# marbl/Winnowmap

Measured on AMD Instinct MI355X. Metric: mapped Gbp/s, higher is better.
Workload: dtype int8

## Files before the change

__graft_entry__.py:

```python
import os
import sys

ROOT = os.path.dirname(os.path.abspath(__file__))
sys.path.insert(0, ROOT)
sys.path.insert(0, os.path.join(ROOT, "tests"))


def build():
    from winnowmap_amd import build as b
    b.build_gpu(verbose=True)
    b.build_oracle()
    b.build_emu()
    b.build_emu_selfmap()
    b.build_emu_sdust()
    b.build_emu_heapseed()
    b.build_emu_evenk()
    b.build_emu_sketchsteps()
    b.build_emu_extra()
    b.build_emu_fix()
    b.build_emu_eqx()
    b.build_emu_cs()
    b.build_emu_chain()
    b.build_harness()
    import winnowmap_amd
    from winnowmap_amd import gpu
    gpu.lib()


def smoke():
    import numpy as np
    from winnowmap_amd import gpu
    import wmtest as W
    import kswcases
    ctx = gpu.Context(0, 2 << 30)
    cases = kswcases.ont_segments(5, 64)
    sc = gpu.KswScore(2, -4, -1, 4, 2, 24, 1)
    jobs, seqs = gpu.pack_jobs([(c["q"], c["t"], dict(w=c["w"], zdrop=c["zdrop"], end_bonus=c["end_bonus"], flag=c["flag"])) for c in cases])
    res, pool = ctx.ksw_batch(sc, jobs, seqs)
    for i, c in enumerate(cases):
        o = W.o_ksw_extd2(c["q"], c["t"], w=c["w"], zdrop=c["zdrop"], end_bonus=c["end_bonus"], flag=c["flag"])
        assert all(int(res[i][k]) == o[k] for k in W.EZ_FIELDS), (i, res[i], o)
        assert np.array_equal(pool[res[i]["cig_off"]:res[i]["cig_off"] + res[i]["n_cigar"]], o["cigar"]), i
    import ctypes as C
    import tempfile
    from winnowmap_amd import build as b, synth
    tmp = tempfile.mkdtemp()
    ref = synth.make_reference(1, 200000, 5, repeat_frac=0.1)
    fa = os.path.join(tmp, "ref.fa")
    synth.write_fasta(fa, ref)
    km, cnt = synth.repetitive_kmers(ref, 15)
    kf = os.path.join(tmp, "rep.txt")
    synth.write_kmer_list(kf, km, cnt, 15)
    reads, _ = synth.make_reads(ref, 4, 12000, 6, profile="ont", sv_frac=0.25)
    rs = [synth.codes_to_ascii(r) for r in reads]
    idx = gpu.Index(fa, kf, k=15, w=50, n_threads=4)
    idx.upload(ctx)
    m = gpu.Mapper(ctx, idx, "map-ont", gpu.MM_F_CIGAR | gpu.MM_F_OUT_CG)
    text, hits, cigars, first = m.map(["r%d" % i for i in range(len(rs))], rs)
    H = C.CDLL(b.build_harness())
    H.h_index_build.restype = C.c_void_p
    H.h_index_build.argtypes = [C.c_char_p, C.c_char_p, C.c_int, C.c_int, C.c_int]
    H.h_map_many.argtypes = [C.c_void_p, C.c_char_p, C.c_int64, C.c_int, C.POINTER(C.c_char_p), W.i32p, C.c_int, W.i32p, C.c_int, C.POINTER(C.c_int64), W.u32p, C.c_int64, C.POINTER(C.c_int64)]
    hh = H.h_index_build(fa.encode(), kf.encode(), 15, 50, 4)
    n = len(rs)
    ho = np.zeros(16 * 1024, np.int32); co = np.zeros(4000000, np.uint32); hf = (C.c_int64 * (n + 1))(); nc = C.c_int64()
    nh = H.h_map_many(hh, b"map-ont", 0x4 | 0x20, n, (C.c_char_p * n)(*rs), np.array([len(r) for r in rs], np.int32), 2, ho, 1024, hf, co, len(co), C.byref(nc))
    assert nh == len(hits) and nh > 0, (nh, len(hits))
    assert np.array_equal(ho[:16 * nh].reshape(-1, 16), hits) and np.array_equal(co[:nc.value], cigars) and list(hf) == list(first)
    m.close(); idx.close(); ctx.close()
    print("smoke OK: %d ksw alignments and %d end-to-end hits (%d CIGAR ops) bit-exact vs the oracle" % (len(cases), nh, nc.value))


if __name__ == "__main__":
    build()
    if len(sys.argv) > 1 and sys.argv[1] == "smoke":
        smoke()
```

include/wm_gpu.h:

```cpp
#ifndef WM_GPU_H
#define WM_GPU_H
#include <stdint.h>
#include <stddef.h>
#ifdef __cplusplus
extern "C" {
#endif

#define WM_OK        0
#define WM_ENODEV   (-1)
#define WM_EINVAL   (-2)
#define WM_ENOMEM   (-3)
#define WM_EINTERNAL (-4)

typedef struct wm_ctx_s wm_ctx_t;

typedef struct { uint64_t x, y; } wm128_t;

int wm_ctx_create(int device, size_t arena_bytes, wm_ctx_t **out);
void wm_ctx_destroy(wm_ctx_t *ctx);
const char *wm_last_error(void);
const char *wm_build_defines(void);
int wm_device_count(void);
float wm_last_kernel_ms(const wm_ctx_t *ctx);
int wm_ctx_device(const wm_ctx_t *ctx);

typedef struct {
	int8_t match, mismatch, sc_ambi;
	int8_t q, e, q2, e2;
} wm_ksw_score_t;

typedef struct {
	uint32_t q_off, t_off;
	int32_t qlen, tlen;
	int32_t w, zdrop, end_bonus, flag;
} wm_ksw_job_t;

typedef struct {
	int32_t max, zdropped, max_q, max_t, mqe, mqe_t, mte, mte_q, score, reach_end;
	int32_t n_cigar;
	uint32_t cig_off;
} wm_ksw_result_t;

#define WM_KSW_MAX_TLEN (1 << 28)

int wm_ksw_batch(wm_ctx_t *ctx, const wm_ksw_score_t *sc, int n_jobs, const wm_ksw_job_t *jobs,
                 const uint8_t *seqs, size_t seqs_bytes,
                 wm_ksw_result_t *results, uint32_t *cigar_pool, size_t cigar_cap, size_t *cigar_used);

typedef struct {
	int64_t qwin_off;
	int32_t qwin_len, q_pos;
	int32_t rid, t_pos;
	int32_t qlen, tlen;
	int32_t w, zdrop, end_bonus, flag;
	int8_t step, has_n, pad[6];
} wm_ksw_pos_t;
int wm_reads_upload(wm_ctx_t *ctx, const uint8_t *codes, size_t n);
int wm_ksw_batch_pos(wm_ctx_t *ctx, const wm_ksw_score_t *sc, int n_jobs, const wm_ksw_pos_t *jobs,
                     wm_ksw_result_t *results, uint32_t *cigar_pool, size_t cigar_cap, size_t *cigar_used);
#define WM_KSW_F_ZDWALK 0x10000
typedef struct { int32_t max_zdrop, t0, t1, q0, q1; } wm_zd_t;
int wm_ksw_batch_pos_zd(wm_ctx_t *ctx, const wm_ksw_score_t *sc, int n_jobs, const wm_ksw_pos_t *jobs,
                        wm_ksw_result_t *results, uint32_t *cigar_pool, size_t cigar_cap, size_t *cigar_used, wm_zd_t *zd);

#define WM_EXTRA_MAX_ABS (1 << 30)
typedef struct { int32_t match, mismatch, ambi, q, e; } wm_extra_score_t;
typedef struct { uint32_t q_off, t_off; uint32_t cig_off; int32_t n_cigar; } wm_extra_job_t;
typedef struct { int64_t qwin_off; int32_t qwin_len, q_pos, rid, t_pos; uint32_t cig_off; int32_t n_cigar; } wm_extra_pos_t;
typedef struct { int32_t dp_max, mlen, blen, n_ambi, qoff, toff; } wm_extra_res_t;
int wm_extra_batch(wm_ctx_t *ctx, const wm_extra_score_t *score, int n_jobs, const wm_extra_job_t *jobs, const uint8_t *seqs, size_t seqs_bytes,
                   const uint32_t *cigars, size_t n_ops, wm_extra_res_t *out);
int wm_extra_batch_pos(wm_ctx_t *ctx, const wm_extra_score_t *score, int n_jobs, const wm_extra_pos_t *jobs, const uint32_t *cigars, size_t n_ops,
                       wm_extra_res_t *out);
typedef struct { int32_t n_cigar, qshift, tshift, changed; } wm_fix_res_t;
int wm_fix_extra_batch(wm_ctx_t *ctx, const wm_extra_score_t *score, int n_jobs, const wm_extra_job_t *jobs, const uint8_t *seqs, size_t seqs_bytes,
                       const uint32_t *cigars, size_t n_ops, uint32_t *cigars_out, wm_fix_res_t *fix_out, wm_extra_res_t *extra_out);
int wm_fix_extra_batch_pos(wm_ctx_t *ctx, const wm_extra_score_t *score, int n_jobs, const wm_extra_pos_t *jobs, const uint32_t *cigars, size_t n_ops,
                           uint32_t *cigars_out, wm_fix_res_t *fix_out, wm_extra_res_t *extra_out);
void wm_extra_set_routing(int long_min_cols, int tile_cols);
int wm_extra_tile_cols(void);
void wm_set_extra_device(int on);
int wm_extra_device_enabled(void);
void wm_extra_stats(uint64_t *out6, int reset);
void wm_set_fix_device(int on);
int wm_fix_device_enabled(void);
void wm_fix_stats(uint64_t *out7, int reset);
typedef struct { uint64_t off; int32_t n_cigar, in_place; } wm_eqx_res_t;
int wm_eqx_batch(wm_ctx_t *ctx, int n_jobs, const wm_extra_job_t *jobs, const uint8_t *seqs, size_t seqs_bytes, const uint32_t *cigars, size_t n_ops,
                 uint32_t *cigars_out, size_t out_cap, size_t *out_used, wm_eqx_res_t *out);
int wm_eqx_batch_pos(wm_ctx_t *ctx, int n_jobs, const wm_extra_pos_t *jobs, const uint32_t *cigars, size_t n_ops,
                     uint32_t *cigars_out, size_t out_cap, size_t *out_used, wm_eqx_res_t *out);
void wm_set_eqx_device(int on);
int wm_eqx_device_enabled(void);
void wm_eqx_stats(uint64_t *out6, int reset);
#define WM_CS_SHORT 0
#define WM_CS_LONG  1
#define WM_CS_MD    2
typedef struct { uint64_t off; uint32_t len; int32_t pad; } wm_cs_res_t;
int wm_cs_batch(wm_ctx_t *ctx, int mode, int n_jobs, const wm_extra_job_t *jobs, const uint8_t *seqs, size_t seqs_bytes, const uint32_t *cigars, size_t n_ops,
                char *text_out, size_t out_cap, size_t *out_used, wm_cs_res_t *out);
int wm_cs_batch_pos(wm_ctx_t *ctx, int mode, int n_jobs, const wm_extra_pos_t *jobs, const uint32_t *cigars, size_t n_ops,
                    char *text_out, size_t out_cap, size_t *out_used, wm_cs_res_t *out);
void wm_set_cs_device(int on);
int wm_cs_device_enabled(void);
void wm_cs_stats(uint64_t *out6, int reset);

int wm_debug_stripe_timing(uint64_t *out16, int reset);

int wm_ksw_ll_i16(int qlen, const uint8_t *query, int tlen, const uint8_t *target, const int8_t *mat5x5, int gapo, int gape, int *qe, int *te);

int wm_ksw_exts2_batch(wm_ctx_t *ctx, const wm_ksw_score_t *sc, int noncan, int junc_bonus, int n_jobs, const wm_ksw_job_t *jobs,
                       const uint8_t *seqs, size_t seqs_bytes, const uint8_t *junc,
                       wm_ksw_result_t *results, uint32_t *cigar_pool, size_t cigar_cap, size_t *cigar_used);

typedef struct wm_ksw_dev_batch_s wm_ksw_dev_batch_t;
int wm_ksw_dev_prepare(wm_ctx_t *ctx, const wm_ksw_score_t *sc, int n_jobs, const wm_ksw_job_t *jobs,
                       const uint8_t *seqs, size_t seqs_bytes, wm_ksw_dev_batch_t **out);
int wm_ksw_dev_run(wm_ctx_t *ctx, wm_ksw_dev_batch_t *b);
int wm_ksw_dev_fetch(wm_ctx_t *ctx, wm_ksw_dev_batch_t *b, wm_ksw_result_t *results,
                     uint32_t *cigar_pool, size_t cigar_cap, size_t *cigar_used);
int wm_ksw_dev_stats(const wm_ksw_dev_batch_t *b, uint64_t *cells, uint64_t *tb_bytes, float *dp_ms, float *bt_ms);
void wm_ksw_dev_free(wm_ctx_t *ctx, wm_ksw_dev_batch_t *b);

void wm_ksw_set_routing(int on, int rows4, int rows8);
void wm_ksw_set_chain_routing(int mode, int min_rows_exact, int bp);
void wm_ksw_set_dual(int on);
int wm_ksw_dual_enabled(void);

int wm_ksw_extd2(wm_ctx_t *ctx, int qlen, const uint8_t *query, int tlen, const uint8_t *target, int8_t m,
                 const int8_t *mat, int8_t q, int8_t e, int8_t q2, int8_t e2, int w, int zdrop, int end_bonus,
                 int flag, wm_ksw_result_t *ez, uint32_t **cigar_out);

typedef struct wm_index_s wm_index_t;
int wm_index_build(const char *fasta, const char *kmer_file, int k, int w, int n_threads, wm_index_t **out);
int wm_index_build_gpu(wm_ctx_t *ctx, const char *fasta, const char *kmer_file, int k, int w, int n_threads, wm_index_t **out, double *stats);
int wm_index_build_flag(const char *fasta, const char *kmer_file, int k, int w, int idx_flag, int n_threads, wm_index_t **out);
int wm_index_build_gpu_flag(wm_ctx_t *ctx, const char *fasta, const char *kmer_file, int k, int w, int idx_flag, int n_threads, wm_index_t **out, double *stats);
void wm_index_destroy(wm_index_t *idx);
int wm_index_save(const wm_index_t *idx, const char *path);
int wm_index_load(const char *path, const char *kmer_file, wm_index_t **out);
int wm_index_upload(wm_ctx_t *ctx, const wm_index_t *idx);
int wm_index_read_junc_bed(wm_index_t *idx, const char *path);
int wm_index_add_junc(wm_index_t *idx, int ctg, int n, const int32_t *st, const int32_t *en, const int32_t *strand);
int wm_index_n_seq(const wm_index_t *idx);
const char *wm_index_seq_name(const wm_index_t *idx, int rid);
int wm_index_seq_len(const wm_index_t *idx, int rid);
uint64_t wm_index_n_minimizers(const wm_index_t *idx);
const uint64_t *wm_index_get(const wm_index_t *idx, uint64_t minier, int *n);

int wm_write_repetitive_kmers(const char *fasta, int k, double distinct, const char *out_path, uint64_t *n_out);
int wm_write_repetitive_kmers_gpu(wm_ctx_t *ctx, const char *fasta, int k, double distinct, const char *out_path, uint64_t *n_out, double *stats);
int wm_index_export(const wm_index_t *idx, uint64_t *sizes9, uint32_t *S, uint64_t *hkey, uint64_t *hval, uint64_t *P, uint8_t *bloom,
                    uint64_t *seq_meta, char *names);
int wm_index_import(const uint64_t *sizes9, const uint32_t *S, const uint64_t *hkey, const uint64_t *hval, const uint64_t *P, const uint8_t *bloom,
                    const uint64_t *seq_meta, const char *names, wm_index_t **out);

int wm_sketch_batch(wm_ctx_t *ctx, int n, const uint8_t *seqs, size_t seqs_bytes, const uint64_t *seq_off, const int32_t *len,
                    wm128_t *out, size_t out_cap, uint64_t *out_off, int32_t *counts);
int wm_sketch_set_filter(wm_ctx_t *ctx, const uint8_t *bits, size_t n_bytes, uint64_t table_bits, uint32_t salt0, uint32_t salt1, int k, int w);
int wm_seed_batch(wm_ctx_t *ctx, int n, const wm128_t *mini, const uint64_t *mini_off, const int32_t *n_mini, const int32_t *qlen,
                  int max_occ, int64_t flag, wm128_t *out, size_t out_cap, uint64_t *out_off, int32_t *n_anchors, int32_t *rep_len);
typedef struct { uint32_t lo, eq; } wm_qkey_t;
int wm_index_query_key(const wm_index_t *idx, const char *qname, wm_qkey_t *key);
int wm_seed_batch_keyed(wm_ctx_t *ctx, int n, const wm128_t *mini, const uint64_t *mini_off, const int32_t *n_mini, const int32_t *qlen, const wm_qkey_t *keys,
                        int max_occ, int64_t flag, wm128_t *out, size_t out_cap, uint64_t *out_off, int32_t *n_anchors, int32_t *rep_len);
typedef struct { int32_t max_dist_x, min_dist_x, max_dist_y, bw, max_skip, max_iter, min_cnt, min_sc; float gap_scale;
                 int32_t is_cdna;  } wm_chain_par_t;
int wm_chain_batch(wm_ctx_t *ctx, int n, wm128_t *a, const uint64_t *a_off, const int32_t *n_a, const wm_chain_par_t *par,
                   uint64_t *u, uint64_t *u_off, int32_t *n_u, int32_t *n_v);
typedef struct {
	int64_t seq_off;
	uint64_t stage_off, pre_off;
	int32_t len, n_pre;
	wm_chain_par_t par;
} wm_window_job_t;
typedef struct { int32_t n_anchors, rep_len, n_mini, n_u, n_v; uint32_t u_off, a_off; } wm_window_res_t;
int wm_window_batch(wm_ctx_t *ctx, int n, const wm_window_job_t *jobs, const uint8_t *seqs, size_t seqs_bytes, const wm128_t *pre, size_t n_pre_total,
                    int max_occ, int64_t flag, wm_window_res_t *res, uint64_t *u_pool, size_t u_cap, size_t *u_used, wm128_t *a_pool, size_t a_cap, size_t *a_used);
int wm_window_batch_keyed(wm_ctx_t *ctx, int n, const wm_window_job_t *jobs, const wm_qkey_t *keys, const uint8_t *seqs, size_t seqs_bytes, const wm128_t *pre, size_t n_pre_total,
                          int max_occ, int64_t flag, wm_window_res_t *res, uint64_t *u_pool, size_t u_cap, size_t *u_used, wm128_t *a_pool, size_t a_cap, size_t *a_used);
int wm_window_batch_dust(wm_ctx_t *ctx, int n, const wm_window_job_t *jobs, const wm_qkey_t *keys, const uint8_t *seqs, size_t seqs_bytes, const wm128_t *pre, size_t n_pre_total,
                         int max_occ, int64_t flag, int sdust_thres, wm_window_res_t *res, uint64_t *u_pool, size_t u_cap, size_t *u_used, wm128_t *a_pool, size_t a_cap, size_t *a_used);
int wm_sdust_batch(wm_ctx_t *ctx, int n, const uint8_t *seqs, size_t seqs_bytes, const uint64_t *seq_off, const int32_t *len, const uint8_t *resident, int thres,
                   int32_t *iv, size_t iv_cap, uint64_t *iv_off, int32_t *n_iv, int32_t *p_high);
void wm_sdust_stats(double *out5, int reset);
void wm_exts2_stats(uint64_t *out2, int reset);
float wm_last_aux_ms(const wm_ctx_t *ctx);
void wm_sketch_set_step_chunks(int on);
int wm_last_sketch_chunks(const wm_ctx_t *ctx);

typedef struct wm_mapper_s wm_mapper_t;
int wm_mapper_create(wm_ctx_t *ctx, const wm_index_t *idx, const char *preset, int64_t flag, wm_mapper_t **out);
void wm_mapper_destroy(wm_mapper_t *m);
void wm_set_even_k(int on);
int wm_even_k_enabled(void);
int wm_mapper_set_threads(wm_mapper_t *m, int n_threads, size_t arena_bytes_per_group);
int wm_map_reads(wm_mapper_t *m, int n, const char *const *names, const char *const *seqs, const int32_t *lens,
                 const char **text, size_t *text_len, const int32_t **hits, const uint32_t **cigars, const int64_t **hit_first);
#define WM_MAX_SLOTS 4
int wm_map_reads_slot(wm_mapper_t *m, int slot, int n, const char *const *names, const char *const *seqs, const int32_t *lens,
                      const char **text, size_t *text_len, const int32_t **hits, const uint32_t **cigars, const int64_t **hit_first);
int wm_mapper_set_slots(wm_mapper_t *m, int n);
int wm_map_reads_rep_len_defined(const wm_mapper_t *m, int slot, const uint8_t **flags, size_t *n);
int wm_map_file(wm_mapper_t *m, const char *reads_path, const char *out_path, int64_t mini_batch_bases, double *stats);
int wm_index_upload_dev(wm_ctx_t *ctx, const wm_index_t *idx, const void *d_S, const void *d_hkey, const void *d_hval, const void *d_P, const void *d_bloom, int src_device);
int wm_index_upload_peer(wm_ctx_t *dst, const wm_index_t *idx, const wm_ctx_t *src);
int wm_map_file_multi(wm_mapper_t *const *mappers, int n, const char *reads_path, const char *out_path, int64_t mini_batch_bases, double *stats);
int wm_mapper_set_cmdline(wm_mapper_t *m, int argc, const char *const *argv);
int wm_set_cmdline(int argc, const char *const *argv);
typedef struct {
	int64_t flag;
	int32_t seed, sdust_thres, max_qlen;
	int32_t bw, max_gap, max_gap_ref, min_gap_ref, max_frag_len;
	int32_t max_chain_skip, max_chain_iter, min_cnt, min_chain_score;
	float chain_gap_scale;
	int32_t SVaware, SVawareMinReadLength, suffixSampleOffset, min_mapq;
	float min_qcov;
	int32_t minPrefixLength, maxPrefixLength;
	float prefixIncrementFactor;
	int32_t stage2_bw, stage2_zdrop_inv, stage2_max_gap;
	float mask_level;
	int32_t mask_len;
	float pri_ratio;
	int32_t best_n;
	int32_t max_join_long, max_join_short, min_join_flank_sc;
	float min_join_flank_ratio, alt_drop;
	int32_t a, b, q, e, q2, e2, sc_ambi;
	int32_t zdrop, zdrop_inv, end_bonus, min_dp_max, min_ksw_len;
	float max_clip_ratio;
	float mid_occ_frac;
	int32_t min_mid_occ, mid_occ, max_occ;
	int64_t mini_batch_size, max_sw_mat;
	int32_t noncan, junc_bonus;
	int32_t anchor_ext_len, anchor_ext_shift;
} wm_mapopt_t;
int wm_mapopt_preset(const char *preset, wm_mapopt_t *out, int *k, int *w);
int wm_mapper_create_opt(wm_ctx_t *ctx, const wm_index_t *idx, const wm_mapopt_t *opt, wm_mapper_t **out);
int wm_index_build_parts(const char *fasta, const char *kmer_file, int k, int w, int n_threads, uint64_t batch_bases, wm_index_t **out, int cap, int *n_parts);
int wm_map_file_split(wm_ctx_t *ctx, int n_parts, wm_index_t *const *parts, const wm_mapopt_t *opt, int n_threads, const char *reads_path, const char *out_path,
                      int64_t mini_batch_bases, double *stats);
typedef struct wm_split_s wm_split_t;
int wm_split_begin(wm_ctx_t *ctx, const wm_mapopt_t *opt, int k, int w, int n_threads, const char *reads_path, int64_t mini_batch_bases, wm_split_t **out);
int wm_split_add_part(wm_split_t *s, wm_index_t *part);
int wm_split_finish(wm_split_t *s, const char *out_path, double *stats);
void wm_split_abort(wm_split_t *s);
int wm_map_file_split_fasta(wm_ctx_t *ctx, const char *fasta, const char *kmer_file, int k, int w, int build_threads, uint64_t batch_bases, int on_device,
                            const wm_mapopt_t *opt, int n_threads, const char *reads_path, const char *out_path, int64_t mini_batch_bases, double *stats, int *n_parts);

int wm_mapper_set_sam_header(wm_mapper_t *m, int on);
int wm_mapper_stats(const wm_mapper_t *m, uint64_t *out9);
int wm_mapper_kernel_stats(const wm_mapper_t *m, double *out, int cap, int *n_classes);
int wm_ksw_n_classes(void);
int wm_ctx_kernel_stats(const wm_ctx_t *ctx, double *out, int cap, int *n_classes);
int wm_mapper_kernel_union(const wm_mapper_t *m, double since_ms, double *out, int cap, double *now_ms);
int wm_mapper_host_stats(const wm_mapper_t *m, double *out, int cap);
int wm_sam_header(const wm_index_t *idx, int argc, const char *const *argv, const char **text, size_t *text_len);

#ifdef __cplusplus
}
#endif
#endif
```

winnowmap_amd/build.py:

```python
import os
import subprocess
import sys

HERE = os.path.dirname(os.path.abspath(__file__))
ROOT = os.path.dirname(HERE)
CSRC = os.path.join(HERE, "csrc")
LIB = os.path.join(HERE, "libwmgpu.so")
HIPCC = os.environ.get("HIPCC", "/opt/rocm/bin/hipcc")


class _Lock:

    def __init__(self, target):
        self.path = target + ".lock"

    def __enter__(self):
        import fcntl
        self.f = open(self.path, "w")
        fcntl.flock(self.f, fcntl.LOCK_EX)

    def __exit__(self, *a):
        import fcntl
        fcntl.flock(self.f, fcntl.LOCK_UN)
        self.f.close()
# ... 49 lines not shown
        if any(rcs):
            raise subprocess.CalledProcessError(next(r for r in rcs if r), cmds[next(i for i, r in enumerate(rcs) if r)])
        link = lambda out_: [HIPCC, "--offload-arch=gfx950", "-shared", "-fPIC", "-o", out_] + [os.path.join(objdir, u + ".o") for u in UNITS] + ["-lz", "-lpthread"]
        if verbose:
            print(" ".join(link(LIB)), file=sys.stderr)
        _run_to(LIB, link)
        with open(stamp, "w") as f:
            f.write(defines)
    return LIB


def build_oracle():
    with _Lock(os.path.join(ROOT, "oracle", "libwm_oracle.so")):
        subprocess.check_call(["make", "-C", os.path.join(ROOT, "oracle"), "oracle"], stdout=subprocess.DEVNULL)
        if os.path.exists("/root/reference/src/map.c"):
            subprocess.check_call(["make", "-C", os.path.join(ROOT, "oracle"), "ref", "-j8"], stdout=subprocess.DEVNULL)
            if os.path.exists(LIB):
                subprocess.check_call(["make", "-C", os.path.join(ROOT, "oracle"), "wm", "subst", "-j8"], stdout=subprocess.DEVNULL)


def build_emu(defines=()):
    emu = os.path.join(ROOT, "tests", "simt_emu")
    tag = "".join("_" + "".join(ch if ch.isalnum() else "_" for ch in d) for d in defines)
    out = os.path.join(emu, "libwm_emu%s.so" % tag)
    srcs = [os.path.join(emu, f) for f in ("emu_driver.cpp", "simt.h")] + [os.path.join(CSRC, f) for f in os.listdir(CSRC) if f.endswith(".h")]
    with _Lock(out):
        if _newer(out, srcs):
            _run_to(out, lambda o: ["g++", "-O1", "-std=c++17", "-fPIC", "-shared", "-ffp-contract=off", "-Wno-unknown-pragmas"] +
                    ["-D" + d for d in defines] + ["-I" + emu, "-I" + CSRC, "-o", o, os.path.join(emu, "emu_driver.cpp")])
    return out


def build_emu_selfmap():
    emu = os.path.join(ROOT, "tests", "simt_emu")
    out = os.path.join(emu, "libwm_emu_selfmap.so")
    srcs = [os.path.join(emu, f) for f in ("emu_selfmap.cpp", "simt.h")] + \
           [os.path.join(CSRC, f) for f in ("seedchain_kernel.h", "window_kernel.h", "wm_internal.h", os.path.join("host", "wm_names.h"))]
    with _Lock(out):
        if _newer(out, srcs):
            _run_to(out, lambda o: ["g++", "-O1", "-std=c++17", "-fPIC", "-shared", "-ffp-contract=off", "-Wno-unknown-pragmas",
                                    "-I" + emu, "-I" + CSRC, "-o", o, os.path.join(emu, "emu_selfmap.cpp")])
    return out


def build_emu_heapseed():
    emu = os.path.join(ROOT, "tests", "simt_emu")
    out = os.path.join(emu, "libwm_emu_heapseed.so")
    core = os.path.join(CSRC, "host", "wm_core.cpp")
    srcs = [os.path.join(emu, f) for f in ("emu_heapseed.cpp", "simt.h")] + [core] + \
           [os.path.join(CSRC, f) for f in ("seedchain_kernel.h", "window_kernel.h", "wm_internal.h", os.path.join("host", "wm_core.h"))]
    with _Lock(out):
        if _newer(out, srcs):
            _run_to(out, lambda o: ["g++", "-O1", "-std=c++17", "-fPIC", "-shared", "-pthread", "-ffp-contract=off", "-Wno-unknown-pragmas",
                                    "-I" + emu, "-I" + CSRC, "-o", o, os.path.join(emu, "emu_heapseed.cpp"), core])
    return out


def build_emu_sdust(defines=()):
    emu = os.path.join(ROOT, "tests", "simt_emu")
    tag = "".join("_" + "".join(ch if ch.isalnum() else "_" for ch in d) for d in defines)
    out = os.path.join(emu, "libwm_emu_sdust%s.so" % tag)
    srcs = [os.path.join(emu, f) for f in ("emu_sdust.cpp", "simt.h")] + \
           [os.path.join(CSRC, f) for f in ("sdust_kernel.h", "sketch_kernel.h", "reads2bit.h", "wm_internal.h", os.path.join("host", "wm_sdust.h"), os.path.join("host", "wm_core.h"))]
    with _Lock(out):
        if _newer(out, srcs):
            _run_to(out, lambda o: ["g++", "-O3", "-std=c++17", "-fPIC", "-shared", "-ffp-contract=off", "-Wno-unknown-pragmas"] +
                    ["-D" + d for d in defines] + ["-I" + emu, "-I" + CSRC, "-o", o, os.path.join(emu, "emu_sdust.cpp")])
    return out


def build_emu_evenk():
    emu = os.path.join(ROOT, "tests", "simt_emu")
    out = os.path.join(emu, "libwm_emu_evenk.so")
    srcs = [os.path.join(emu, f) for f in ("emu_evenk.cpp", "simt.h")] + [os.path.join(CSRC, f) for f in ("sketch_kernel.h", "reads2bit.h", "wm_internal.h")]
    with _Lock(out):
        if _newer(out, srcs):
            _run_to(out, lambda o: ["g++", "-O3", "-std=c++17", "-fPIC", "-shared", "-ffp-contract=off", "-Wno-unknown-pragmas",
                                    "-I" + emu, "-I" + CSRC, "-o", o, os.path.join(emu, "emu_evenk.cpp")])
    return out


def build_emu_sketchsteps():
    emu = os.path.join(ROOT, "tests", "simt_emu")
    out = os.path.join(emu, "libwm_emu_sketchsteps.so")
    srcs = [os.path.join(emu, f) for f in ("emu_sketchsteps.cpp", "simt.h")] + [os.path.join(CSRC, f) for f in ("sketch_kernel.h", "reads2bit.h", "wm_internal.h")]
    with _Lock(out):
        if _newer(out, srcs):
            _run_to(out, lambda o: ["g++", "-O3", "-std=c++17", "-fPIC", "-shared", "-ffp-contract=off", "-Wno-unknown-pragmas",
                                    "-I" + emu, "-I" + CSRC, "-o", o, os.path.join(emu, "emu_sketchsteps.cpp")])
    return out


def build_emu_extra():
    emu = os.path.join(ROOT, "tests", "simt_emu")
    out = os.path.join(emu, "libwm_emu_extra.so")
    srcs = [os.path.join(emu, f) for f in ("emu_extra.cpp", "simt.h")] + [os.path.join(CSRC, f) for f in ("extra_kernel.h", "reads2bit.h")] + \
           [os.path.join(ROOT, "include", "wm_gpu.h")]
    with _Lock(out):
        if _newer(out, srcs):
            _run_to(out, lambda o: ["g++", "-O2", "-std=c++17", "-fPIC", "-shared", "-ffp-contract=off", "-Wno-unknown-pragmas",
                                    "-I" + emu, "-I" + CSRC, "-o", o, os.path.join(emu, "emu_extra.cpp")])
    return out


def build_emu_fix():
    emu = os.path.join(ROOT, "tests", "simt_emu")
    out = os.path.join(emu, "libwm_emu_fix.so")
    srcs = [os.path.join(emu, f) for f in ("emu_fix.cpp", "simt.h")] + \
           [os.path.join(CSRC, f) for f in ("fix_kernel.h", "cigar_fix.h", "extra_kernel.h", "reads2bit.h")] + [os.path.join(ROOT, "include", "wm_gpu.h")]
    with _Lock(out):
        if _newer(out, srcs):
            _run_to(out, lambda o: ["g++", "-O2", "-std=c++17", "-fPIC", "-shared", "-ffp-contract=off", "-Wno-unknown-pragmas",
                                    "-I" + emu, "-I" + CSRC, "-o", o, os.path.join(emu, "emu_fix.cpp")])
    return out


def build_emu_eqx():
    emu = os.path.join(ROOT, "tests", "simt_emu")
    out = os.path.join(emu, "libwm_emu_eqx.so")
    srcs = [os.path.join(emu, f) for f in ("emu_eqx.cpp", "simt.h")] + \
           [os.path.join(CSRC, f) for f in ("eqx_kernel.h", "cigar_eqx.h", "extra_kernel.h", "reads2bit.h")] + [os.path.join(ROOT, "include", "wm_gpu.h")]
    with _Lock(out):
        if _newer(out, srcs):
            _run_to(out, lambda o: ["g++", "-O2", "-std=c++17", "-fPIC", "-shared", "-ffp-contract=off", "-Wno-unknown-pragmas",
                                    "-I" + emu, "-I" + CSRC, "-o", o, os.path.join(emu, "emu_eqx.cpp")])
    return out


def build_emu_cs():
    emu = os.path.join(ROOT, "tests", "simt_emu")
    out = os.path.join(emu, "libwm_emu_cs.so")
    srcs = [os.path.join(emu, f) for f in ("emu_cs.cpp", "simt.h")] + \
           [os.path.join(CSRC, f) for f in ("cs_kernel.h", "cigar_cs.h", "extra_kernel.h", "reads2bit.h")] + [os.path.join(ROOT, "include", "wm_gpu.h")]
    with _Lock(out):
        if _newer(out, srcs):
            _run_to(out, lambda o: ["g++", "-O2", "-std=c++17", "-fPIC", "-shared", "-ffp-contract=off", "-Wno-unknown-pragmas",
                                    "-I" + emu, "-I" + CSRC, "-o", o, os.path.join(emu, "emu_cs.cpp")])
    return out


def build_emu_fix_main(sanitize=True):
    emu = os.path.join(ROOT, "tests", "simt_emu")
    out = os.path.join(emu, "emu_fix_main_san" if sanitize else "emu_fix_main")
    srcs = [os.path.join(emu, f) for f in ("emu_fix_main.cpp", "emu_fix.cpp", "simt.h")] + \
           [os.path.join(CSRC, f) for f in ("fix_kernel.h", "cigar_fix.h", "extra_kernel.h", "reads2bit.h")] + [os.path.join(ROOT, "include", "wm_gpu.h")]
    with _Lock(out):
        if _newer(out, srcs):
            _run_to(out, lambda o: ["g++", "-O1", "-g", "-std=c++17", "-ffp-contract=off", "-Wno-unknown-pragmas"] +
                                   (["-fsanitize=address,undefined", "-fno-sanitize-recover=undefined", "-fno-omit-frame-pointer"] if sanitize else []) +
                                   ["-I" + emu, "-I" + CSRC, "-o", o, os.path.join(emu, "emu_fix_main.cpp"), os.path.join(emu, "emu_fix.cpp")])
    return out


def build_emu_stripe(defines=()):
    emu = os.path.join(ROOT, "tests", "simt_emu")
    tag = "".join("_" + "".join(ch if ch.isalnum() else "_" for ch in d) for d in defines)
    out = os.path.join(emu, "libwm_emu_stripe%s.so" % tag)
    srcs = [os.path.join(emu, f) for f in ("emu_stripe.cpp", "simt.h")] + \
           [os.path.join(CSRC, f) for f in ("ksw_stripe_kernel.h", "ksw_packed_kernel.h", "ksw_kernel.h", "ksw_plan.h")]
    with _Lock(out):
        if _newer(out, srcs):
            _run_to(out, lambda o: ["g++", "-O1", "-std=c++17", "-fPIC", "-shared", "-pthread", "-ffp-contract=off", "-Wno-unknown-pragmas"] +
                    ["-D" + d for d in defines] + ["-I" + emu, "-I" + CSRC, "-o", o, os.path.join(emu, "emu_stripe.cpp")])
    return out


def build_emu_chain(defines=()):
    emu = os.path.join(ROOT, "tests", "simt_emu")
    tag = "".join("_" + "".join(ch if ch.isalnum() else "_" for ch in d) for d in defines)
    out = os.path.join(emu, "libwm_emu_chain%s.so" % tag)
    srcs = [os.path.join(emu, f) for f in ("emu_chain.cpp", "simt.h")] + \
           [os.path.join(CSRC, f) for f in ("ksw_chain_kernel.h", "ksw_stripe_kernel.h", "ksw_packed_kernel.h", "ksw_kernel.h", "ksw_plan.h")]
    with _Lock(out):
        if _newer(out, srcs):
            _run_to(out, lambda o: ["g++", "-O1", "-std=c++17", "-fPIC", "-shared", "-pthread", "-ffp-contract=off", "-Wno-unknown-pragmas"] +
                    ["-D" + d for d in defines] + ["-I" + emu, "-I" + CSRC, "-o", o, os.path.join(emu, "emu_chain.cpp")])
    return out


def build_harness():
    hd = os.path.join(ROOT, "tests", "host_harness")
    out = os.path.join(hd, "libwm_harness.so")
    srcs = [os.path.join(hd, "harness.cpp"), os.path.join(ROOT, "oracle", "wm_oracle.c")] + \
           [os.path.join(CSRC, "host", f) for f in os.listdir(os.path.join(CSRC, "host"))]
    with _Lock(out):
        if _newer(out, srcs):
            _run_to(out, lambda o: ["g++", "-std=c++17", "-O2", "-g", "-ffp-contract=off", "-fPIC", "-shared", "-o", o,
                                    os.path.join(hd, "harness.cpp"), os.path.join(ROOT, "oracle", "wm_oracle.c"), "-lz", "-pthread"])
    return out


if __name__ == "__main__":
    build_gpu(force="--force" in sys.argv, verbose=True)
    build_oracle()
    build_emu()
    build_emu_selfmap()
    build_emu_heapseed()
    build_emu_sdust()
    build_emu_evenk()
    build_emu_sketchsteps()
    build_emu_extra()
    build_emu_fix()
    build_emu_eqx()
    build_emu_cs()
    build_emu_stripe()
    build_emu_chain()
    build_harness()
```

winnowmap_amd/csrc/wm_ksw.hip:

```cpp
#include "wm_rt.h"
#include "simt.h"
#include "ksw_kernel.h"
#include "ksw_packed_kernel.h"
#include "ksw_packed_multi_kernel.h"
#include "ksw_dual_kernel.h"
#include "ksw_stripe_kernel.h"
#include "ksw_chain_kernel.h"
#include "ksw_exts2_kernel.h"
#include "cigar_walk.h"
#include "reads2bit.h"

#ifndef WM_OCC_HINT
#define WM_OCC_HINT 1
#endif
template <int BP, bool CLIP, bool HASN, bool EXACT>
__global__ __launch_bounds__(64, (WM_OCC_HINT && BP == 8 && CLIP && EXACT) ? 4 : 1) void ksw_dpp_kernel(wm_ksw_score_t sc, const wm_ksw_djob_t *__restrict__ jobs,
                                                      const int *__restrict__ order, const uint8_t *__restrict__ seqs,
                                                      uint8_t *__restrict__ tb, wm_ksw_dres_t *__restrict__ res)
{
	if constexpr (EXACT || CLIP || BP >= 16) WM_SETPRIO(2);
	const int j = order[blockIdx.x];
	wmk::ksw_dp_packed<BP, CLIP, HASN, EXACT>(sc, jobs[j], seqs, tb, res + j);
}

// ... 433 lines not shown
			for (int kk = 129; kk >= 0; --kk) { pos_[kk] = acc; acc += cnt[kk]; }
			tmp.resize(o.size());
			for (int j : o) tmp[pos_[size_key(j)]++] = j;
			o.swap(tmp);
		}
	}
	size_t chain_mw = 0;
	bool chain_any = false;
	for (int kc = 0; kc < WM_KSW_NCLASS - WM_KSW_CHAIN; ++kc) {
		const int sw = 128 * wm_ksw_chain_bp[kc >> 2];
		const std::vector<int> &o = b->order[WM_KSW_CHAIN + kc];
		b->d_cmap[kc][0] = b->d_cmap[kc][1] = 0;
		for (size_t jo = 0; jo < o.size(); ++jo) {
			const wm_ksw_djob_t &d = b->jobs[o[jo]];
			const int nwv = wm_chain_nwv(d.n_col, d.tlen, sw);
			std::vector<uint4> &cm = b->cmap[kc][(d.flag & KSW_F_APPROX_MAX) ? 0 : 1];
			for (int wv = 0; wv < nwv; ++wv) cm.push_back(make_uint4((unsigned)jo, (unsigned)wv, (unsigned)(chain_mw / 16), (unsigned)nwv));
			chain_mw += ((size_t)wm_chain_box::words(nwv) + 15) & ~(size_t)15;
			chain_any = true;
		}
	}
	const size_t nj = n_jobs > 0 ? n_jobs : 1;
	auto al256 = [](size_t x) { return (x + 255) & ~(size_t)255; };
	const size_t o_ord = al256(nj * sizeof(wm_ksw_djob_t)), o_src = o_ord + al256(nj * sizeof(int));
	size_t o_cm[WM_KSW_NCLASS - WM_KSW_CHAIN][2], tab_bytes = o_src + (pos ? al256(nj * sizeof(wm_ksw_dsrc_t)) : 0);
	for (int kc = 0; kc < WM_KSW_NCLASS - WM_KSW_CHAIN; ++kc)
		for (int e = 0; e < 2; ++e) { o_cm[kc][e] = tab_bytes; tab_bytes += al256(b->cmap[kc][e].size() * sizeof(uint4)); }
	uint8_t *d_tab = (uint8_t*)arena_take(c, tab_bytes);
	b->d_jobs = (wm_ksw_djob_t*)d_tab;
	b->d_order = d_tab ? (int*)(d_tab + o_ord) : 0;
	for (int kc = 0; kc < WM_KSW_NCLASS - WM_KSW_CHAIN && d_tab; ++kc)
		for (int e = 0; e < 2; ++e) if (!b->cmap[kc][e].empty()) b->d_cmap[kc][e] = (uint4*)(d_tab + o_cm[kc][e]);
	b->d_res = (wm_ksw_dres_t*)arena_take(c, al256(nj * sizeof(wm_ksw_dres_t)) + nj * 4 + 64);
	b->d_off = b->d_res ? (uint32_t*)((uint8_t*)b->d_res + al256(nj * sizeof(wm_ksw_dres_t))) : 0;
	b->d_err = (int*)arena_take(c, 64);
	b->d_total = b->d_err ? (uint32_t*)(b->d_err + 1) : 0;
	bool any_zd = false;
	for (int i = 0; i < n_jobs && !any_zd; ++i) any_zd = (b->jobs[i].flag & WM_KSW_F_ZDWALK) != 0;
	b->d_zd = any_zd ? (wm_zd_t*)arena_take(c, nj * sizeof(wm_zd_t)) : 0;
	b->d_seqs = (uint8_t*)arena_take(c, slab_bytes + 64);
	b->slab_bytes = slab_bytes;
	wm_ksw_dsrc_t *d_src = pos && d_tab ? (wm_ksw_dsrc_t*)(d_tab + o_src) : 0;
	b->d_cig = (uint32_t*)arena_take(c, (cig_off + 16) * 4);
	b->pool_cap = cig_off + 16;
	b->d_pool = (uint32_t*)arena_take(c, b->pool_cap * 4);
	b->d_tb = (uint8_t*)arena_take(c, tb_off + 64);
	{
		uint64_t go = 0;
		for (int j : b->order[WM_KSW_GENERIC]) { const uint64_t T = ((uint64_t)b->jobs[j].tlen + 15) / 16 * 16; b->goff.push_back(go); go += 12 * T + 256; }
		b->d_gscratch = (uint8_t*)arena_take(c, go + 256);
		b->d_goff = (uint64_t*)arena_take(c, b->goff.size() * 8 + 64);
		if (!b->d_gscratch || !b->d_goff) b->d_tb = 0;
		uint64_t so = 0;
		for (int j : b->order[WM_KSW_BLOCK3]) { b->b3off.push_back(so); so += 3 * wm_ksw_blk3_wn(b->jobs[j].tlen); }
		b->d_b3state = (uint8_t*)arena_take(c, so * 4 + 256);
		b->d_b3off = (uint64_t*)arena_take(c, b->b3off.size() * 8 + 64);
		if (!b->d_b3state || !b->d_b3off) b->d_tb = 0;
	}
	if (chain_any) {
		b->mail_words = chain_mw;
		b->d_mail = (wm_mbox_t*)arena_take(c, chain_mw * 8 + 256);
		b->d_tickets = (int*)arena_take(c, 64 * sizeof(int));
		if (!b->d_mail || !b->d_tickets) b->d_tb = 0;
	}
	if (!b->d_jobs || !b->d_order || !b->d_res || !b->d_off || !b->d_total || !b->d_err || !b->d_seqs || (any_zd && !b->d_zd) || (pos && !d_src) || !b->d_cig || !b->d_pool || !b->d_tb) {
		c->arena_used = b->arena_mark;
		delete b;
		return set_err(WM_ENOMEM, "batch needs %.1f MB of traceback + buffers; arena is %.1f MB", (tb_off + cig_off * 8 + slab_bytes) / 1048576.0, c->arena_bytes / 1048576.0);
	}
	b->ord.clear();
	b->ord.reserve(nj);
	for (int k = 0; k < WM_KSW_NCLASS; ++k) b->ord.insert(b->ord.end(), b->order[k].begin(), b->order[k].end());
	UBuf<uint8_t> ptab(tab_bytes, c);
	if (n_jobs) memcpy(ptab.data(), b->jobs.data(), (size_t)n_jobs * sizeof(wm_ksw_djob_t));
	if (!b->ord.empty()) memcpy(ptab.data() + o_ord, b->ord.data(), b->ord.size() * sizeof(int));
	if (pos && n_jobs > 0) memcpy(ptab.data() + o_src, dsrc.data(), (size_t)n_jobs * sizeof(wm_ksw_dsrc_t));
	for (int kc = 0; kc < WM_KSW_NCLASS - WM_KSW_CHAIN; ++kc)
		for (int e = 0; e < 2; ++e)
			if (!b->cmap[kc][e].empty()) memcpy(ptab.data() + o_cm[kc][e], b->cmap[kc][e].data(), b->cmap[kc][e].size() * sizeof(uint4));
	HIPCHK(hipMemcpyAsync(d_tab, ptab.data(), tab_bytes, hipMemcpyHostToDevice, c->stream));
	if (pos) {
		if (n_jobs > 0) hipLaunchKernelGGL(ksw_expand_kernel, dim3(n_jobs), dim3(64), 0, c->stream, b->d_jobs, d_src, c->d_reads, c->d_reads_nm, c->d_S, b->d_seqs);
	} else if (slab_bytes) HIPCHK(hipMemcpyAsync(b->d_seqs, seqs + slab_lo, slab_bytes, hipMemcpyHostToDevice, c->stream));
	if (!b->goff.empty()) HIPCHK(hipMemcpyAsync(b->d_goff, b->goff.data(), b->goff.size() * 8, hipMemcpyHostToDevice, c->stream));
	if (!b->b3off.empty()) HIPCHK(hipMemcpyAsync(b->d_b3off, b->b3off.data(), b->b3off.size() * 8, hipMemcpyHostToDevice, c->stream));
	HIPCHK(ctx_sync(c));
	*out = b;
	return WM_OK;
}

extern "C" int wm_ksw_dev_prepare(wm_ctx_t *c, const wm_ksw_score_t *sc_in, int n_jobs, const wm_ksw_job_t *jobs,
                                  const uint8_t *seqs, size_t seqs_bytes, wm_ksw_dev_batch_t **out)
{
	return ksw_prepare_impl(c, sc_in, n_jobs, jobs, seqs, seqs_bytes, 0, out);
}

int reads_alloc(wm_ctx_t *c, size_t cap)
{
	const size_t pkw = cap / 32 + 2, nmw = cap / 64 + 2;
	c->d_reads = 0; c->d_reads_nm = 0; c->reads_cap = 0;
	if (hipMalloc((void**)&c->d_reads, (pkw + nmw) * 8) != hipSuccess) { (void)hipGetLastError(); c->d_reads = 0; return set_err(WM_ENOMEM, "cannot allocate %zu bytes for the resident reads", (pkw + nmw) * 8); }
	c->d_reads_nm = c->d_reads + pkw;
	c->reads_cap = cap;
	return WM_OK;
}
extern "C" int wm_reads_upload(wm_ctx_t *c, const uint8_t *codes, size_t n)
{
	if (!c || (n && !codes)) return set_err(WM_EINVAL, "null argument");
	HIPCHK(hipSetDevice(c->device));
	if (!c->owns_reads) { c->d_reads = 0; c->d_reads_nm = 0; c->reads_cap = 0; }
	if (n + 256 > c->reads_cap) {
		if (c->d_reads) HIPCHK(hipFree(c->d_reads));
		c->d_reads = 0; c->d_reads_nm = 0; c->reads_cap = 0;
		const size_t cap = (n + n / 8 + (1 << 20) + 255) & ~(size_t)255;
		const int rc = reads_alloc(c, cap);
		if (rc) return rc;
	}
	c->owns_reads = true;
	std::vector<uint64_t> pk(wm_pk_words(n)), nm(wm_nm_words(n));
	wm_pack_codes(codes, n, pk.data(), nm.data());
	HIPCHK(hipMemcpy(c->d_reads, pk.data(), pk.size() * 8, hipMemcpyHostToDevice));
	HIPCHK(hipMemcpy(c->d_reads_nm, nm.data(), nm.size() * 8, hipMemcpyHostToDevice));
	c->reads_bytes = n;
	return WM_OK;
}

static bool pmulti_lean() { static const bool v = !(getenv("WM_KSW_PMULTI_LEAN") && atoi(getenv("WM_KSW_PMULTI_LEAN")) == 0); return v; }
static int ksw_pmulti_level() { const char *e = getenv("WM_KSW_PMULTI"); return e ? atoi(e) : 2; }

extern "C" int wm_ksw_dev_run(wm_ctx_t *c, wm_ksw_dev_batch_t *b)
{
	HIPCHK(hipSetDevice(c->device));
	const int n = b->n_jobs;
	if (n == 0) return WM_OK;
	HIPCHK(hipMemsetAsync(b->d_err, 0, 4, c->stream));
	if (b->d_mail) {
		HIPCHK(hipMemsetAsync(b->d_mail, 0xff, b->mail_words * 8, c->stream));
		HIPCHK(hipMemsetAsync(b->d_tickets, 0, 64 * sizeof(int), c->stream));
	}
	if (!b->degenerate.empty()) hipLaunchKernelGGL(ksw_reset_kernel, dim3((n + 255) / 256), dim3(256), 0, c->stream, n, b->d_jobs, b->d_res);
	HIPCHK(hipEventRecord(c->ev[0], c->stream));
	int off = 0;
	static const bool trace_k = getenv("WM_TRACE_KSW") != 0;
	auto class_done = [&](int k, double t0) {
		if (!trace_k) return;
		hipStreamSynchronize(c->stream);
		const std::vector<int> &o = b->order[k];
		const wm_ksw_djob_t &big = b->jobs[o[0]];
		fprintf(stderr, "[ksw class %2d] jobs %zu  %.2f ms  largest q=%d t=%d w=%d flag=0x%x n_col=%d\n", k, o.size(), now_ms() - t0, big.qlen, big.tlen, big.w, big.flag, big.n_col);
	};
	int n_nonempty = 0, used_mask = 0, rr = 0;
	for (int k = 0; k < WM_KSW_NCLASS; ++k) n_nonempty += !b->order[k].empty();
	static const int n_side = std::max(0, std::min(4, getenv("WM_SIDE_STREAMS") ? atoi(getenv("WM_SIDE_STREAMS")) : 3));
	const bool fan = n_nonempty > 1 && !trace_k && n_side > 0;
	if (fan) HIPCHK(hipEventRecord(c->kev[4], c->stream));
	hipStream_t ks = c->stream;
	hipStream_t side[4] = {0, 0, 0, 0};
	int pool_lo = 0, pool_n = c->n_side_pool, wclass = 0;
	if (c->side_pool && c->n_side_pool >= 6) {
		static const long heavy_units = getenv("WM_KSW_HEAVY_UNITS") ? atol(getenv("WM_KSW_HEAVY_UNITS")) : 8192, huge_units = getenv("WM_KSW_HUGE_UNITS") ? atol(getenv("WM_KSW_HUGE_UNITS")) : 131072;
		static int split_l = -1, split_h = -1;
		if (split_l < 0) { int a, h; side_split(c->n_side_pool, &a, &h); split_h = h; split_l = a; }
		if (split_l > 0 && split_h > 0 && split_l + split_h < c->n_side_pool) {
			long mx = 0;
			for (const wm_ksw_djob_t &d : b->jobs) {
				if (d.klass < 0) continue;
				long w_ = d.w < 0 ? std::max(d.qlen, d.tlen) : d.w, nn = std::min(d.qlen, d.tlen);
				if (nn > w_ + 1) nn = w_ + 1;
				mx = std::max(mx, ((long)d.qlen + d.tlen) * ((nn + 127) / 128 + 1));
			}
			wclass = huge_units > 0 && mx > huge_units ? 2 : heavy_units > 0 && mx > heavy_units ? 1 : 0;
			pool_lo = wclass == 0 ? 0 : wclass == 1 ? split_l : split_l + split_h;
			pool_n = wclass == 0 ? split_l : wclass == 1 ? split_h : c->n_side_pool - split_l - split_h;
		}
	}
	const int n_use = c->side_pool ? std::min(n_side, pool_n) : n_side;
	if (fan && n_use > 0) {
		if (c->side_pool) { const unsigned b0 = c->side_next[wclass].fetch_add((unsigned)n_use); for (int i = 0; i < n_use; ++i) side[i] = c->side_pool[pool_lo + (int)((b0 + (unsigned)i) % (unsigned)pool_n)]; }
		else for (int i = 0; i < n_use; ++i) { if (!c->kstream[i]) HIPCHK(hipStreamCreateWithFlags(&c->kstream[i], hipStreamNonBlocking)); side[i] = c->kstream[i]; }
	}
	auto next_stream = [&]() {
		if (!fan || n_use <= 0) return;
		const int si = rr++ % n_use;
		ks = side[si];
		if (!(used_mask >> si & 1)) { hipStreamWaitEvent(ks, c->kev[4], 0); used_mask |= 1 << si; }
	};
	static const bool class_events = !(getenv("WM_KSW_CLASS_EVENTS") && atoi(getenv("WM_KSW_CLASS_EVENTS")) == 0);
	int offs[WM_KSW_NCLASS + 1];
	offs[0] = 0;
	for (int k = 0; k < WM_KSW_NCLASS; ++k) offs[k + 1] = offs[k] + (int)b->order[k].size();
	int lorder[WM_KSW_NCLASS], nl = 0;
	lorder[nl++] = WM_KSW_GENERIC; lorder[nl++] = WM_KSW_BLOCK3; lorder[nl++] = WM_KSW_BLOCK2; lorder[nl++] = WM_KSW_BLOCK;
	for (int k = WM_KSW_NCLASS - 1; k >= WM_KSW_STRIPE; --k) lorder[nl++] = k;
	for (int k = WM_KSW_BLOCK - 1; k >= 0; --k) lorder[nl++] = k;
	for (int li = 0; li < nl; ++li) {
		const int k = lorder[li];
		const int nk = (int)b->order[k].size();
		if (nk == 0) continue;
		off = offs[k];
		next_stream();
		const double tk0 = trace_k ? now_ms() : 0;
		if (class_events) hipEventRecord(c->cev[k][0], ks);
		struct Done { decltype(class_done) &f; int k; double t; hipEvent_t e; hipStream_t s; bool on; ~Done() { if (on) hipEventRecord(e, s); f(k, t); } } done_guard{ class_done, k, tk0, c->cev[k][1], ks, class_events };
		if (k == WM_KSW_BLOCK || k == WM_KSW_BLOCK2 || k == WM_KSW_BLOCK3) {
			const size_t fixed = (size_t)WM_KSW_BLK_PUB * 4;
			if (k == WM_KSW_BLOCK || k == WM_KSW_BLOCK2) {
				const int seq_cap = 64 * 1024;
				if (k == WM_KSW_BLOCK) {
					const size_t lds = (size_t)wmk::ksw_pmulti_lds<4, 8>::INTS * 4 + seq_cap;
					HIPCHK(hipFuncSetAttribute((const void*)ksw_pmulti_kernel<4, 8>, hipFuncAttributeMaxDynamicSharedMemorySize, (int)lds));
					hipLaunchKernelGGL((ksw_pmulti_kernel<4, 8>), dim3(nk), dim3(64 * 8), lds, ks, b->sc, b->d_jobs, b->d_order + off, b->d_seqs, b->d_tb, b->d_res, seq_cap);
				} else {
					const size_t lds = (size_t)wmk::ksw_pmulti_lds<8, 8>::INTS * 4 + seq_cap;
					HIPCHK(hipFuncSetAttribute((const void*)ksw_pmulti_kernel<8, 8>, hipFuncAttributeMaxDynamicSharedMemorySize, (int)lds));
					hipLaunchKernelGGL((ksw_pmulti_kernel<8, 8>), dim3(nk), dim3(64 * 8), lds, ks, b->sc, b->d_jobs, b->d_order + off, b->d_seqs, b->d_tb, b->d_res, seq_cap);
				}
			} else {
				const size_t lds = fixed + WM_KSW_BLK3_SEQ_LDS;
				HIPCHK(hipFuncSetAttribute((const void*)ksw_block_kernel<WM_KSW_BLK2_K, 0>, hipFuncAttributeMaxDynamicSharedMemorySize, (int)lds));
				hipLaunchKernelGGL((ksw_block_kernel<WM_KSW_BLK2_K, 0>), dim3(nk), dim3(64 * WM_KSW_BLK_NWV), lds, ks, b->sc, b->d_jobs, b->d_order + off, b->d_seqs, b->d_tb, b->d_res, (int)WM_KSW_BLK3_SEQ_LDS, (int*)b->d_b3state, b->d_b3off);
			}
			continue;
		}
		if (k >= WM_KSW_CHAIN) {
			const int kc = k - WM_KSW_CHAIN, var = kc & 3;
			for (int e = 1; e >= 0; --e) {
				const int nw = (int)b->cmap[kc][e].size();
				if (!nw) continue;
				if (wm_ksw_chain_bp[kc >> 2] == 2) {
					if (e) launch_chain<2, true>(var, nw, ks, b->sc, b->d_jobs, b->d_order + off, b->d_seqs, b->d_tb, b->d_res, b->d_cmap[kc][e], b->d_tickets + 2 * kc + e, b->d_mail);
					else launch_chain<2, false>(var, nw, ks, b->sc, b->d_jobs, b->d_order + off, b->d_seqs, b->d_tb, b->d_res, b->d_cmap[kc][e], b->d_tickets + 2 * kc + e, b->d_mail);
				} else {
					if (e) launch_chain<4, true>(var, nw, ks, b->sc, b->d_jobs, b->d_order + off, b->d_seqs, b->d_tb, b->d_res, b->d_cmap[kc][e], b->d_tickets + 2 * kc + e, b->d_mail);
					else launch_chain<4, false>(var, nw, ks, b->sc, b->d_jobs, b->d_order + off, b->d_seqs, b->d_tb, b->d_res, b->d_cmap[kc][e], b->d_tickets + 2 * kc + e, b->d_mail);
				}
			}
			continue;
		}
		if (k >= WM_KSW_STRIPE) {
			const int var = (k - WM_KSW_STRIPE) & 3;
			static const char *dump_dir = getenv("WM_KSW_DUMP");
			if (dump_dir) {
				static std::atomic<int> seq(0);
				std::vector<uint8_t> hs(b->slab_bytes + 64);
				hipStreamSynchronize(c->stream);
				hipMemcpy(hs.data(), b->d_seqs, b->slab_bytes, hipMemcpyDeviceToHost);
				char path[512];
				snprintf(path, sizeof(path), "%s/stripe_%d_%d.bin", dump_dir, (int)getpid(), seq++);
				if (FILE *fp = fopen(path, "wb")) {
					const int32_t hdr[4] = { k, nk, (int32_t)sizeof(wm_ksw_djob_t), (int32_t)sizeof(wm_ksw_score_t) };
					fwrite(hdr, 4, 4, fp); fwrite(&b->sc, sizeof(b->sc), 1, fp);
					for (int j : b->order[k]) {
						const wm_ksw_djob_t &d = b->jobs[j];
						fwrite(&d, sizeof(d), 1, fp); fwrite(hs.data() + d.q_off, 1, d.qlen, fp); fwrite(hs.data() + d.t_off, 1, d.tlen, fp);
					}
					fclose(fp);
					b->dumped.push_back(path);
				}
			}
			switch ((k - WM_KSW_STRIPE) >> 2) {
			case 0: launch_stripe<2, 4>(var, nk, ks, b->sc, b->d_jobs, b->d_order + off, b->d_seqs, b->d_tb, b->d_res); break;
			case 1: launch_stripe<2, 8>(var, nk, ks, b->sc, b->d_jobs, b->d_order + off, b->d_seqs, b->d_tb, b->d_res); break;
			case 2: launch_stripe<4, 8>(var, nk, ks, b->sc, b->d_jobs, b->d_order + off, b->d_seqs, b->d_tb, b->d_res); break;
			case 4: launch_stripe<1, 16>(var, nk, ks, b->sc, b->d_jobs, b->d_order + off, b->d_seqs, b->d_tb, b->d_res); break;
			case 5: launch_stripe<2, 16>(var, nk, ks, b->sc, b->d_jobs, b->d_order + off, b->d_seqs, b->d_tb, b->d_res); break;
			default: launch_stripe<8, 8>(var, nk, ks, b->sc, b->d_jobs, b->d_order + off, b->d_seqs, b->d_tb, b->d_res); break;
			}
			continue;
		}
		if (k == WM_KSW_GENERIC) {
			hipLaunchKernelGGL(ksw_generic_kernel, dim3(nk), dim3(64), 0, ks, b->sc, b->d_jobs, b->d_order + off, b->d_seqs, b->d_tb, b->d_gscratch, b->d_goff, b->d_res);
			continue;
		}
		switch (k & ~7) {
		case WM_KSW_P4: launch_dpp<4>(k & 7, nk, ks, b->sc, b->d_jobs, b->d_order + off, b->d_seqs, b->d_tb, b->d_res); break;
		case WM_KSW_P8: launch_dpp<8>(k & 7, nk, ks, b->sc, b->d_jobs, b->d_order + off, b->d_seqs, b->d_tb, b->d_res); break;
		default:
			if (ksw_pmulti_level() >= 2) {
				const int seq_cap = 32 * 1024;
				const size_t lds = (size_t)wmk::ksw_pmulti_lds<4, 4>::INTS * 4 + seq_cap;
				auto go = [&](auto kern) -> int {
					HIPCHK(hipFuncSetAttribute((const void*)kern, hipFuncAttributeMaxDynamicSharedMemorySize, (int)lds));
					hipLaunchKernelGGL(kern, dim3(nk), dim3(64 * 4), lds, ks, b->sc, b->d_jobs, b->d_order + off, b->d_seqs, b->d_tb, b->d_res, seq_cap);
					return WM_OK;
				};
				int rc_;
				if (!pmulti_lean()) rc_ = go(ksw_pmulti_kernel<4, 4, true, true>);
				else if ((k & 2) && (k & 1)) rc_ = go(ksw_pmulti_kernel<4, 4, true, true>);
				else if (k & 2) rc_ = go(ksw_pmulti_kernel<4, 4, true, false>);
				else if (k & 1) rc_ = go(ksw_pmulti_kernel<4, 4, false, true>);
				else rc_ = go(ksw_pmulti_kernel<4, 4, false, false>);
				if (rc_) return rc_;
			} else
				launch_dpp<16>(k & 7, nk, ks, b->sc, b->d_jobs, b->d_order + off, b->d_seqs, b->d_tb, b->d_res);
			break;
		}
	}
	for (int si = 0; si < 4; ++si)
		if (used_mask >> si & 1) { HIPCHK(hipEventRecord(c->kev[si], side[si])); HIPCHK(hipStreamWaitEvent(c->stream, c->kev[si], 0)); }
	HIPCHK(hipEventRecord(c->ev[1], c->stream));
	if (getenv("WM_KSW_COOP_BT") && atoi(getenv("WM_KSW_COOP_BT")) > 0)
		hipLaunchKernelGGL(ksw_backtrack_coop_kernel, dim3(n), dim3(64), 0, c->stream, n, b->d_jobs, b->d_tb, b->d_res, b->d_cig, b->d_err);
	else
		hipLaunchKernelGGL(ksw_backtrack_kernel, dim3((n + 63) / 64), dim3(64), 0, c->stream, n, b->d_jobs, b->d_tb, b->d_res, b->d_cig, b->d_err);
	hipLaunchKernelGGL(ksw_scan_kernel, dim3(1), dim3(1024), 0, c->stream, n, b->d_res, b->d_off, b->d_total);
	hipLaunchKernelGGL(ksw_gather_kernel, dim3(n), dim3(64), 0, c->stream, b->d_jobs, b->d_res, b->d_off, b->d_cig, b->d_pool, (uint32_t)b->pool_cap);
	if (b->d_zd) hipLaunchKernelGGL(ksw_zdwalk_kernel, dim3((n + 63) / 64), dim3(64), 0, c->stream, n, b->sc_in, b->d_jobs, b->d_res, b->d_off, b->d_pool, b->d_seqs, b->d_zd);
	HIPCHK(hipEventRecord(c->ev[2], c->stream));
	HIPCHK(hipGetLastError());
	int *h_small = c->pin_small ? c->pin_small : &b->h_err;
	uint32_t *h_total = c->pin_small ? (uint32_t*)(c->pin_small + 1) : &b->total_ops;
	if (c->pin_small) HIPCHK(hipMemcpyAsync(h_small, b->d_err, 8, hipMemcpyDeviceToHost, c->stream));
	else { HIPCHK(hipMemcpyAsync(h_small, b->d_err, 4, hipMemcpyDeviceToHost, c->stream)); HIPCHK(hipMemcpyAsync(h_total, b->d_total, 4, hipMemcpyDeviceToHost, c->stream)); }
	HIPCHK(ctx_sync(c));
	b->h_err = *h_small; b->total_ops = *h_total;
	for (const std::string &f : b->dumped) unlink(f.c_str());
	b->dumped.clear();
	HIPCHK(hipEventElapsedTime(&b->dp_ms, c->ev[0], c->ev[1]));
	HIPCHK(hipEventElapsedTime(&b->bt_ms, c->ev[1], c->ev[2]));
	c->last_ms = b->dp_ms + b->bt_ms;
	for (int k = 0; k < WM_KSW_NCLASS && class_events; ++k)
		if (!b->order[k].empty()) {
			float ms = 0;
			if (hipEventElapsedTime(&ms, c->cev[k][0], c->cev[k][1]) == hipSuccess) {
				c->k_ms[k] += ms; c->k_cells[k] += b->class_cells[k]; c->k_launches[k] += 1;
				float t0 = 0;
				if (hipEvent_t base = device_base_event(c->device)) if (hipEventElapsedTime(&t0, base, c->cev[k][0]) == hipSuccess) {
					std::lock_guard<std::mutex> lk(c->iv_mu);
					if (c->k_iv[k].size() > 100000) c->k_iv[k].erase(c->k_iv[k].begin(), c->k_iv[k].begin() + 50000);
					c->k_iv[k].push_back(std::make_pair(t0, t0 + ms));
				}
			}
		}
	if (b->h_err == 2) return set_err(WM_EINTERNAL, "a stripe-pipelined / chained-workgroup alignment kernel gave up waiting for a neighbouring wavefront (watchdog, ksw_stripe_kernel.h, ksw_chain_kernel.h); WM_KSW_CHAIN=0 / WM_KSW_STRIPE=0 route around them");
	if (b->h_err) return set_err(WM_EINTERNAL, "cigar slot overflow in backtrack");
	return WM_OK;
}

extern "C" int wm_ksw_dev_fetch(wm_ctx_t *c, wm_ksw_dev_batch_t *b, wm_ksw_result_t *results, uint32_t *cigar_pool, size_t cigar_cap, size_t *cigar_used)
try {
	HIPCHK(hipSetDevice(c->device));
	const int n = b->n_jobs;
	if (cigar_used) *cigar_used = b->total_ops;
	if (n == 0) return WM_OK;
	const size_t off_at = (size_t)((uint8_t*)b->d_off - (uint8_t*)b->d_res);
	UBuf<uint8_t> ro(off_at + (size_t)n * 4, c);
	const wm_ksw_dres_t *res = (const wm_ksw_dres_t*)ro.data();
	const uint32_t *off = (const uint32_t*)(ro.data() + off_at);
	if (b->total_ops > cigar_cap) return set_err(WM_ENOMEM, "cigar_pool too small: need %u ops", b->total_ops);
	HIPCHK(hipMemcpyAsync(ro.data(), b->d_res, off_at + (size_t)n * 4, hipMemcpyDeviceToHost, c->stream));
	if (b->total_ops) HIPCHK(hipMemcpyAsync(cigar_pool, b->d_pool, (size_t)b->total_ops * 4, hipMemcpyDeviceToHost, c->stream));
	HIPCHK(ctx_sync(c));
	WM_SITE("ksw.results");
	wm::parallel_for(c->host_threads, (size_t)n, [&](size_t i) {
		wm_ksw_result_t &o = results[i];
		const wm_ksw_dres_t &r = res[i];
		o.max = r.max; o.zdropped = r.zdropped; o.max_q = r.max_q; o.max_t = r.max_t; o.mqe = r.mqe; o.mqe_t = r.mqe_t;
		o.mte = r.mte; o.mte_q = r.mte_q; o.score = r.score; o.reach_end = r.reach_end; o.n_cigar = r.n_cigar; o.cig_off = off[i];
	});
	return WM_OK;
}
catch (const std::bad_alloc &) { return set_err(WM_ENOMEM, "out of host memory"); }

extern "C" int wm_ksw_dev_stats(const wm_ksw_dev_batch_t *b, uint64_t *cells, uint64_t *tb_bytes, float *dp_ms, float *bt_ms)
{
	if (cells) *cells = b->cells;
	if (tb_bytes) *tb_bytes = b->tb_bytes;
	if (dp_ms) *dp_ms = b->dp_ms;
	if (bt_ms) *bt_ms = b->bt_ms;
	return WM_OK;
}

extern "C" void wm_ksw_dev_free(wm_ctx_t *c, wm_ksw_dev_batch_t *b)
{
	if (!b) return;
	if (c && c->arena_used >= b->arena_mark) c->arena_used = b->arena_mark;
	delete b;
}

static int ksw_fetch_zd(wm_ctx_t *c, wm_ksw_dev_batch_t *b, wm_zd_t *out)
{
	const int n = b->n_jobs;
	if (!b->d_zd) { for (int i = 0; i < n; ++i) out[i] = wm_zd_t{ 0, -1, -1, -1, -1 }; return WM_OK; }
	if (n == 0) return WM_OK;
	HIPCHK(hipSetDevice(c->device));
	UBuf<wm_zd_t> z(n, c);
	HIPCHK(hipMemcpyAsync(z.data(), b->d_zd, (size_t)n * sizeof(wm_zd_t), hipMemcpyDeviceToHost, c->stream));
	HIPCHK(ctx_sync(c));
	memcpy(out, z.data(), (size_t)n * sizeof(wm_zd_t));
	return WM_OK;
}

static int ksw_batch_impl(wm_ctx_t *c, const wm_ksw_score_t *sc, int n_jobs, const wm_ksw_job_t *jobs, const uint8_t *seqs, size_t seqs_bytes, const wm_ksw_pos_t *pos,
                          wm_ksw_result_t *results, uint32_t *cigar_pool, size_t cigar_cap, size_t *cigar_used, wm_zd_t *zd = 0)
{
	if (!c) return set_err(WM_EINVAL, "null context");
	size_t used = 0;
	int i0 = 0;
	float kms = 0;
	const size_t budget = (size_t)(c->arena_bytes * 0.8);
	while (i0 < n_jobs || (n_jobs == 0 && i0 == 0)) {
		int i1 = i0;
		size_t need = 0;
		while (i1 < n_jobs) {
			const int ql = pos ? pos[i1].qlen : jobs[i1].qlen, tl = pos ? pos[i1].tlen : jobs[i1].tlen, w = pos ? pos[i1].w : jobs[i1].w;
			size_t t = 128;
			if (ql > 0 && tl > 0) t = ((size_t)ql + tl) * ((size_t)wm_ksw_ncol(ql, tl, w) + 10) + 512;
			if (i1 > i0 && need + t > budget) break;
			need += t; ++i1;
		}
		wm_ksw_dev_batch_t *b = 0;
		const double ta = now_ms();
		int rc = ksw_prepare_impl(c, sc, i1 - i0, pos ? 0 : jobs + i0, seqs, seqs_bytes, pos ? pos + i0 : 0, &b);
		if (rc) return rc;
		const double tb_ = now_ms();
		rc = wm_ksw_dev_run(c, b);
		const double tc = now_ms();
		size_t u = 0;
		if (!rc) rc = wm_ksw_dev_fetch(c, b, results + i0, cigar_pool + used, cigar_cap - used, &u);
		if (!rc && zd) rc = ksw_fetch_zd(c, b, zd + i0);
		c->acc_cells += b->cells; c->t_prep += tb_ - ta; c->t_run += tc - tb_; c->t_fetch += now_ms() - tc; kms += b->dp_ms + b->bt_ms;
		wm_ksw_dev_free(c, b);
		if (rc) { if (cigar_used) *cigar_used = used + u; return rc; }
		for (int i = i0; i < i1; ++i) results[i].cig_off += (uint32_t)used;
		used += u;
		i0 = i1;
		if (n_jobs == 0) break;
	}
	if (cigar_used) *cigar_used = used;
	c->last_ms = kms;
	return WM_OK;
}

extern "C" int wm_ksw_batch(wm_ctx_t *c, const wm_ksw_score_t *sc, int n_jobs, const wm_ksw_job_t *jobs, const uint8_t *seqs, size_t seqs_bytes,
                            wm_ksw_result_t *results, uint32_t *cigar_pool, size_t cigar_cap, size_t *cigar_used)
{
	return ksw_batch_impl(c, sc, n_jobs, jobs, seqs, seqs_bytes, 0, results, cigar_pool, cigar_cap, cigar_used);
}

extern "C" int wm_ksw_batch_pos(wm_ctx_t *c, const wm_ksw_score_t *sc, int n_jobs, const wm_ksw_pos_t *jobs,
                                wm_ksw_result_t *results, uint32_t *cigar_pool, size_t cigar_cap, size_t *cigar_used)
{
	if (n_jobs > 0 && !jobs) return set_err(WM_EINVAL, "null jobs");
	return ksw_batch_impl(c, sc, n_jobs, 0, 0, 0, jobs, results, cigar_pool, cigar_cap, cigar_used);
}

extern "C" int wm_ksw_batch_pos_zd(wm_ctx_t *c, const wm_ksw_score_t *sc, int n_jobs, const wm_ksw_pos_t *jobs,
                                   wm_ksw_result_t *results, uint32_t *cigar_pool, size_t cigar_cap, size_t *cigar_used, wm_zd_t *zd)
{
	if (n_jobs > 0 && (!jobs || !zd)) return set_err(WM_EINVAL, "null jobs / zd");
	return ksw_batch_impl(c, sc, n_jobs, 0, 0, 0, jobs, results, cigar_pool, cigar_cap, cigar_used, zd);
}

extern "C" int wm_debug_stripe_timing(uint64_t *out16, int reset)
{
#ifdef WM_STRIPE_TIMING
	unsigned long long h[16];
	if (hipMemcpyFromSymbol(h, HIP_SYMBOL(g_wm_stripe_timing), sizeof(h)) != hipSuccess) return set_err(WM_EINTERNAL, "hipMemcpyFromSymbol: %s", hipGetErrorString(hipGetLastError()));
	for (int i = 0; i < 16; ++i) out16[i] = h[i];
	if (reset) { memset(h, 0, sizeof(h)); if (hipMemcpyToSymbol(HIP_SYMBOL(g_wm_stripe_timing), h, sizeof(h)) != hipSuccess) return set_err(WM_EINTERNAL, "hipMemcpyToSymbol failed"); }
	return WM_OK;
#else
	(void)out16; (void)reset;
	return set_err(WM_EINVAL, "this library was not built with WM_STRIPE_TIMING");
#endif
}

extern "C" int wm_ksw_extd2(wm_ctx_t *c, int qlen, const uint8_t *query, int tlen, const uint8_t *target, int8_t m, const int8_t *mat,
                            int8_t q, int8_t e, int8_t q2, int8_t e2, int w, int zdrop, int end_bonus, int flag, wm_ksw_result_t *ez, uint32_t **cigar_out)
{
	if (m != 5) return set_err(WM_EINVAL, "only the 5-letter alphabet of src/align.c:9 is supported");
	wm_ksw_score_t sc = { mat[0], mat[1], mat[24], q, e, q2, e2 };
	wm_ksw_job_t jb = { 0, (uint32_t)(qlen > 0 ? qlen : 0), qlen, tlen, w, zdrop, end_bonus, flag };
	std::vector<uint8_t> seqs((qlen > 0 ? qlen : 0) + (tlen > 0 ? tlen : 0) + 1);
	if (qlen > 0) memcpy(seqs.data(), query, qlen);
	if (tlen > 0) memcpy(seqs.data() + (qlen > 0 ? qlen : 0), target, tlen);
	const size_t cap = (size_t)(qlen > 0 ? qlen : 0) + (tlen > 0 ? tlen : 0) + 4;
	uint32_t *cig = (uint32_t*)malloc(cap * 4);
	size_t used = 0;
	int rc = wm_ksw_batch(c, &sc, 1, &jb, seqs.data(), seqs.size(), ez, cig, cap, &used);
	if (rc) { free(cig); *cigar_out = 0; return rc; }
	*cigar_out = cig;
	return WM_OK;
}

__global__ __launch_bounds__(64) void ksw_exts2_kernel(wm_ksw_score_t sc, int noncan, int junc_bonus, const wm_ksw_djob_t *__restrict__ jobs,
                                                        const uint8_t *__restrict__ seqs, const uint8_t *__restrict__ junc, uint8_t *__restrict__ tb,
                                                        uint8_t *scratch, const uint64_t *__restrict__ scratch_off, wm_ksw_dres_t *__restrict__ res)
{
	const int j = blockIdx.x;
	const wm_ksw_djob_t jb = jobs[j];
	const uint64_t T = ((uint64_t)jb.tlen + 15) / 16 * 16;
	signed char *mem = (signed char*)(scratch + scratch_off[j]);
	wmk::ksw_dp_exts2<true>(sc, noncan, junc_bonus, jb, seqs, junc, tb, mem, (int*)(mem + 8 * T), res + j);
}
__global__ __launch_bounds__(64) void ksw_exts2_backtrack_kernel(wm_ksw_score_t sc, int n, const wm_ksw_djob_t *__restrict__ jobs, const uint8_t *__restrict__ tb,
                                                                  wm_ksw_dres_t *__restrict__ res, uint32_t *__restrict__ cig_scratch, int *__restrict__ err)
{
	const int j = blockIdx.x * 64 + threadIdx.x;
	if (j >= n) return;
	wm_ksw_dres_t r = res[j];
	int nc = 0;
	if (r.bt_i == KSW_BT_WATCHDOG) atomicMax(err, 2);
	if (r.bt_i >= 0) {
		nc = wmk::ksw_exts2_backtrack_thread(sc, jobs[j], tb, r.bt_i, r.bt_j, cig_scratch + jobs[j].cig_off, jobs[j].cig_cap);
		if (nc < 0) { atomicMax(err, 1); nc = 0; }
	}
	res[j].n_cigar = nc;
}

extern "C" int wm_ksw_exts2_batch(wm_ctx_t *c, const wm_ksw_score_t *sc_in, int noncan, int junc_bonus, int n_jobs, const wm_ksw_job_t *jobs,
                                  const uint8_t *seqs, size_t seqs_bytes, const uint8_t *junc,
                                  wm_ksw_result_t *results, uint32_t *cigar_pool, size_t cigar_cap, size_t *cigar_used)
try {
	if (!c) return set_err(WM_EINVAL, "null context");
	if (cigar_used) *cigar_used = 0;
	if (n_jobs < 0) return set_err(WM_EINVAL, "n_jobs < 0");
	if (n_jobs == 0) return WM_OK;
	if (!sc_in || !jobs || !seqs || !results) return set_err(WM_EINVAL, "null argument");
	const wm_ksw_score_t sc = *sc_in;
	const int sc_bad = wm_ksw_exts2_score_check(&sc);
	if (sc_bad == 1) return set_err(WM_EINVAL, "ksw_exts2 needs e > 0 and q2 > q + e (src/ksw2_exts2_sse.c:66)");
	if (sc_bad == 2) return set_err(WM_EINVAL, "mismatch penalty above 2 (q + e): the reference returns without aligning (src/ksw2_exts2_sse.c:84)");
	if (sc_bad == 3) return set_err(WM_EINVAL, "N score below -2 (q + e): the reference returns without aligning (src/ksw2_exts2_sse.c:84)");
	if (noncan < -127 || noncan > 127 || junc_bonus < -127 || junc_bonus > 127) return set_err(WM_EINVAL, "noncan / junc_bonus are int8 in the reference");
	HIPCHK(hipSetDevice(c->device));
	ArenaMark mark(c);
	std::vector<wm_ksw_djob_t> dj(n_jobs);
	std::vector<uint64_t> soff(n_jobs);
	uint64_t tb_off = 0, cig_off = 0, sc_off = 0;
	for (int i = 0; i < n_jobs; ++i) {
		const wm_ksw_job_t &jb = jobs[i];
		if (jb.qlen <= 0 || jb.tlen <= 0) return set_err(WM_EINVAL, "job %d: empty operand", i);
		if (jb.tlen > WM_KSW_MAX_TLEN) return set_err(WM_EINVAL, "job %d: target longer than WM_KSW_MAX_TLEN = %d bases (the exact-maximum reduction carries the target lane in 28 bits)", i, WM_KSW_MAX_TLEN);
		if ((uint64_t)jb.q_off + jb.qlen > seqs_bytes || (uint64_t)jb.t_off + jb.tlen > seqs_bytes) return set_err(WM_EINVAL, "job %d: operands outside seqs", i);
		if (jb.flag & (0x01 | 0x04 | 0x10)) return set_err(WM_EINVAL, "job %d: KSW_EZ_SCORE_ONLY / GENERIC_SC / APPROX_DROP are not supported", i);
		wm_ksw_djob_t &d = dj[i];
		memset(&d, 0, sizeof(d));
		d.q_off = jb.q_off; d.t_off = jb.t_off; d.qlen = jb.qlen; d.tlen = jb.tlen; d.w = -1; d.zdrop = jb.zdrop; d.end_bonus = 0; d.flag = jb.flag;
		d.n_col = (((jb.qlen < jb.tlen ? jb.qlen : jb.tlen) + 15) / 16 + 1) * 16;
		d.tb_off = tb_off;
		tb_off += ((uint64_t)(jb.qlen + jb.tlen - 1) * d.n_col + 15) & ~(uint64_t)15;
		d.cig_off = (uint32_t)cig_off; d.cig_cap = jb.qlen + jb.tlen + 2;
		cig_off += d.cig_cap;
		soff[i] = sc_off;
		sc_off += (12 * (((uint64_t)jb.tlen + 15) / 16 * 16) + 256 + 255) & ~(uint64_t)255;
	}
	if (cig_off >= ((uint64_t)1 << 32)) return set_err(WM_ENOMEM, "ksw_exts2: batch too large (split it)");
	const size_t nj = (size_t)n_jobs;
	wm_ksw_djob_t *d_jobs = (wm_ksw_djob_t*)arena_take(c, nj * sizeof(wm_ksw_djob_t));
	uint64_t *d_soff = (uint64_t*)arena_take(c, nj * 8);
	wm_ksw_dres_t *d_res = (wm_ksw_dres_t*)arena_take(c, nj * sizeof(wm_ksw_dres_t));
	uint32_t *d_off = (uint32_t*)arena_take(c, nj * 4 + 64);
	uint32_t *d_total = (uint32_t*)arena_take(c, 64);
	int *d_err = (int*)arena_take(c, 64);
	uint8_t *d_seqs = (uint8_t*)arena_take(c, seqs_bytes + 64);
	uint8_t *d_junc = junc ? (uint8_t*)arena_take(c, seqs_bytes + 64) : 0;
	uint32_t *d_cig = (uint32_t*)arena_take(c, (cig_off + 16) * 4);
	uint32_t *d_pool = (uint32_t*)arena_take(c, (cig_off + 16) * 4);
	uint8_t *d_scratch = (uint8_t*)arena_take(c, sc_off + 256);
	uint8_t *d_tb = (uint8_t*)arena_take(c, tb_off + 64);
	if (!d_jobs || !d_soff || !d_res || !d_off || !d_total || !d_err || !d_seqs || (junc && !d_junc) || !d_cig || !d_pool || !d_scratch || !d_tb)
		return set_err(WM_ENOMEM, "ksw_exts2: batch does not fit the arena (%llu traceback bytes); split it", (unsigned long long)tb_off);
	HIPCHK(hipMemcpyAsync(d_jobs, dj.data(), nj * sizeof(wm_ksw_djob_t), hipMemcpyHostToDevice, c->stream));
	HIPCHK(hipMemcpyAsync(d_soff, soff.data(), nj * 8, hipMemcpyHostToDevice, c->stream));
	HIPCHK(hipMemcpyAsync(d_seqs, seqs, seqs_bytes, hipMemcpyHostToDevice, c->stream));
	if (junc) HIPCHK(hipMemcpyAsync(d_junc, junc, seqs_bytes, hipMemcpyHostToDevice, c->stream));
	HIPCHK(hipMemsetAsync(d_err, 0, 4, c->stream));
	hipLaunchKernelGGL(ksw_exts2_kernel, dim3(n_jobs), dim3(64), 0, c->stream, sc, noncan, junc_bonus, d_jobs, d_seqs, d_junc, d_tb, d_scratch, d_soff, d_res);
	hipLaunchKernelGGL(ksw_exts2_backtrack_kernel, dim3((n_jobs + 63) / 64), dim3(64), 0, c->stream, sc, n_jobs, d_jobs, d_tb, d_res, d_cig, d_err);
	hipLaunchKernelGGL(ksw_scan_kernel, dim3(1), dim3(1024), 0, c->stream, n_jobs, d_res, d_off, d_total);
	hipLaunchKernelGGL(ksw_gather_kernel, dim3(n_jobs), dim3(64), 0, c->stream, d_jobs, d_res, d_off, d_cig, d_pool, (uint32_t)(cig_off + 16));
	HIPCHK(hipGetLastError());
	UBuf<wm_ksw_dres_t> res(nj, c);
	UBuf<uint32_t> off(nj, c);
	UBuf<uint32_t> small(4, c);
// ... 25 lines not shown
```

winnowmap_amd/csrc/wm_mapper.hip:

```cpp
#include "wm_rt.h"
#include "reads2bit.h"
#include "host/wm_core.cpp"
#include "host/wm_index.cpp"
#include "host/wm_seqio.cpp"
#include "host/wm_hit.cpp"
#include "host/wm_chain.cpp"
#include "host/wm_ops.cpp"
#include "host/wm_align.cpp"
#include "host/wm_mapper.cpp"
#include "host/wm_format.cpp"
#include "host/wm_kmers.cpp"
#include "host/wm_pipeline.cpp"

static std::atomic<uint64_t> g_exts2_calls{0}, g_exts2_groups{0};
extern "C" void wm_exts2_stats(uint64_t *out2, int reset)
{
	if (out2) { out2[0] = g_exts2_calls.load(); out2[1] = g_exts2_groups.load(); }
	if (reset) { g_exts2_calls = 0; g_exts2_groups = 0; }
}

struct GpuOpsCtx {
	wm_ctx_t *c;
	uint64_t cells = 0;
	double ksw_us = 0, aux_us = 0;
// ... 323 lines not shown
	}
	bool cs_batch(std::vector<wm::CsReq*> &reqs)
	{
		const int n = (int)reqs.size();
		if (!resident || n == 0) return false;
		const int mode = reqs[0]->mode;
		uint64_t bound = 0;
		for (int i = 0; i < n; ++i) {
			const wm::CsReq &r = *reqs[i];
			if (!r.resident() || r.mode != mode || wm_cigar_cs_check(mode, r.cigar->data(), (int)r.cigar->size()) != -1) return false;
			const int64_t b = wm_cigar_cs_bound(r.cigar->data(), (int)r.cigar->size());
			if (b >= ((int64_t)1 << 31)) return false;
			bound += (uint64_t)b;
		}
		const double t0 = now_ms();
		std::vector<wm_extra_pos_t> jobs(n);
		size_t tot = 0;
		for (int i = 0; i < n; ++i) {
			const wm::CsReq &r = *reqs[i];
			wm_extra_pos_t &j = jobs[i];
			j.qwin_off = r.qwin_off; j.qwin_len = r.qwin_len; j.q_pos = r.q_pos; j.rid = r.rid; j.t_pos = r.rs; j.cig_off = (uint32_t)tot; j.n_cigar = (int32_t)r.cigar->size();
			tot += r.cigar->size();
		}
		if (tot >= ((size_t)1 << 31)) { error = "cs batch exceeds 2^31 CIGAR ops"; return true; }
		UBuf<uint32_t> cig(tot + 1, c);
		WM_SITE("cs.cigars");
		wm::parallel_for(c->host_threads, (size_t)n, [&](size_t i) { if (!reqs[i]->cigar->empty()) memcpy(cig.data() + jobs[i].cig_off, reqs[i]->cigar->data(), reqs[i]->cigar->size() * 4); });
		std::vector<wm_cs_res_t> res(n);
		size_t cap = (size_t)(bound / 8) + 64, used = 0;
		std::vector<char> pool(cap);
		int rc = wm_cs_batch_pos(c, mode, n, jobs.data(), cig.data(), tot, pool.data(), cap, &used, res.data());
		if (rc == WM_ENOMEM && used > cap) { cap = used; pool.resize(cap); rc = wm_cs_batch_pos(c, mode, n, jobs.data(), cig.data(), tot, pool.data(), cap, &used, res.data()); }
		if (rc) { fail("cs"); return true; }
		WM_SITE("cs.unpack");
		wm::parallel_for(c->host_threads, (size_t)n, [&](size_t i) { reqs[i]->body->assign(pool.data() + res[i].off, (size_t)res[i].len); });
		wm::CsStats &st = wm::cs_stats();
		st.on_device += (uint64_t)n; ++st.calls; st.bytes += (uint64_t)used; st.us += (uint64_t)((now_ms() - t0) * 1e3);
		return true;
	}
	void exts2_batch(const wm_ksw_score_t &sc, int noncan, int junc_bonus, std::vector<wm::KswReq*> &reqs)
	{
		const size_t budget = (size_t)(c->arena_bytes * 0.6);
		const int n = (int)reqs.size();
		if (n > 0) ++g_exts2_calls;
		for (int i0 = 0; i0 < n;) {
			size_t need = 0, tot = 0, cap = 16;
			int i1 = i0;
			for (; i1 < n; ++i1) {
				const wm::KswReq &r = *reqs[i1];
				const size_t n_col = (size_t)((((r.ql < r.tl ? r.ql : r.tl) + 15) / 16 + 1) * 16);
				const size_t b = ((size_t)r.ql + r.tl) * (n_col + 10) + 16 * (size_t)r.tl + 1024;
				if (i1 > i0 && (need + b > budget || tot + r.ql + r.tl >= ((size_t)1 << 31))) break;
				need += b; tot += (size_t)r.ql + r.tl; cap += (size_t)r.ql + r.tl + 2;
			}
			const int m = i1 - i0;
			++g_exts2_groups;
			std::vector<wm_ksw_job_t> jobs(m);
			std::vector<wm_ksw_result_t> res(m);
			std::vector<uint8_t> seqs(tot + 1), junc;
			std::vector<uint32_t> pool(cap);
			size_t off = 0, used = 0;
			bool any_junc = false;
			for (int i = 0; i < m; ++i) any_junc |= !reqs[i0 + i]->junc.empty();
			if (any_junc) junc.assign(tot + 1, 0);
			for (int i = 0; i < m; ++i) {
				wm::KswReq &r = *reqs[i0 + i];
				jobs[i].q_off = (uint32_t)off; off += (size_t)r.ql;
				jobs[i].t_off = (uint32_t)off; off += (size_t)r.tl;
				jobs[i].qlen = r.ql; jobs[i].tlen = r.tl; jobs[i].w = -1; jobs[i].zdrop = r.zdrop; jobs[i].end_bonus = 0; jobs[i].flag = r.flag;
			}
			wm::parallel_for(c->host_threads, (size_t)m, [&](size_t i) {
				const wm::KswReq &r = *reqs[i0 + i];
				r.copy_query(seqs.data() + jobs[i].q_off); r.copy_target(seqs.data() + jobs[i].t_off);
				if (!r.junc.empty()) memcpy(junc.data() + jobs[i].t_off, r.junc.data(), r.junc.size());
			});
			if (wm_ksw_exts2_batch(c, &sc, noncan, junc_bonus, m, jobs.data(), seqs.data(), tot, any_junc ? junc.data() : 0, res.data(), pool.data(), cap, &used)) { fail("ksw_exts2"); return; }
			for (int i = 0; i < m; ++i) {
				reqs[i0 + i]->ez = res[i];
				reqs[i0 + i]->cigar.assign(pool.begin() + res[i].cig_off, pool.begin() + res[i].cig_off + res[i].n_cigar);
			}
			i0 = i1;
		}
	}
};

struct GpuOps {
	std::vector<GpuOpsCtx> ctxs;
	std::vector<int> free_;
	std::mutex mu;
	std::condition_variable cv;
	void init(const std::vector<wm_ctx_t*> &cs) { ctxs.resize(cs.size()); for (size_t i = 0; i < cs.size(); ++i) { ctxs[i].c = cs[i]; free_.push_back((int)i); } }
	int max_inflight() const { return (int)ctxs.size(); }
	bool waits_asleep() const { return getenv("WM_SPIN_SYNC") == 0; }
	std::mutex reads_mu;
	hipStream_t up_stream = 0;
	uint64_t *stage[WM_MAX_SLOTS] = { 0 }; size_t stage_words[WM_MAX_SLOTS] = { 0 }; bool stage_pinned[WM_MAX_SLOTS] = { false };
	~GpuOps()
	{
		if (up_stream) hipStreamDestroy(up_stream);
		for (int i = 0; i < WM_MAX_SLOTS; ++i) if (stage[i]) { if (stage_pinned[i]) hipHostFree(stage[i]); else free(stage[i]); }
	}
	size_t slab = 0;
	int n_slabs = 0;
	std::atomic<int> slots_hint{0};
	bool slot_busy[WM_MAX_SLOTS] = { false };
	bool load_reads(const uint8_t *codes, size_t n, int slot, int64_t *base, std::string &err)
	{
		*base = 0;
		const bool off = getenv("WM_NO_RESIDENT") != 0;
		if (off || ctxs.empty() || slot < 0 || slot >= WM_MAX_SLOTS) return false;
		wm_ctx_t *c0 = ctxs[0].c;
		std::lock_guard<std::mutex> lk(reads_mu);
		if (hipSetDevice(c0->device) != hipSuccess) return false;
		if (slot + 1 > slots_hint.load()) slots_hint = slot + 1;
		if (n + 256 > slab || slot >= n_slabs || !c0->d_reads || !c0->owns_reads) {
			for (int o = 0; o < WM_MAX_SLOTS; ++o) if (o != slot && slot_busy[o]) {
				static std::atomic<bool> told(false);
				if (!told.exchange(true)) fprintf(stderr, "[wmgpu] mini-batch on slot %d is served from host views (no resident slab: %d slab(s) of %zu bases, another slot busy); "
				                                  "tell the mapper how many mini-batches are in flight (wm_mapper_set_slots / WM_READ_SLABS)\n", slot, n_slabs, slab);
				return false;
			}
			if (c0->d_reads && c0->owns_reads) hipFree(c0->d_reads);
			c0->d_reads = 0; c0->owns_reads = false; slab = 0;
			const size_t want = (n + n / 8 + (1 << 20) + 255) & ~(size_t)255;
			n_slabs = std::max(2, std::min((int)WM_MAX_SLOTS, getenv("WM_READ_SLABS") ? atoi(getenv("WM_READ_SLABS")) : std::max(slots_hint.load(), getenv("WM_MAP_LANES") ? atoi(getenv("WM_MAP_LANES")) : 2)));
			if (slot >= n_slabs) n_slabs = slot + 1;
			if (reads_alloc(c0, (size_t)n_slabs * want) != WM_OK) return false;
			c0->owns_reads = true; c0->reads_bytes = (size_t)n_slabs * want; slab = want;
			for (size_t i = 1; i < ctxs.size(); ++i) {
				wm_ctx_t *c = ctxs[i].c;
				if (c->owns_reads && c->d_reads) hipFree(c->d_reads);
				c->d_reads = c0->d_reads; c->d_reads_nm = c0->d_reads_nm; c->reads_bytes = c0->reads_bytes; c->reads_cap = 0; c->owns_reads = false;
			}
		}
		const size_t pkw = wm_pk_words(n), nmw = wm_nm_words(n);
		if (stage_words[slot] < pkw + nmw) {
			if (stage[slot]) { if (stage_pinned[slot]) hipHostFree(stage[slot]); else free(stage[slot]); }
			stage[slot] = 0; stage_words[slot] = 0;
			const size_t want_w = pkw + nmw + (pkw + nmw) / 8 + 1024;
			stage_pinned[slot] = hipHostMalloc((void**)&stage[slot], want_w * 8, hipHostMallocDefault) == hipSuccess;
			if (!stage_pinned[slot]) { (void)hipGetLastError(); stage[slot] = (uint64_t*)malloc(want_w * 8); }
			if (!stage[slot]) { err = "no host memory for the packed reads"; return false; }
			stage_words[slot] = want_w;
		}
		uint64_t *h_pk = stage[slot], *h_nm = stage[slot] + pkw;
		{
			const size_t CH = (size_t)1 << 22;
			const size_t n_ch = (n + CH - 1) / CH;
			const int nt = (int)std::max<size_t>(1, std::min<size_t>(std::min<size_t>(8, (size_t)wm::usable_cores()), n_ch));
			wm::parallel_for(nt, n_ch, [&](size_t ci) { const size_t at = ci * CH, len = std::min(CH, n - at); wm_pack_blocks(codes + at, len, h_pk + at / 32, h_nm + at / 64); });
			for (size_t i = 2 * ((n + 63) / 64); i < pkw; ++i) h_pk[i] = 0;
			for (size_t i = (n + 63) / 64; i < nmw; ++i) h_nm[i] = 0;
		}
		if (!up_stream && hipStreamCreateWithFlags(&up_stream, hipStreamNonBlocking) != hipSuccess) { up_stream = 0; (void)hipGetLastError(); }
		uint64_t *d_pk = c0->d_reads + (size_t)slot * slab / 32, *d_nm = c0->d_reads_nm + (size_t)slot * slab / 64;
		if (n && (up_stream ? (hipMemcpyAsync(d_pk, h_pk, pkw * 8, hipMemcpyHostToDevice, up_stream) != hipSuccess || hipMemcpyAsync(d_nm, h_nm, nmw * 8, hipMemcpyHostToDevice, up_stream) != hipSuccess ||
		                       hipStreamSynchronize(up_stream) != hipSuccess)
		                    : (hipMemcpy(d_pk, h_pk, pkw * 8, hipMemcpyHostToDevice) != hipSuccess || hipMemcpy(d_nm, h_nm, nmw * 8, hipMemcpyHostToDevice) != hipSuccess))) {
			err = std::string("reads upload: ") + hipGetErrorString(hipGetLastError()); return false;
		}
		for (GpuOpsCtx &x : ctxs) x.resident = true;
		slot_busy[slot] = true;
		*base = (int64_t)((size_t)slot * slab);
		return true;
	}
	void release_reads(int slot) { std::lock_guard<std::mutex> lk(reads_mu); if (slot >= 0 && slot < WM_MAX_SLOTS) slot_busy[slot] = false; }
	template <class F> void with(wm::ErrorSink &sink, F f)
	{
		{ std::lock_guard<std::mutex> lk(sink.mu); if (!sink.msg.empty()) return; }
		int i;
		{ std::unique_lock<std::mutex> lk(mu); cv.wait(lk, [&] { return !free_.empty(); }); i = free_.back(); free_.pop_back(); }
		ctxs[i].error.clear();
		try { f(ctxs[i]); }
		catch (const std::exception &e) { if (ctxs[i].error.empty()) ctxs[i].error = std::string("batched device call: ") + e.what(); }
		if (!ctxs[i].error.empty()) { sink.put(ctxs[i].error); ctxs[i].error.clear(); }
		{ std::lock_guard<std::mutex> lk(mu); free_.push_back(i); }
		cv.notify_one();
	}
	template <class R, class F> static void run_split(GpuOpsCtx &x, std::vector<R*> &reqs, F f)
	{
		if (!x.error.empty()) return;
		f(reqs);
		if (x.error.empty() || reqs.size() < 2 || x.error.find("does not fit the arena") == std::string::npos) return;
		x.error.clear();
		std::vector<R*> a(reqs.begin(), reqs.begin() + reqs.size() / 2), b(reqs.begin() + reqs.size() / 2, reqs.end());
		run_split(x, a, f);
		if (x.error.empty()) run_split(x, b, f);
	}
	void sketch_batch(wm::ErrorSink &e, int w, int k, std::vector<wm::SketchReq*> &reqs) { with(e, [&](GpuOpsCtx &x) { run_split(x, reqs, [&](std::vector<wm::SketchReq*> &part) { x.sketch_batch(w, k, part); }); }); }
	void seed_batch(wm::ErrorSink &e, std::vector<wm::SeedReq*> &reqs) { with(e, [&](GpuOpsCtx &x) { run_split(x, reqs, [&](std::vector<wm::SeedReq*> &part) { x.seed_batch(part); }); }); }
	void chain_batch(wm::ErrorSink &e, std::vector<wm::ChainReq*> &reqs) { with(e, [&](GpuOpsCtx &x) { run_split(x, reqs, [&](std::vector<wm::ChainReq*> &part) { x.chain_batch(part); }); }); }
	void ksw_batch(wm::ErrorSink &e, const wm_ksw_score_t &sc, std::vector<wm::KswReq*> &reqs) { with(e, [&](GpuOpsCtx &x) { x.ksw_batch(sc, reqs); }); }
	void exts2_batch(wm::ErrorSink &e, const wm_ksw_score_t &sc, int noncan, int junc_bonus, std::vector<wm::KswReq*> &reqs) { with(e, [&](GpuOpsCtx &x) { x.exts2_batch(sc, noncan, junc_bonus, reqs); }); }
	void extra_batch(wm::ErrorSink &e, const wm_extra_score_t &sc, std::vector<wm::ExtraReq*> &reqs, bool *served)
	{
		*served = false;
		with(e, [&](GpuOpsCtx &x) { bool all = true; run_split(x, reqs, [&](std::vector<wm::ExtraReq*> &part) { all = x.extra_batch(sc, part) && all; }); *served = all; });
	}
	template <class R, class F> void batch_or_rest(wm::ErrorSink &e, std::vector<R*> &reqs, std::vector<R*> &rest, F call)
	{
		bool ran = false;
		with(e, [&](GpuOpsCtx &x) { ran = true; run_split(x, reqs, [&](std::vector<R*> &part) { if (!call(x, part)) rest.insert(rest.end(), part.begin(), part.end()); }); });
		if (!ran) rest = reqs;
	}
	void window_batch(wm::ErrorSink &e, std::vector<wm::WindowReq*> &reqs) { with(e, [&](GpuOpsCtx &x) { run_split(x, reqs, [&](std::vector<wm::WindowReq*> &part) { x.window_batch(part); }); }); }
};

struct CallOps : wm::DeviceOps {
	GpuOps &g;
	wm::ErrorSink err;
	explicit CallOps(GpuOps &g_) : g(g_) {}
	int max_inflight() const override { return g.max_inflight(); }
	bool waits_asleep() const override { return g.waits_asleep(); }
	bool load_reads(const uint8_t *codes, size_t n, int slot, int64_t *base) override
	{
		std::string e;
		const bool ok = g.load_reads(codes, n, slot, base, e);
		if (!e.empty()) err.put(e);
		return ok;
	}
	void release_reads(int slot) override { g.release_reads(slot); }
	void sketch_batch(int w, int k, std::vector<wm::SketchReq*> &reqs) override { g.sketch_batch(err, w, k, reqs); }
	void seed_batch(std::vector<wm::SeedReq*> &reqs) override { g.seed_batch(err, reqs); }
	void chain_batch(std::vector<wm::ChainReq*> &reqs) override { g.chain_batch(err, reqs); }
	void ksw_batch(const wm_ksw_score_t &sc, std::vector<wm::KswReq*> &reqs) override { g.ksw_batch(err, sc, reqs); }
	void exts2_batch(const wm_ksw_score_t &sc, int noncan, int junc_bonus, std::vector<wm::KswReq*> &reqs) override { g.exts2_batch(err, sc, noncan, junc_bonus, reqs); }
	void window_batch(int, int, std::vector<wm::WindowReq*> &reqs) override { g.window_batch(err, reqs); }
	void extra_batch(const wm_extra_score_t &sc, std::vector<wm::ExtraReq*> &reqs) override
	{
		bool served = false;
		g.extra_batch(err, sc, reqs, &served);
		if (!served) wm::DeviceOps::extra_batch(sc, reqs);
	}
	void fix_extra_batch(const wm_extra_score_t &sc, std::vector<wm::FixReq*> &reqs) override
	{
		std::vector<wm::FixReq*> rest;
		g.batch_or_rest(err, reqs, rest, [&](GpuOpsCtx &x, std::vector<wm::FixReq*> &part) { return x.fix_extra_batch(sc, part); });
		if (!rest.empty()) wm::DeviceOps::fix_extra_batch(sc, rest);
	}
	void cs_batch(std::vector<wm::CsReq*> &reqs) override
	{
		std::vector<wm::CsReq*> rest;
		g.batch_or_rest(err, reqs, rest, [](GpuOpsCtx &x, std::vector<wm::CsReq*> &part) { return x.cs_batch(part); });
		if (!rest.empty()) wm::DeviceOps::cs_batch(rest);
	}
	void eqx_batch(std::vector<wm::EqxReq*> &reqs) override
	{
		std::vector<wm::EqxReq*> rest;
		g.batch_or_rest(err, reqs, rest, [](GpuOpsCtx &x, std::vector<wm::EqxReq*> &part) { return x.eqx_batch(part); });
		if (!rest.empty()) wm::DeviceOps::eqx_batch(rest);
	}
};

struct wm_mapper_s {
	wm_ctx_t *c; const wm_index_t *idx;
	std::vector<wm_ctx_t*> workers;
	int n_threads = 1;
	int n_threads_cap = 0;
	int call_threads() const { return n_threads_cap > 0 && n_threads_cap < n_threads ? n_threads_cap : n_threads; }
	wm::IdxOpt io; wm::MapOpt mo;
	struct Result { std::string text; std::vector<int32_t> hits; std::vector<uint32_t> cigars; std::vector<int64_t> first; std::vector<uint8_t> rl_defined; } res[WM_MAX_SLOTS];
	uint64_t stats[9];
	double host_stats[24] = {0};
	std::mutex stats_mu;
	std::unique_ptr<GpuOps> ops;
	int slots_hint = 0;
	bool sam_header = true;
	std::vector<std::string> cmdline;
};

static std::atomic<int> g_even_k(-1);
static bool even_k_on()
{
	const int v = g_even_k.load(std::memory_order_relaxed);
	if (v >= 0) return v != 0;
	const char *e = getenv("WM_EVEN_K");
	return e && atoi(e) != 0;
}
extern "C" void wm_set_even_k(int on) { g_even_k = on < 0 ? -1 : on ? 1 : 0; }
extern "C" int wm_even_k_enabled(void) { return even_k_on(); }
static int mapper_index_ok(const wm_index_t *idx)
{
	if (!(idx->ix.k & 1) && !even_k_on())
		return set_err(WM_EINVAL, "k = %d: the mapper's device path needs an odd k (every preset of the reference has one) unless even k is switched on: wm_set_even_k(1) or WM_EVEN_K=1", idx->ix.k);
	return WM_OK;
}
extern "C" int wm_mapper_create(wm_ctx_t *c, const wm_index_t *idx, const char *preset, int64_t flag, wm_mapper_t **out)
{
	*out = 0;
	if (!c || !idx) return set_err(WM_EINVAL, "null argument");
	if (!c->have_index) return set_err(WM_EINVAL, "wm_index_upload has not been called on this context");
	if (mapper_index_ok(idx)) return WM_EINVAL;
	wm_default_malloc();
	wm_mapper_t *m = new wm_mapper_t();
	m->c = c; m->idx = idx;
	wm::set_preset(0, m->io, m->mo);
	if (preset && preset[0] && wm::set_preset(preset, m->io, m->mo) < 0) { delete m; return set_err(WM_EINVAL, "unknown preset '%s'", preset); }
	m->mo.flag |= flag;
	m->io.k = idx->ix.k; m->io.w = idx->ix.w;
	wm::mapopt_update(m->mo, idx->ix);
	std::string err;
	if (wm::check_opt(m->io, m->mo, err) < 0) { delete m; return set_err(WM_EINVAL, "%s", err.c_str()); }
	memset(m->stats, 0, sizeof(m->stats));
	*out = m;
	return WM_OK;
}
#define WM_MAPOPT_FIELDS(X) X(flag) X(seed) X(sdust_thres) X(max_qlen) X(bw) X(max_gap) X(max_gap_ref) X(min_gap_ref) X(max_frag_len) \
	X(max_chain_skip) X(max_chain_iter) X(min_cnt) X(min_chain_score) X(chain_gap_scale) X(SVawareMinReadLength) X(suffixSampleOffset) X(min_mapq) \
	X(min_qcov) X(minPrefixLength) X(maxPrefixLength) X(prefixIncrementFactor) X(stage2_bw) X(stage2_zdrop_inv) X(stage2_max_gap) X(mask_level) \
	X(mask_len) X(pri_ratio) X(best_n) X(max_join_long) X(max_join_short) X(min_join_flank_sc) X(min_join_flank_ratio) X(alt_drop) X(a) X(b) X(q) X(e) \
	X(q2) X(e2) X(sc_ambi) X(zdrop) X(zdrop_inv) X(end_bonus) X(min_dp_max) X(min_ksw_len) X(max_clip_ratio) X(mid_occ_frac) X(min_mid_occ) X(mid_occ) \
	X(max_occ) X(mini_batch_size) X(max_sw_mat) X(noncan) X(junc_bonus) X(anchor_ext_len) X(anchor_ext_shift)
static void mapopt_to_c(const wm::MapOpt &o, wm_mapopt_t *c)
{
	memset(c, 0, sizeof(*c));
#define X(f) c->f = (decltype(c->f))o.f;
	WM_MAPOPT_FIELDS(X)
#undef X
	c->SVaware = o.SVaware ? 1 : 0;
}
static void mapopt_from_c(const wm_mapopt_t *c, wm::MapOpt &o)
{
#define X(f) o.f = (decltype(o.f))c->f;
	WM_MAPOPT_FIELDS(X)
#undef X
	o.SVaware = c->SVaware != 0;
}
extern "C" int wm_mapopt_preset(const char *preset, wm_mapopt_t *out, int *k, int *w)
{
	wm::IdxOpt io; wm::MapOpt mo;
	wm::set_preset(0, io, mo);
	if (preset && preset[0] && wm::set_preset(preset, io, mo) < 0) return set_err(WM_EINVAL, "unknown preset '%s'", preset);
	mapopt_to_c(mo, out);
	if (k) *k = io.k;
	if (w) *w = io.w;
	return WM_OK;
}
extern "C" int wm_mapper_create_opt(wm_ctx_t *c, const wm_index_t *idx, const wm_mapopt_t *opt, wm_mapper_t **out)
{
	*out = 0;
	if (!c || !idx || !opt) return set_err(WM_EINVAL, "null argument");
	if (!c->have_index) return set_err(WM_EINVAL, "wm_index_upload has not been called on this context");
	if (mapper_index_ok(idx)) return WM_EINVAL;
	wm_default_malloc();
	wm_mapper_t *m = new wm_mapper_t();
	m->c = c; m->idx = idx;
	wm::set_preset(0, m->io, m->mo);
	mapopt_from_c(opt, m->mo);
	m->io.k = idx->ix.k; m->io.w = idx->ix.w;
	wm::mapopt_update(m->mo, idx->ix);
	std::string err;
	if (wm::check_opt(m->io, m->mo, err) < 0) { delete m; return set_err(WM_EINVAL, "%s", err.c_str()); }
	memset(m->stats, 0, sizeof(m->stats));
	*out = m;
	return WM_OK;
}
extern "C" int wm_mapper_set_sam_header(wm_mapper_t *m, int on) { if (!m) return set_err(WM_EINVAL, "null mapper"); m->sam_header = on != 0; return WM_OK; }

extern "C" void wm_mapper_destroy(wm_mapper_t *m)
{
	if (!m) return;
	if (wm::prof_on()) wm::prof_report(stderr);
	for (wm_ctx_t *w : m->workers) wm_ctx_destroy(w);
	delete m;
}

extern "C" int wm_mapper_set_threads(wm_mapper_t *m, int n_threads, size_t arena_bytes_per_context)
{
	if (n_threads < 1) return set_err(WM_EINVAL, "n_threads < 1");
	for (wm_ctx_t *w : m->workers) wm_ctx_destroy(w);
	m->workers.clear();
	m->ops.reset();
	int C = getenv("WM_CONTEXTS") ? atoi(getenv("WM_CONTEXTS")) : (getenv("WM_GROUPS") ? atoi(getenv("WM_GROUPS")) : (n_threads >= 8 ? 6 : n_threads >= 2 ? 2 : 1));
	if (C < 1) C = 1;
	m->n_threads = n_threads;
	const int bt = getenv("WM_BATCH_THREADS") ? atoi(getenv("WM_BATCH_THREADS")) : 1;
	m->c->host_threads = std::max(1, bt);
	for (int g = 1; g < C; ++g) {
		wm_ctx_t *w = 0;
		const int rc = wm_ctx_create(m->c->device, arena_bytes_per_context ? arena_bytes_per_context : m->c->arena_bytes, &w);
		if (rc) return rc;
		w->d_hkey = m->c->d_hkey; w->d_hval = m->c->d_hval; w->d_P = m->c->d_P; w->d_bloom = m->c->d_bloom; w->hbits = m->c->hbits; w->skp = m->c->skp;
		w->d_S = m->c->d_S; w->d_name_rank = m->c->d_name_rank; w->d_seq_len = m->c->d_seq_len; w->seq_off = m->c->seq_off; w->seq_len = m->c->seq_len;
		w->have_index = true; w->owns_index = false;
		w->host_threads = m->c->host_threads;
		m->workers.push_back(w);
	}
	{
		const int hwq = getenv("GPU_MAX_HW_QUEUES") ? atoi(getenv("GPU_MAX_HW_QUEUES")) : 4;
		int P = getenv("WM_SIDE_POOL") ? atoi(getenv("WM_SIDE_POOL")) : std::max(0, hwq - C);
		if (C == 1) P = 0;
		wm_ctx_t *c0 = m->c;
		HIPCHK(hipStreamSynchronize(c0->stream));
		while ((int)c0->owned_pool.size() > P) { hipStreamDestroy(c0->owned_pool.back()); c0->owned_pool.pop_back(); }
		while ((int)c0->owned_pool.size() < P) { hipStream_t st; HIPCHK(hipStreamCreateWithFlags(&st, hipStreamNonBlocking)); c0->owned_pool.push_back(st); }
		c0->side_pool = P > 0 ? c0->owned_pool.data() : 0; c0->n_side_pool = P; c0->side_next = c0->owned_next;
		for (wm_ctx_t *w : m->workers) { w->side_pool = c0->side_pool; w->n_side_pool = P; w->side_next = c0->owned_next; }
	}
	{ size_t mark = 0; if (pin_take(m->c, 1, &mark)) pin_release(m->c, mark); }
	for (wm_ctx_t *w : m->workers) { size_t mark = 0; if (pin_take(w, 1, &mark)) pin_release(w, mark); }
	return WM_OK;
}

static int map_reads_impl(wm_mapper_t *m, std::vector<wm::ReadIn> &reads, double tm0, int slot = 0);

extern "C" int wm_map_reads(wm_mapper_t *m, int n, const char *const *names, const char *const *seqs, const int32_t *lens,
                            const char **text, size_t *text_len, const int32_t **hits, const uint32_t **cigars, const int64_t **hit_first)
{
	const double tm0 = now_ms();
	std::vector<wm::ReadIn> reads(n);
	wm::parallel_for(m->n_threads, (size_t)n, [&](size_t i) { reads[i].name = names[i]; reads[i].seq.assign(seqs[i], lens[i]); });
	const int rc = map_reads_impl(m, reads, tm0, 0);
	if (rc) return rc;
	if (text) *text = m->res[0].text.data();
	if (text_len) *text_len = m->res[0].text.size();
	if (hits) *hits = m->res[0].hits.data();
	if (cigars) *cigars = m->res[0].cigars.data();
	if (hit_first) *hit_first = m->res[0].first.data();
	return WM_OK;
}

extern "C" int wm_map_reads_slot(wm_mapper_t *m, int slot, int n, const char *const *names, const char *const *seqs, const int32_t *lens,
                                 const char **text, size_t *text_len, const int32_t **hits, const uint32_t **cigars, const int64_t **hit_first)
{
	if (!m || slot < 0 || slot >= WM_MAX_SLOTS) return set_err(WM_EINVAL, "slot must be 0 .. WM_MAX_SLOTS - 1");
	const double tm0 = now_ms();
	std::vector<wm::ReadIn> reads(n);
	wm::parallel_for(m->n_threads, (size_t)n, [&](size_t i) { reads[i].name = names[i]; reads[i].seq.assign(seqs[i], lens[i]); });
	const int rc = map_reads_impl(m, reads, tm0, slot);
	if (rc) return rc;
	wm_mapper_t::Result &R = m->res[slot];
	if (text) *text = R.text.data();
	if (text_len) *text_len = R.text.size();
	if (hits) *hits = R.hits.data();
	if (cigars) *cigars = R.cigars.data();
	if (hit_first) *hit_first = R.first.data();
	return WM_OK;
}

static void ensure_ops(wm_mapper_t *m)
{
	if (m->ops) return;
	m->ops.reset(new GpuOps());
	std::vector<wm_ctx_t*> cs; cs.push_back(m->c); cs.insert(cs.end(), m->workers.begin(), m->workers.end());
	m->ops->init(cs);
	m->ops->slots_hint = m->slots_hint;
}

extern "C" int wm_mapper_set_slots(wm_mapper_t *m, int n)
{
	if (!m || n < 1 || n > WM_MAX_SLOTS) return set_err(WM_EINVAL, "slots must be 1 .. WM_MAX_SLOTS");
	std::lock_guard<std::mutex> lk(m->stats_mu);
	if (n > m->slots_hint) m->slots_hint = n;
	ensure_ops(m);
	if (n > m->ops->slots_hint.load()) m->ops->slots_hint = n;
	return WM_OK;
}

extern "C" int wm_map_reads_rep_len_defined(const wm_mapper_t *m, int slot, const uint8_t **flags, size_t *n)
{
	if (!m || slot < 0 || slot >= WM_MAX_SLOTS || !flags) return set_err(WM_EINVAL, "bad argument");
	*flags = m->res[slot].rl_defined.data();
	if (n) *n = m->res[slot].rl_defined.size();
	return WM_OK;
}

static int map_reads_impl(wm_mapper_t *m, std::vector<wm::ReadIn> &reads, double tm0, int slot)
{
	wm_mapper_t::Result &R = m->res[slot];
	static const bool trace_m = getenv("WM_TRACE") != 0;
	const int n = (int)reads.size();
	uint64_t bases = 0;
	for (int i = 0; i < n; ++i) bases += reads[i].seq.size();
	std::vector<wm::ReadOut> out(n);
	const double tm1 = now_ms();
	{
		std::lock_guard<std::mutex> lk(m->stats_mu);
		ensure_ops(m);
	}
	GpuOps &ops = *m->ops;
	uint64_t cells0 = 0; double ksw_us0 = 0, aux_us0 = 0;
	for (GpuOpsCtx &x : ops.ctxs) { cells0 += x.cells; ksw_us0 += x.ksw_us; aux_us0 += x.aux_us; }
	wm::MapStats st;
	hipSetDevice(m->c->device);
	std::vector<std::string> texts(n);
	const std::function<void(size_t)> fmt = [&](size_t i) { wm::write_read(texts[i], m->idx->ix, reads[i], out[i], m->mo.flag); };
	CallOps call(ops);
	wm::map_batch(m->idx->ix, m->mo, &call, reads, out, &st, m->call_threads(), &fmt, slot);
	if (!call.err.msg.empty()) return set_err(WM_ENODEV, "%s", call.err.msg.c_str());
	if (!st.internal_error.empty()) return set_err(WM_EINTERNAL, "%s", st.internal_error.c_str());
	{ std::string ie; if (wm::take_internal_error(ie)) return set_err(WM_EINTERNAL, "%s", ie.c_str()); }
	GpuOpsCtx tot; tot.c = m->c;
	for (GpuOpsCtx &x : ops.ctxs) { tot.cells += x.cells; tot.ksw_us += x.ksw_us; tot.aux_us += x.aux_us; }
	tot.cells -= cells0; tot.ksw_us -= ksw_us0; tot.aux_us -= aux_us0;
	GpuOpsCtx &opsr = tot;
	if (getenv("WM_TRACE")) {
		double a[8] = {0};
		for (GpuOpsCtx &x : ops.ctxs) { a[0] += x.t_pack; a[1] += x.t_prep; a[2] += x.t_run; a[3] += x.t_fetch; a[4] += x.t_unpack; a[5] += x.t_sketch; a[6] += x.t_seed; a[7] += x.t_chain; }
		fprintf(stderr, "[ops, sum over %zu contexts, ms] ksw: pack %.0f prepare %.0f run %.0f fetch %.0f unpack %.0f | sketch %.0f seed %.0f chain %.0f | batches %llu\n", ops.ctxs.size(), a[0], a[1], a[2], a[3], a[4], a[5], a[6], a[7], (unsigned long long)st.n_flush);
	}
	const double tm2 = now_ms();
	std::vector<size_t> toff(n + 1, 0), coff(n + 1, 0);
	R.first.assign(n + 1, 0);
	R.rl_defined.resize(n);
	for (int i = 0; i < n; ++i) {
		R.rl_defined[i] = out[i].rep_len_defined ? 1 : 0;
		toff[i + 1] = toff[i] + texts[i].size();
		R.first[i + 1] = R.first[i] + (int64_t)out[i].regs.size();
		size_t nc = 0;
		for (const wm::Reg &r : out[i].regs) nc += r.cigar.size();
		coff[i + 1] = coff[i] + nc;
	}
	R.text.resize(toff[n]); R.hits.resize((size_t)R.first[n] * 16); R.cigars.resize(coff[n]);
	wm::parallel_for(m->n_threads, (size_t)n, [&](size_t i) {
		if (!texts[i].empty()) memcpy(&R.text[toff[i]], texts[i].data(), texts[i].size());
		int32_t *ho = R.hits.data() + (size_t)R.first[i] * 16;
		uint32_t *co = R.cigars.data() + coff[i];
		for (const wm::Reg &r : out[i].regs) {
			const int32_t o[16] = { r.rid, r.rs, r.re, r.qs, r.qe, (int32_t)r.rev, (int32_t)r.mapq, r.has_p ? (int32_t)r.cigar.size() : 0, r.score, r.cnt, r.mlen, r.blen,
			                        r.dp_score, r.dp_max, r.dp_max2, (int32_t)((r.parent == r.id) | r.inv << 1 | r.sam_pri << 2 | r.split << 3 | (r.has_p ? r.trans_strand << 5 : 0)) };
			memcpy(ho, o, sizeof(o)); ho += 16;
			if (!r.cigar.empty()) { memcpy(co, r.cigar.data(), r.cigar.size() * 4); co += r.cigar.size(); }
		}
	});
	if (trace_m) fprintf(stderr, "[map_reads] n=%d ingest %.1f ms, map %.1f ms, format %.1f ms\n", n, tm1 - tm0, tm2 - tm1, now_ms() - tm2);
	std::lock_guard<std::mutex> stats_lk(m->stats_mu);
	m->stats[0] = st.n_flush; m->stats[1] = st.n_ksw; m->stats[2] = st.n_chain; m->stats[3] = st.n_seed; m->stats[4] = st.n_sketch;
	m->host_stats[0] += st.cpu_fiber; m->host_stats[1] += st.wall_idle;
	for (int op = 0; op < 4; ++op) { m->host_stats[2 + op] += st.cpu_op[op]; m->host_stats[6 + op] += st.wall_op[op]; m->host_stats[10 + op] += (double)st.n_batches[op]; }
	m->host_stats[14] += (tm2 - tm1) * 1e-3; m->host_stats[15] += (now_ms() - tm2) * 1e-3; m->host_stats[16] = m->call_threads(); m->host_stats[17] += st.cpu_help;
	m->host_stats[18] += st.wall_fiber; m->host_stats[19] += st.wall_lock; m->host_stats[20] += st.wall_total;
	if (trace_m) fprintf(stderr, "[host] fibers cpu %.2f s | idle wall %.2f s | batched calls cpu/wall/n: sketch %.2f/%.2f/%llu seed %.2f/%.2f/%llu chain %.2f/%.2f/%llu ksw %.2f/%.2f/%llu\n", st.cpu_fiber, st.wall_idle,
	                     st.cpu_op[0], st.wall_op[0], (unsigned long long)st.n_batches[0], st.cpu_op[1], st.wall_op[1], (unsigned long long)st.n_batches[1],
	                     st.cpu_op[2], st.wall_op[2], (unsigned long long)st.n_batches[2], st.cpu_op[3], st.wall_op[3], (unsigned long long)st.n_batches[3]);
	m->stats[5] = opsr.cells; m->stats[6] = (uint64_t)opsr.ksw_us; m->stats[7] = (uint64_t)opsr.aux_us; m->stats[8] = bases;
	return WM_OK;
}

static std::mutex g_cmdline_mu;
static std::vector<std::string> g_cmdline;
static bool g_split_pg = true;
extern "C" int wm_set_cmdline(int argc, const char *const *argv)
{
	if (argc > 0 && !argv) return set_err(WM_EINVAL, "bad argument");
	std::lock_guard<std::mutex> lk(g_cmdline_mu);
	g_split_pg = argc >= 0;
	g_cmdline.clear();
	if (argc > 0) g_cmdline.assign(argv, argv + argc);
	return WM_OK;
}
extern "C" int wm_mapper_set_cmdline(wm_mapper_t *m, int argc, const char *const *argv)
{
	if (!m || argc < 0 || (argc > 0 && !argv)) return set_err(WM_EINVAL, "bad argument");
	m->cmdline.assign(argv, argv + argc);
	return WM_OK;
}

struct LaneError {
	std::mutex mu; int code = 0; std::string msg;
	void keep(int rc) { std::lock_guard<std::mutex> lk(mu); if (!code) { code = rc; msg = wm_err_text(); } }
};

extern "C" int wm_map_file(wm_mapper_t *m, const char *reads_path, const char *out_path, int64_t mini_batch_bases, double *stats)
{
	wm_err_clear();
	FILE *out = strcmp(out_path, "-") == 0 ? stdout : fopen(out_path, "wb");
	if (!out) return set_err(WM_EINVAL, "cannot open '%s' for writing", out_path);
	std::string err;
	if ((m->mo.flag & 0x8) && m->sam_header) {
		std::string hdr;
		std::vector<const char*> av;
		for (const std::string &a : m->cmdline) av.push_back(a.c_str());
		wm::write_sam_header(hdr, m->idx->ix, (int)av.size(), av.data());
		if (fwrite(hdr.data(), 1, hdr.size(), out) != hdr.size()) { if (out != stdout) fclose(out); return set_err(WM_EINVAL, "write error on '%s'", out_path); }
	}
	wm::FileStats fs;
	const bool with_qual = (m->mo.flag & 0x8) != 0;
	LaneError le;
	const int rc = wm::map_file(reads_path, mini_batch_bases, with_qual, [&](std::vector<wm::ReadIn> &batch, std::string &text, int lane) {
		const int r = map_reads_impl(m, batch, now_ms(), lane);
		if (r == 0) text.swap(m->res[lane].text);
		else le.keep(r);
		return r;
	}, out, &fs, err);
	if (out != stdout) fclose(out);
	if (stats) { stats[0] = (double)fs.n_reads; stats[1] = (double)fs.n_bases; stats[2] = (double)fs.n_batches; stats[3] = fs.t_read; stats[4] = fs.t_map; stats[5] = fs.t_write; }
	if (rc) return le.code ? set_err(le.code, "%s", le.msg.c_str()) : set_err(WM_EINVAL, "%s", err.c_str());
	return WM_OK;
}

extern "C" int wm_map_file_multi(wm_mapper_t *const *ms, int n, const char *reads_path, const char *out_path, int64_t mini_batch_bases, double *stats)
{
	wm_err_clear();
	if (!ms || n < 1 || !reads_path || !out_path) return set_err(WM_EINVAL, "bad argument");
// ... 274 lines not shown
```

winnowmap_amd/csrc/wm_rt.h:

```cpp
#pragma once
#include <hip/hip_runtime.h>
#include <malloc.h>
#include <string.h>
#include <cstring>
#include <stdio.h>
#include <stdlib.h>
#include <string.h>
#include <stdarg.h>
#include <vector>
#include <new>
#include <algorithm>
#include <numeric>
#include <thread>
#include <chrono>
#include <atomic>
#include <mutex>
#include <unistd.h>
#include "host/wm_core.h"
#include "host/wm_index.h"
#include "wm_internal.h"
#include "ksw_plan.h"
struct wm_ctx_s;
void *pin_take(wm_ctx_s *c, size_t bytes, size_t *mark);
void pin_release(wm_ctx_s *c, size_t mark);
template <class T> struct UBuf {
	T *p; size_t n; wm_ctx_s *c; size_t mark; bool pinned;
	explicit UBuf(size_t n_, wm_ctx_s *c_ = 0) : p(0), n(n_), c(c_), mark(0), pinned(false)
	{
		const size_t bytes = (n_ ? n_ : 1) * sizeof(T);
		if (c) { p = (T*)pin_take(c, bytes, &mark); pinned = p != 0; }
		if (!p) p = (T*)malloc(bytes);
		if (!p) throw std::bad_alloc();
	}
	~UBuf() { if (pinned) pin_release(c, mark); else free(p); }
	UBuf(const UBuf&) = delete; UBuf &operator=(const UBuf&) = delete;
	T *data() { return p; } const T *data() const { return p; }
	size_t size() const { return n; }
	T &operator[](size_t i) { return p[i]; } const T &operator[](size_t i) const { return p[i]; }
	T *begin() { return p; } T *end() { return p + n; }
};
inline double now_ms() { return std::chrono::duration<double, std::milli>(std::chrono::steady_clock::now().time_since_epoch()).count(); }

namespace wm { int read_fastx(const std::string &fn, std::vector<std::string> &names, std::vector<std::string> &seqs, std::vector<std::string> *quals, std::vector<std::string> *comments, std::string &err); }

#ifndef WM_PRIO
#define WM_PRIO 1
#endif
#ifndef WM_STRIPE_PRIO
#define WM_STRIPE_PRIO 2
#endif
#if WM_PRIO
#define WM_SETPRIO(n) __builtin_amdgcn_s_setprio(n)
#else
#define WM_SETPRIO(n) ((void)0)
#endif

int set_err(int code, const char *fmt, ...);
void wm_err_clear();
const char *wm_err_text();
#define HIPCHK(x) do { hipError_t e_ = (x); if (e_ != hipSuccess) return set_err(WM_ENODEV, "%s failed: %s (%s:%d)", #x, hipGetErrorString(e_), __FILE__, __LINE__); } while (0)

struct wm_ctx_s {
	int device;
	hipStream_t stream;
	hipStream_t kstream[4];
	hipStream_t *side_pool; int n_side_pool; std::atomic<unsigned> *side_next;
	std::vector<hipStream_t> owned_pool; std::atomic<unsigned> owned_next[3];
	hipEvent_t kev[5];
	hipEvent_t cev[WM_KSW_NCLASS][2];
	double k_ms[WM_KSW_NCLASS]; uint64_t k_cells[WM_KSW_NCLASS], k_launches[WM_KSW_NCLASS];
	std::vector<std::pair<float, float>> k_iv[WM_KSW_NCLASS];
	std::mutex iv_mu;
	uint8_t *arena;
	size_t arena_bytes, arena_used;
	hipEvent_t ev[4];
	hipEvent_t sync_ev;
	float last_ms, aux_ms;
	int sketch_chunks;
	uint64_t acc_cells; double t_prep, t_run, t_fetch;
	uint64_t *d_hkey, *d_hval, *d_P;
	uint8_t *d_bloom;
	uint32_t *d_S;
	std::vector<uint64_t> seq_off; std::vector<uint32_t> seq_len;
	uint32_t *d_name_rank, *d_seq_len;
	uint64_t *d_reads, *d_reads_nm; size_t reads_bytes, reads_cap; bool owns_reads;
	int hbits;
	wm_sketch_params_t skp;
	bool have_index, owns_index;
	bool owns_filter;
	int host_threads;
	uint8_t *pin; size_t pin_bytes, pin_used;
	int *pin_small;
};

hipError_t ctx_sync(wm_ctx_s *c);
void wm_default_malloc();
hipEvent_t device_base_event(int device);
void side_split(int P, int *light, int *heavy);
void *arena_take(wm_ctx_t *c, size_t bytes);
struct ArenaMark { wm_ctx_t *c; size_t m; ArenaMark(wm_ctx_t *c_) : c(c_), m(c_->arena_used) {} ~ArenaMark() { c->arena_used = m; } };
int reads_alloc(wm_ctx_t *c, size_t cap);

struct wm_index_s { wm::Index ix; };

int sketch_batch_impl(wm_ctx_t *c, int n, const uint8_t *seqs, size_t seqs_bytes, const uint64_t *seq_off, const int32_t *len, const uint8_t *resident,
                      wm128_t *out, size_t out_cap, uint64_t *out_off, int32_t *counts);
int wm_index_build_seqs_dev(wm_ctx_t *c, const wm::IdxOpt &io, std::vector<std::string> &names, std::vector<std::string> &seqs, const std::string &kmer_file, int n_threads,
                            wm_index_t **out, double *stats = 0, bool replace_ok = true, double t0 = -1);
size_t sketch_long_bytes(int n, const wm_sketch_job_t *h_jobs, bool allow_long, bool hpc = false, bool even = false);
int sketch_launch(wm_ctx_t *c, int n, const wm_sketch_job_t *h_jobs, const wm_sketch_job_t *d_jobs, const int *d_ord, const uint8_t *d_seqs,
                  double *d_so, uint64_t *d_sx, uint32_t *d_sy, uint32_t *d_sl, wm128_t *d_out, int *d_cnt, bool allow_long, uint8_t *mem = 0, size_t mem_bytes = 0);

struct WinDev { wm_win_res_t *d_res; uint64_t *d_upool; wm128_t *d_vpool; uint64_t *d_ctr; uint64_t ctr[4]; uint32_t tot[3]; };
int window_launch(wm_ctx_t *c, int n, const wm_window_job_t *jobs, const uint8_t *seqs, size_t seqs_bytes, const wm128_t *pre, size_t n_pre_total,
                  int max_occ, int64_t flag, bool slot_full, WinDev &D, const wm_qkey_t *keys = 0, int sdust_thres = 0);
int window_fetch(wm_ctx_t *c, const WinDev &D, int n, wm_window_res_t *res, uint64_t *u_pool, wm128_t *a_pool);
int window_verdict(const WinDev &D, int round);
```

winnowmap_amd/csrc/wm_rt.hip:

```cpp
#include "wm_rt.h"

static thread_local char g_err[512] = "";
const char *wm_err_text() { return g_err; }
void wm_err_clear() { g_err[0] = 0; }
int set_err(int code, const char *fmt, ...)
{
	va_list ap;
	va_start(ap, fmt);
	vsnprintf(g_err, sizeof(g_err), fmt, ap);
	va_end(ap);
	return code;
}


void *pin_take(wm_ctx_s *c, size_t bytes, size_t *mark)
{
	if (!c->pin) {
		if (c->pin_bytes == (size_t)-1) return 0;
		const size_t want = (size_t)(getenv("WM_PINNED_MB") ? atoll(getenv("WM_PINNED_MB")) : 3072) << 20;
		if (want == 0 || hipHostMalloc((void**)&c->pin, want, hipHostMallocDefault) != hipSuccess) { c->pin = 0; c->pin_bytes = (size_t)-1; (void)hipGetLastError(); return 0; }
		c->pin_bytes = want; c->pin_used = 0;
	}
	const size_t off = (c->pin_used + 255) & ~(size_t)255;
	if (off + bytes > c->pin_bytes) return 0;
	*mark = c->pin_used;
	c->pin_used = off + bytes;
	return c->pin + off;
}
void pin_release(wm_ctx_s *c, size_t mark) { c->pin_used = mark; }


extern "C" const char *wm_last_error(void) { return g_err; }
#ifndef WM_BUILD_DEFINES
#define WM_BUILD_DEFINES ""
#endif
extern "C" const char *wm_build_defines(void) { return WM_BUILD_DEFINES; }

hipError_t ctx_sync(wm_ctx_s *c)
{
	static const bool spin = getenv("WM_SPIN_SYNC") != 0;
	if (spin) return hipStreamSynchronize(c->stream);
	hipError_t e = hipEventRecord(c->sync_ev, c->stream);
	if (e != hipSuccess) return e;
	int us = 50;
	for (;;) {
		e = hipEventQuery(c->sync_ev);
		if (e != hipErrorNotReady) return e;
		std::this_thread::sleep_for(std::chrono::microseconds(us));
		if (us < 1000) us *= 2;
	}
}

static void wm_default_hw_queues()
{
	static std::once_flag once;
	std::call_once(once, [] { if (!getenv("WM_NO_PROCESS_DEFAULTS")) setenv("GPU_MAX_HW_QUEUES", "20", 0); });
}

void wm_default_malloc()
{
	static std::once_flag once;
	std::call_once(once, [] {
		const char *off = getenv("WM_MALLOPT");
		if ((off && atoi(off) == 0) || getenv("WM_NO_PROCESS_DEFAULTS")) return;
		if (!getenv("MALLOC_TOP_PAD_")) mallopt(M_TOP_PAD, 64 << 20);
		if (!getenv("MALLOC_TRIM_THRESHOLD_")) mallopt(M_TRIM_THRESHOLD, 0x7fffffff);
		if (!getenv("MALLOC_MMAP_THRESHOLD_")) mallopt(M_MMAP_THRESHOLD, 32 << 20);
	});
}

hipEvent_t device_base_event(int device)
{
	static std::mutex mu;
	static std::vector<hipEvent_t> ev;
	std::lock_guard<std::mutex> lk(mu);
	if ((int)ev.size() <= device) ev.resize(device + 1, (hipEvent_t)0);
	if (!ev[device]) {
		hipEvent_t e;
		if (hipSetDevice(device) != hipSuccess || hipEventCreate(&e) != hipSuccess) return 0;
		if (hipEventRecord(e, 0) != hipSuccess || hipEventSynchronize(e) != hipSuccess) { hipEventDestroy(e); return 0; }
		ev[device] = e;
	}
	return ev[device];
}

void side_split(int P, int *light, int *heavy)
{
	int a = (P * 3 + 3) / 7, h = (P * 2 + 3) / 7;
	if (const char *e = getenv("WM_SIDE_SPLIT")) sscanf(e, "%d,%d", &a, &h);
	*light = std::max(0, a); *heavy = std::max(0, h);
}

extern "C" int wm_device_count(void)
{
	wm_default_hw_queues();
	int n = 0;
	if (hipGetDeviceCount(&n) != hipSuccess) return 0;
	return n;
}

extern "C" int wm_ctx_create(int device, size_t arena_bytes, wm_ctx_t **out)
{
	int n = 0;
	*out = 0;
	wm_default_hw_queues();
	if (hipGetDeviceCount(&n) != hipSuccess || n <= 0) return set_err(WM_ENODEV, "no HIP device visible (libwmgpu has no CPU fallback)");
	if (device < 0 || device >= n) return set_err(WM_EINVAL, "device %d out of range (%d visible)", device, n);
	HIPCHK(hipSetDevice(device));
	wm_ctx_t *c = new wm_ctx_t();
	c->device = device;
	if (arena_bytes == 0) {
		size_t fr = 0, tot = 0;
		HIPCHK(hipMemGetInfo(&fr, &tot));
		arena_bytes = fr / 4 < ((size_t)24 << 30) ? fr / 4 : ((size_t)24 << 30);
	}
	c->arena_bytes = arena_bytes;
	HIPCHK(hipMalloc((void**)&c->arena, arena_bytes));
	HIPCHK(hipStreamCreateWithFlags(&c->stream, hipStreamNonBlocking));
	for (int i = 0; i < 4; ++i) c->kstream[i] = 0;
	c->side_pool = 0; c->n_side_pool = 0; c->side_next = 0;
	for (int i = 0; i < 3; ++i) c->owned_next[i] = 0;
	for (int i = 0; i < 5; ++i) HIPCHK(hipEventCreateWithFlags(&c->kev[i], hipEventDisableTiming));
	for (int k = 0; k < WM_KSW_NCLASS; ++k) { HIPCHK(hipEventCreate(&c->cev[k][0])); HIPCHK(hipEventCreate(&c->cev[k][1])); c->k_ms[k] = 0; c->k_cells[k] = c->k_launches[k] = 0; }
	for (int i = 0; i < 4; ++i) HIPCHK(hipEventCreate(&c->ev[i]));
	HIPCHK(hipEventCreateWithFlags(&c->sync_ev, hipEventBlockingSync | hipEventDisableTiming));
	c->arena_used = 0; c->last_ms = 0; c->aux_ms = 0; c->sketch_chunks = 0; c->host_threads = 1; c->pin = 0; c->pin_bytes = c->pin_used = 0; c->have_index = false; c->owns_index = false; c->d_hkey = c->d_hval = c->d_P = 0; c->d_bloom = 0;
	c->owns_filter = false;
	c->pin_small = 0;
	if (hipHostMalloc((void**)&c->pin_small, 256, hipHostMallocDefault) != hipSuccess) { c->pin_small = 0; (void)hipGetLastError(); }
	c->d_S = 0; c->d_name_rank = c->d_seq_len = 0; c->d_reads = 0; c->d_reads_nm = 0; c->reads_bytes = c->reads_cap = 0; c->owns_reads = false;
	*out = c;
	return WM_OK;
}

extern "C" void wm_ctx_destroy(wm_ctx_t *c)
{
	if (!c) return;
	hipSetDevice(c->device);
	hipStreamSynchronize(c->stream);
	for (int i = 0; i < 4; ++i) hipEventDestroy(c->ev[i]);
	hipEventDestroy(c->sync_ev);
	hipStreamDestroy(c->stream);
	if (c->pin) hipHostFree(c->pin);
	if (c->pin_small) hipHostFree(c->pin_small);
	for (int i = 0; i < 4; ++i) if (c->kstream[i]) hipStreamDestroy(c->kstream[i]);
	for (hipStream_t st : c->owned_pool) hipStreamDestroy(st);
	for (int i = 0; i < 5; ++i) hipEventDestroy(c->kev[i]);
	for (int k = 0; k < WM_KSW_NCLASS; ++k) { hipEventDestroy(c->cev[k][0]); hipEventDestroy(c->cev[k][1]); }
	hipFree(c->arena);
	if (c->have_index && c->owns_index) { hipFree(c->d_hkey); hipFree(c->d_hval); hipFree(c->d_P); hipFree(c->d_bloom); hipFree(c->d_S); hipFree(c->d_name_rank); }
	if (c->d_reads && c->owns_reads) hipFree(c->d_reads);
	if (!c->have_index && c->owns_filter && c->d_bloom) hipFree(c->d_bloom);
	delete c;
}

extern "C" float wm_last_kernel_ms(const wm_ctx_t *c) { return c ? c->last_ms : 0.f; }
extern "C" int wm_ctx_device(const wm_ctx_t *c) { return c ? c->device : -1; }
extern "C" int wm_ctx_kernel_stats(const wm_ctx_t *c, double *out, int cap, int *n_classes)
{
	if (n_classes) *n_classes = WM_KSW_NCLASS;
	if (!c || !out) return set_err(WM_EINVAL, "null context or output");
	if (cap < 3 * WM_KSW_NCLASS) return set_err(WM_EINVAL, "need room for %d doubles", 3 * WM_KSW_NCLASS);
	for (int k = 0; k < WM_KSW_NCLASS; ++k) { out[3 * k] = c->k_ms[k]; out[3 * k + 1] = (double)c->k_cells[k]; out[3 * k + 2] = (double)c->k_launches[k]; }
	return WM_OK;
}

void *arena_take(wm_ctx_t *c, size_t bytes)
{
	size_t a = (c->arena_used + 255) & ~(size_t)255;
	if (a + bytes > c->arena_bytes) return 0;
	c->arena_used = a + bytes;
	return c->arena + a;
}
```

winnowmap_amd/gpu.py:

```python
import ctypes as C
import os
import numpy as np

HERE = os.path.dirname(os.path.abspath(__file__))
LIB_PATH = os.environ.get("WM_LIBWMGPU") or os.path.join(HERE, "libwmgpu.so")


class WmError(RuntimeError):
    pass


class KswScore(C.Structure):
    _fields_ = [("match", C.c_int8), ("mismatch", C.c_int8), ("sc_ambi", C.c_int8),
                ("q", C.c_int8), ("e", C.c_int8), ("q2", C.c_int8), ("e2", C.c_int8)]


KSW_JOB_DTYPE = np.dtype([("q_off", np.uint32), ("t_off", np.uint32), ("qlen", np.int32), ("tlen", np.int32),
                          ("w", np.int32), ("zdrop", np.int32), ("end_bonus", np.int32), ("flag", np.int32)])
KSW_RES_DTYPE = np.dtype([("max", np.int32), ("zdropped", np.int32), ("max_q", np.int32), ("max_t", np.int32),
                          ("mqe", np.int32), ("mqe_t", np.int32), ("mte", np.int32), ("mte_q", np.int32),
                          ("score", np.int32), ("reach_end", np.int32), ("n_cigar", np.int32), ("cig_off", np.uint32)])

KSW_F_ZDWALK = 0x10000
KSW_POS_DTYPE = np.dtype([("qwin_off", np.int64), ("qwin_len", np.int32), ("q_pos", np.int32), ("rid", np.int32), ("t_pos", np.int32),
                          ("qlen", np.int32), ("tlen", np.int32), ("w", np.int32), ("zdrop", np.int32), ("end_bonus", np.int32), ("flag", np.int32),
                          ("step", np.int8), ("has_n", np.int8), ("pad", np.int8, (6,))])

_lib = None


def lib():
    global _lib
    if _lib is None:
        if not os.path.exists(LIB_PATH):
            raise WmError("libwmgpu.so is not built (run `python -m winnowmap_amd.build`); there is no CPU fallback")
        L = C.CDLL(LIB_PATH)
        L.wm_last_error.restype = C.c_char_p
        L.wm_ctx_create.argtypes = [C.c_int, C.c_size_t, C.POINTER(C.c_void_p)]
        L.wm_ctx_destroy.argtypes = [C.c_void_p]
        L.wm_last_kernel_ms.restype = C.c_float
        L.wm_last_kernel_ms.argtypes = [C.c_void_p]
        L.wm_ksw_batch.argtypes = [C.c_void_p, C.POINTER(KswScore), C.c_int, C.c_void_p, C.c_void_p, C.c_size_t,
                                   C.c_void_p, C.c_void_p, C.c_size_t, C.POINTER(C.c_size_t)]
        L.wm_ksw_dev_prepare.argtypes = [C.c_void_p, C.POINTER(KswScore), C.c_int, C.c_void_p, C.c_void_p, C.c_size_t, C.POINTER(C.c_void_p)]
        L.wm_ksw_dev_run.argtypes = [C.c_void_p, C.c_void_p]
        L.wm_ksw_dev_fetch.argtypes = [C.c_void_p, C.c_void_p, C.c_void_p, C.c_void_p, C.c_size_t, C.POINTER(C.c_size_t)]
        L.wm_ksw_dev_stats.argtypes = [C.c_void_p, C.POINTER(C.c_uint64), C.POINTER(C.c_uint64), C.POINTER(C.c_float), C.POINTER(C.c_float)]
        L.wm_ksw_dev_free.argtypes = [C.c_void_p, C.c_void_p]
        _lib = L
    return _lib


def _chk(rc):
    if rc != 0:
        raise WmError("libwmgpu error %d: %s" % (rc, lib().wm_last_error().decode()))


class Context:

    def __init__(self, device=0, arena_bytes=0):
        self._h = C.c_void_p()
        _chk(lib().wm_ctx_create(device, arena_bytes, C.byref(self._h)))

    def close(self):
        if self._h:
            lib().wm_ctx_destroy(self._h)
            self._h = C.c_void_p()

    def __del__(self):
        try:
            self.close()
        except Exception:
            pass

    def last_sketch_chunks(self):
        lib().wm_last_sketch_chunks.argtypes = [C.c_void_p]
        lib().wm_last_sketch_chunks.restype = C.c_int
        return int(lib().wm_last_sketch_chunks(self._h))

    def ksw_batch(self, score, jobs, seqs):
        jobs = np.ascontiguousarray(jobs, KSW_JOB_DTYPE)
        seqs = np.ascontiguousarray(seqs, np.uint8)
        res = np.zeros(len(jobs), KSW_RES_DTYPE)
        cap = int((jobs["qlen"].astype(np.int64) + jobs["tlen"] + 2).sum()) + 16
        pool = np.zeros(cap, np.uint32)
        used = C.c_size_t(0)
        _chk(lib().wm_ksw_batch(self._h, C.byref(score), len(jobs), jobs.ctypes.data, seqs.ctypes.data, seqs.nbytes,
                                res.ctypes.data, pool.ctypes.data, cap, C.byref(used)))
        return res, pool[:used.value]

    def ksw_exts2_batch(self, score, noncan, junc_bonus, jobs, seqs, junc=None):
        jobs = np.ascontiguousarray(jobs, KSW_JOB_DTYPE)
        seqs = np.ascontiguousarray(seqs, np.uint8)
        jn = None if junc is None else np.ascontiguousarray(junc, np.uint8)
        assert jn is None or jn.nbytes == seqs.nbytes
        res = np.zeros(len(jobs), KSW_RES_DTYPE)
        cap = int((jobs["qlen"].astype(np.int64) + jobs["tlen"] + 2).sum()) + 16
        pool = np.zeros(cap, np.uint32)
        used = C.c_size_t(0)
        lib().wm_ksw_exts2_batch.argtypes = [C.c_void_p, C.POINTER(KswScore), C.c_int, C.c_int, C.c_int, C.c_void_p, C.c_void_p, C.c_size_t, C.c_void_p,
                                             C.c_void_p, C.c_void_p, C.c_size_t, C.POINTER(C.c_size_t)]
        _chk(lib().wm_ksw_exts2_batch(self._h, C.byref(score), noncan, junc_bonus, len(jobs), jobs.ctypes.data, seqs.ctypes.data, seqs.nbytes,
                                      None if jn is None else jn.ctypes.data, res.ctypes.data, pool.ctypes.data, cap, C.byref(used)))
        return res, pool[:used.value]

    def reads_upload(self, codes):
        codes = np.ascontiguousarray(codes, np.uint8)
        lib().wm_reads_upload.argtypes = [C.c_void_p, C.c_void_p, C.c_size_t]
        _chk(lib().wm_reads_upload(self._h, codes.ctypes.data, codes.nbytes))

    def ksw_batch_pos(self, score, jobs):
        jobs = np.ascontiguousarray(jobs, KSW_POS_DTYPE)
        assert KSW_POS_DTYPE.itemsize == 56
        res = np.zeros(len(jobs), KSW_RES_DTYPE)
        cap = int((np.maximum(jobs["qlen"], 0).astype(np.int64) + np.maximum(jobs["tlen"], 0) + 2).sum()) + 16
        pool = np.zeros(cap, np.uint32)
        used = C.c_size_t(0)
        lib().wm_ksw_batch_pos.argtypes = [C.c_void_p, C.POINTER(KswScore), C.c_int, C.c_void_p, C.c_void_p, C.c_void_p, C.c_size_t, C.POINTER(C.c_size_t)]
        _chk(lib().wm_ksw_batch_pos(self._h, C.byref(score), len(jobs), jobs.ctypes.data, res.ctypes.data, pool.ctypes.data, cap, C.byref(used)))
        return res, pool[:used.value]

    def ksw_batch_pos_zd(self, score, jobs):
        jobs = np.ascontiguousarray(jobs, KSW_POS_DTYPE)
        res = np.zeros(len(jobs), KSW_RES_DTYPE)
        cap = int((np.maximum(jobs["qlen"], 0).astype(np.int64) + np.maximum(jobs["tlen"], 0) + 2).sum()) + 16
        pool = np.zeros(cap, np.uint32)
        zd = np.zeros((len(jobs), 5), np.int32)
        used = C.c_size_t(0)
        lib().wm_ksw_batch_pos_zd.argtypes = [C.c_void_p, C.POINTER(KswScore), C.c_int, C.c_void_p, C.c_void_p, C.c_void_p, C.c_size_t, C.POINTER(C.c_size_t), C.c_void_p]
        _chk(lib().wm_ksw_batch_pos_zd(self._h, C.byref(score), len(jobs), jobs.ctypes.data, res.ctypes.data, pool.ctypes.data, cap, C.byref(used), zd.ctypes.data))
        return res, pool[:used.value], zd

    def extra_batch(self, score, jobs, seqs, cigars):
        jobs = np.ascontiguousarray(jobs, EXTRA_JOB_DTYPE)
        seqs = np.ascontiguousarray(seqs, np.uint8)
        cigars = np.ascontiguousarray(cigars, np.uint32)
        sc = np.array(score, np.int32)
        assert EXTRA_JOB_DTYPE.itemsize == 16 and sc.shape == (5,)
        out = np.zeros((len(jobs), 6), np.int32)
        lib().wm_extra_batch.argtypes = [C.c_void_p, C.c_void_p, C.c_int, C.c_void_p, C.c_void_p, C.c_size_t, C.c_void_p, C.c_size_t, C.c_void_p]
        _chk(lib().wm_extra_batch(self._h, sc.ctypes.data, len(jobs), jobs.ctypes.data, seqs.ctypes.data, seqs.nbytes, cigars.ctypes.data, len(cigars), out.ctypes.data))
        return out

    def extra_batch_pos(self, score, jobs, cigars):
        jobs = np.ascontiguousarray(jobs, EXTRA_POS_DTYPE)
        cigars = np.ascontiguousarray(cigars, np.uint32)
        sc = np.array(score, np.int32)
        assert EXTRA_POS_DTYPE.itemsize == 32 and sc.shape == (5,)
        out = np.zeros((len(jobs), 6), np.int32)
        lib().wm_extra_batch_pos.argtypes = [C.c_void_p, C.c_void_p, C.c_int, C.c_void_p, C.c_void_p, C.c_size_t, C.c_void_p]
        _chk(lib().wm_extra_batch_pos(self._h, sc.ctypes.data, len(jobs), jobs.ctypes.data, cigars.ctypes.data, len(cigars), out.ctypes.data))
        return out

    def fix_extra_batch(self, score, jobs, seqs, cigars):
        jobs = np.ascontiguousarray(jobs, EXTRA_JOB_DTYPE)
        seqs = np.ascontiguousarray(seqs, np.uint8)
        cigars = np.ascontiguousarray(cigars, np.uint32)
        sc = None if score is None else np.array(score, np.int32)
        assert sc is None or sc.shape == (5,)
        out = np.zeros(len(cigars), np.uint32); fix = np.zeros((len(jobs), 4), np.int32)
        extra = None if sc is None else np.zeros((len(jobs), 6), np.int32)
        lib().wm_fix_extra_batch.argtypes = [C.c_void_p, C.c_void_p, C.c_int, C.c_void_p, C.c_void_p, C.c_size_t, C.c_void_p, C.c_size_t, C.c_void_p, C.c_void_p, C.c_void_p]
        _chk(lib().wm_fix_extra_batch(self._h, None if sc is None else sc.ctypes.data, len(jobs), jobs.ctypes.data, seqs.ctypes.data, seqs.nbytes, cigars.ctypes.data,
                                      len(cigars), out.ctypes.data, fix.ctypes.data, None if extra is None else extra.ctypes.data))
        return out, fix, extra

    def fix_extra_batch_pos(self, score, jobs, cigars):
        jobs = np.ascontiguousarray(jobs, EXTRA_POS_DTYPE)
        cigars = np.ascontiguousarray(cigars, np.uint32)
        sc = None if score is None else np.array(score, np.int32)
        assert sc is None or sc.shape == (5,)
        out = np.zeros(len(cigars), np.uint32); fix = np.zeros((len(jobs), 4), np.int32)
        extra = None if sc is None else np.zeros((len(jobs), 6), np.int32)
        lib().wm_fix_extra_batch_pos.argtypes = [C.c_void_p, C.c_void_p, C.c_int, C.c_void_p, C.c_void_p, C.c_size_t, C.c_void_p, C.c_void_p, C.c_void_p]
        _chk(lib().wm_fix_extra_batch_pos(self._h, None if sc is None else sc.ctypes.data, len(jobs), jobs.ctypes.data, cigars.ctypes.data, len(cigars), out.ctypes.data,
                                          fix.ctypes.data, None if extra is None else extra.ctypes.data))
        return out, fix, extra

    def _eqx(self, fn, head, cigars, n_jobs, out_cap):
        cigars = np.ascontiguousarray(cigars, np.uint32)
        assert EQX_RES_DTYPE.itemsize == 16
        if out_cap is None:
            out_cap = len(cigars) + int((cigars[(cigars & 0xf) == 0] >> 4).astype(np.int64).sum())
        pool = np.zeros(max(int(out_cap), 1), np.uint32)
        res = np.zeros(n_jobs, EQX_RES_DTYPE)
        used = C.c_size_t(0)
        rc = fn(*head, cigars.ctypes.data, len(cigars), pool.ctypes.data, int(out_cap), C.byref(used), res.ctypes.data)
        if rc != 0:
            e = WmError("libwmgpu error %d: %s" % (rc, lib().wm_last_error().decode()))
            e.rc, e.needed, e.res = rc, used.value, res
            raise e
        return pool[:used.value], res

    def eqx_batch(self, jobs, seqs, cigars, out_cap=None):
        jobs = np.ascontiguousarray(jobs, EXTRA_JOB_DTYPE)
        seqs = np.ascontiguousarray(seqs, np.uint8)
        lib().wm_eqx_batch.argtypes = [C.c_void_p, C.c_int, C.c_void_p, C.c_void_p, C.c_size_t, C.c_void_p, C.c_size_t, C.c_void_p, C.c_size_t, C.POINTER(C.c_size_t), C.c_void_p]
        return self._eqx(lib().wm_eqx_batch, (self._h, len(jobs), jobs.ctypes.data, seqs.ctypes.data, seqs.nbytes), cigars, len(jobs), out_cap)

    def eqx_batch_pos(self, jobs, cigars, out_cap=None):
        jobs = np.ascontiguousarray(jobs, EXTRA_POS_DTYPE)
        lib().wm_eqx_batch_pos.argtypes = [C.c_void_p, C.c_int, C.c_void_p, C.c_void_p, C.c_size_t, C.c_void_p, C.c_size_t, C.POINTER(C.c_size_t), C.c_void_p]
        return self._eqx(lib().wm_eqx_batch_pos, (self._h, len(jobs), jobs.ctypes.data), cigars, len(jobs), out_cap)

    def _cs(self, fn, head, cigars, n_jobs, out_cap):
        cigars = np.ascontiguousarray(cigars, np.uint32)
        assert CS_RES_DTYPE.itemsize == 16
        if out_cap is None:
            op, ln = cigars & 0xf, (cigars >> 4).astype(np.int64)
            out_cap = int(np.where((op == 1) | (op == 2), ln + 12, np.where(op == 3, 16, 3 * ln + 12)).sum()) + 11 * n_jobs
        pool = np.zeros(max(int(out_cap), 1), np.uint8)
        res = np.zeros(n_jobs, CS_RES_DTYPE)
        used = C.c_size_t(0)
        rc = fn(*head, cigars.ctypes.data, len(cigars), pool.ctypes.data, int(out_cap), C.byref(used), res.ctypes.data)
        if rc != 0:
            e = WmError("libwmgpu error %d: %s" % (rc, lib().wm_last_error().decode()))
            e.rc, e.needed, e.res = rc, used.value, res
            raise e
        return pool[:used.value], res

    def cs_batch(self, mode, jobs, seqs, cigars, out_cap=None):
        jobs = np.ascontiguousarray(jobs, EXTRA_JOB_DTYPE)
        seqs = np.ascontiguousarray(seqs, np.uint8)
        lib().wm_cs_batch.argtypes = [C.c_void_p, C.c_int, C.c_int, C.c_void_p, C.c_void_p, C.c_size_t, C.c_void_p, C.c_size_t, C.c_void_p, C.c_size_t, C.POINTER(C.c_size_t), C.c_void_p]
        return self._cs(lib().wm_cs_batch, (self._h, int(mode), len(jobs), jobs.ctypes.data, seqs.ctypes.data, seqs.nbytes), cigars, len(jobs), out_cap)

    def cs_batch_pos(self, mode, jobs, cigars, out_cap=None):
        jobs = np.ascontiguousarray(jobs, EXTRA_POS_DTYPE)
        lib().wm_cs_batch_pos.argtypes = [C.c_void_p, C.c_int, C.c_int, C.c_void_p, C.c_void_p, C.c_size_t, C.c_void_p, C.c_size_t, C.POINTER(C.c_size_t), C.c_void_p]
        return self._cs(lib().wm_cs_batch_pos, (self._h, int(mode), len(jobs), jobs.ctypes.data), cigars, len(jobs), out_cap)

# ... 384 lines not shown
class SplitRun:

    def __init__(self, ctx, opt, k, w, n_threads, reads_path, mini_batch_bases=0):
        L = lib()
        L.wm_split_begin.argtypes = [C.c_void_p, C.POINTER(MapOpt), C.c_int, C.c_int, C.c_int, C.c_char_p, C.c_int64, C.POINTER(C.c_void_p)]
        L.wm_split_add_part.argtypes = [C.c_void_p, C.c_void_p]
        L.wm_split_finish.argtypes = [C.c_void_p, C.c_char_p, C.c_void_p]
        L.wm_split_abort.argtypes = [C.c_void_p]
        L.wm_split_abort.restype = None
        self._h = C.c_void_p()
        _chk(L.wm_split_begin(ctx._h, C.byref(opt), k, w, n_threads, os.fsencode(reads_path), mini_batch_bases, C.byref(self._h)))

    def add_part(self, idx):
        _chk(lib().wm_split_add_part(self._h, idx._h))

    def finish(self, out_path):
        st = np.zeros(6, np.float64)
        h, self._h = self._h, None
        _chk(lib().wm_split_finish(h, os.fsencode(out_path), st.ctypes.data))
        return dict(zip(("reads", "bases", "batches", "t_read", "t_map", "t_write"), (float(x) for x in st)))

    def abort(self):
        if self._h:
            lib().wm_split_abort(self._h)
            self._h = None


class Index:

    def __init__(self, fasta=None, kmer_file=None, k=15, w=50, n_threads=8, _handle=None, hpc=False):
        L = lib()
        _bind_map(L)
        self._h = C.c_void_p()
        if _handle is not None:
            self._h = _handle
            return
        L.wm_index_build_flag.argtypes = [C.c_char_p, C.c_char_p, C.c_int, C.c_int, C.c_int, C.c_int, C.POINTER(C.c_void_p)]
        _chk(L.wm_index_build_flag(os.fsencode(fasta), os.fsencode(kmer_file) if kmer_file else None, k, w, 1 if hpc else 0, n_threads, C.byref(self._h)))

    @staticmethod
    def build_on_device(ctx, fasta, kmer_file=None, k=15, w=50, n_threads=8, hpc=False):
        L = lib()
        _bind_map(L)
        L.wm_index_build_gpu_flag.argtypes = [C.c_void_p, C.c_char_p, C.c_char_p, C.c_int, C.c_int, C.c_int, C.c_int, C.POINTER(C.c_void_p), C.c_void_p]
        h = C.c_void_p()
        st = np.zeros(4, np.float64)
        _chk(L.wm_index_build_gpu_flag(ctx._h, os.fsencode(fasta), os.fsencode(kmer_file) if kmer_file else None, k, w, 1 if hpc else 0, n_threads, C.byref(h), st.ctypes.data))
        L.wm_last_aux_ms.restype = C.c_float
        L.wm_last_aux_ms.argtypes = [C.c_void_p]
        return Index(_handle=h), {"read_pack_s": float(st[0]), "device_sketch_s": float(st[1]), "table_s": float(st[2]), "minimizers": int(st[3]),
                                  "table_on_device_s": float(L.wm_last_aux_ms(ctx._h)) * 1e-3}

    def read_junc_bed(self, path):
        L = lib()
        L.wm_index_read_junc_bed.argtypes = [C.c_void_p, C.c_char_p]
        _chk(L.wm_index_read_junc_bed(self._h, os.fsencode(path)))

    def export_arrays(self):
        L = lib()
        sizes = np.zeros(9, np.uint64)
        _chk(L.wm_index_export(self._h, sizes.ctypes.data, None, None, None, None, None, None, None))
        n = [int(sizes[0]), int(sizes[1]), int(sizes[1]), int(sizes[2]), int(sizes[3]), 2 * int(sizes[4]), int(sizes[5])]
        arrs = [np.zeros(max(m, 1), dt) for m, dt in zip(n, _EXPORT_DTYPES)]
        _chk(L.wm_index_export(self._h, sizes.ctypes.data, *[a.ctypes.data for a in arrs]))
        return sizes, arrs

    @staticmethod
    def from_arrays(sizes, arrs):
        L = lib()
        _bind_map(L)
        h = C.c_void_p()
        arrs = [np.ascontiguousarray(a, dt) for a, dt in zip(arrs, _EXPORT_DTYPES)]
        sizes = np.ascontiguousarray(sizes, np.uint64)
        _chk(L.wm_index_import(sizes.ctypes.data, *[a.ctypes.data for a in arrs], C.byref(h)))
        return Index(_handle=h)

    def save(self, path):
        L = lib()
        L.wm_index_save.argtypes = [C.c_void_p, C.c_char_p]
        _chk(L.wm_index_save(self._h, path.encode()))

    @staticmethod
    def load(path, kmer_file=None):
        L = lib()
        _bind_map(L)
        L.wm_index_load.argtypes = [C.c_char_p, C.c_char_p, C.POINTER(C.c_void_p)]
        h = C.c_void_p()
        _chk(L.wm_index_load(path.encode(), kmer_file.encode() if kmer_file else None, C.byref(h)))
        return Index(_handle=h)

    def upload(self, ctx):
        _chk(lib().wm_index_upload(ctx._h, self._h))

    def upload_dev(self, ctx, d_ptrs, src_device):
        L = lib()
        L.wm_index_upload_dev.argtypes = [C.c_void_p, C.c_void_p] + [C.c_void_p] * 5 + [C.c_int]
        _chk(L.wm_index_upload_dev(ctx._h, self._h, *[C.c_void_p(int(p)) for p in d_ptrs], int(src_device)))

    def upload_peer(self, dst_ctx, src_ctx):
        L = lib()
        L.wm_index_upload_peer.argtypes = [C.c_void_p, C.c_void_p, C.c_void_p]
        _chk(L.wm_index_upload_peer(dst_ctx._h, self._h, src_ctx._h))

    @property
    def n_minimizers(self):
        if not self._h:
            raise RuntimeError("the index has been closed")
        return int(lib().wm_index_n_minimizers(self._h))

    def names(self):
        L = lib()
        return [L.wm_index_seq_name(self._h, i).decode() for i in range(L.wm_index_n_seq(self._h))]

    def query_key(self, name):
        return tuple(int(x) for x in self.query_keys([name])[0])

    def query_keys(self, names):
        L = lib()
        L.wm_index_query_key.argtypes = [C.c_void_p, C.c_char_p, C.c_void_p]
        out = np.zeros((len(names), 2), np.uint32)
        for i, nm in enumerate(names):
            _chk(L.wm_index_query_key(self._h, nm if isinstance(nm, bytes) else nm.encode(), out[i:].ctypes.data))
        return out

    def close(self):
        if self._h:
            lib().wm_index_destroy(self._h)
            self._h = C.c_void_p()


MM_F_CIGAR, MM_F_OUT_SAM, MM_F_OUT_CG = 0x4, 0x8, 0x20
MM_F_NO_DIAG, MM_F_NO_DUAL, MM_F_NO_LJOIN, MM_F_ALL_CHAINS = 0x1, 0x2, 0x400, 0x800000
MM_F_AVA = MM_F_ALL_CHAINS | MM_F_NO_DIAG | MM_F_NO_DUAL | MM_F_NO_LJOIN
MM_F_HEAP_SORT = 0x400000
MM_F_OUT_CS = 0x040
MM_F_OUT_CS_LONG = 0x800
MM_F_OUT_MD = 0x1000000
MM_F_EQX = 0x4000000
STAT_NAMES = ("super_steps", "ksw_jobs", "chain_jobs", "seed_jobs", "sketch_jobs", "dp_cells", "ksw_kernel_us", "aux_kernel_us", "read_bases")


class Mapper:

    def __init__(self, ctx, index, preset="map-ont", flag=MM_F_CIGAR | MM_F_OUT_CG):
        L = lib()
        _bind_map(L)
        self.ctx, self.index = ctx, index
        self._h = C.c_void_p()
        _chk(L.wm_mapper_create(ctx._h, index._h, preset.encode() if preset else None, flag, C.byref(self._h)))

    def set_threads(self, n_threads, arena_bytes_per_thread=0):
        _chk(lib().wm_mapper_set_threads(self._h, n_threads, arena_bytes_per_thread))

    @staticmethod
    def marshal(names, seqs):
        n = len(seqs)
        nm = (C.c_char_p * n)(*[x if isinstance(x, bytes) else x.encode() for x in names])
        sq = (C.c_char_p * n)(*seqs)
        lens = np.array([len(s) for s in seqs], np.int32)
        return n, nm, sq, lens, (names, seqs)

    def map(self, names, seqs=None, copy_text=True, slot=0):
        L = lib()
        n, nm, sq, lens, _keep = names if seqs is None else Mapper.marshal(names, seqs)
        text, tlen = C.c_char_p(), C.c_size_t()
        hits, cig, first = C.c_void_p(), C.c_void_p(), C.c_void_p()
        _chk(L.wm_map_reads_slot(self._h, slot, n, nm, sq, lens.ctypes.data, C.byref(text), C.byref(tlen), C.byref(hits), C.byref(cig), C.byref(first)))
        fa = np.ctypeslib.as_array(C.cast(first, C.POINTER(C.c_int64)), shape=(n + 1,)).copy()
        nh = int(fa[n])
        ha = np.ctypeslib.as_array(C.cast(hits, C.POINTER(C.c_int32)), shape=(nh, 16)).copy() if nh else np.zeros((0, 16), np.int32)
        if not copy_text:
            return tlen.value, ha, None, fa
        nc = int(ha[:, 7].sum()) if nh else 0
        ca = np.ctypeslib.as_array(C.cast(cig, C.POINTER(C.c_uint32)), shape=(nc,)).copy() if nc else np.zeros(0, np.uint32)
        return C.string_at(text, tlen.value), ha, ca, fa

    def rep_len_defined(self, slot=0):
        L = lib()
        L.wm_map_reads_rep_len_defined.argtypes = [C.c_void_p, C.c_int, C.POINTER(C.c_void_p), C.POINTER(C.c_size_t)]
        p, n = C.c_void_p(), C.c_size_t()
        _chk(L.wm_map_reads_rep_len_defined(self._h, slot, C.byref(p), C.byref(n)))
        return np.ctypeslib.as_array(C.cast(p, C.POINTER(C.c_uint8)), shape=(n.value,)).copy() if n.value else np.zeros(0, np.uint8)

    def stats(self):
        a = np.zeros(9, np.uint64)
        lib().wm_mapper_stats(self._h, a.ctypes.data)
        return dict(zip(STAT_NAMES, (int(x) for x in a)))

    def map_file(self, reads_path, out_path, mini_batch_bases=0):
        L = lib()
        L.wm_map_file.argtypes = [C.c_void_p, C.c_char_p, C.c_char_p, C.c_int64, C.c_void_p]
        st = np.zeros(6, np.float64)
        _chk(L.wm_map_file(self._h, reads_path.encode(), out_path.encode(), mini_batch_bases, st.ctypes.data))
        return dict(zip(("reads", "bases", "batches", "t_read", "t_map", "t_write"), (float(x) for x in st)))

    def kernel_stats(self):
        out = np.zeros(3 * 64, np.float64)
        n = C.c_int()
        lib().wm_mapper_kernel_stats.argtypes = [C.c_void_p, C.c_void_p, C.c_int, C.POINTER(C.c_int)]
        _chk(lib().wm_mapper_kernel_stats(self._h, out.ctypes.data, len(out), C.byref(n)))
        return {k: (float(out[3 * k]), float(out[3 * k + 1]), int(out[3 * k + 2])) for k in range(n.value)}

    def kernel_union(self, since_ms=0.0):
        ncl = int(lib().wm_ksw_n_classes())
        out = np.zeros(max(64, ncl), np.float64)
        now = C.c_double()
        lib().wm_mapper_kernel_union.argtypes = [C.c_void_p, C.c_double, C.c_void_p, C.c_int, C.POINTER(C.c_double)]
        _chk(lib().wm_mapper_kernel_union(self._h, float(since_ms), out.ctypes.data, len(out), C.byref(now)))
        return {k: float(out[k]) for k in range(ncl)}, now.value

    def host_stats(self):
        a = np.zeros(24, np.float64)
        lib().wm_mapper_host_stats.argtypes = [C.c_void_p, C.c_void_p, C.c_int]
        _chk(lib().wm_mapper_host_stats(self._h, a.ctypes.data, len(a)))
        ops = ("window", "seed", "chain", "ksw")
        return {"cpu_glue_s": float(a[0]), "idle_wall_s": float(a[1]), "cpu_batched_s": {o: float(a[2 + i]) for i, o in enumerate(ops)},
                "wall_batched_s": {o: float(a[6 + i]) for i, o in enumerate(ops)}, "batched_calls": {o: int(a[10 + i]) for i, o in enumerate(ops)},
                "map_wall_s": float(a[14]), "format_wall_s": float(a[15]), "threads": int(a[16]), "cpu_help_s": float(a[17]),
                "glue_wall_s": float(a[18]), "lock_wait_wall_s": float(a[19]), "workers_wall_s": float(a[20])}

    def close(self):
        if self._h:
            lib().wm_mapper_destroy(self._h)
            self._h = C.c_void_p()
```

Measured before the change: 0.1760.

## Add shared load-balanced stream queue set for mapper device ops

Adds a QueueSet of shared non-blocking streams with a load-estimating placement plan. Each batched device op (sketch, seed, chain, ksw, upload, etc.) temporarily moves its context stream to the least-loaded queue stream, charged by a running mean of that op's duration. When a queue set is present, it replaces the per-worker own stream, the ksw side-stream fan-out and the dedicated upload stream. The aim is better overlap of concurrent worker groups on the GPU, at the cost of mutex contention and extra bookkeeping. The layout heuristic decides between a narrow queue mode and the old side-pool mode based on WM_QSTREAMS and the thread count.

```diff
diff --git a/__graft_entry__.py b/__graft_entry__.py
--- a/__graft_entry__.py
+++ b/__graft_entry__.py
@@ -21,6 +21,7 @@
     b.build_emu_eqx()
     b.build_emu_cs()
     b.build_emu_chain()
+    b.build_emu_queue_plan()
     b.build_harness()
     import winnowmap_amd
     from winnowmap_amd import gpu
diff --git a/include/wm_gpu.h b/include/wm_gpu.h
--- a/include/wm_gpu.h
+++ b/include/wm_gpu.h
@@ -18,6 +18,8 @@
 
 int wm_ctx_create(int device, size_t arena_bytes, wm_ctx_t **out);
 void wm_ctx_destroy(wm_ctx_t *ctx);
+int wm_ctx_set_queue_streams(wm_ctx_t *ctx, int n);
+int wm_ctx_queue_streams(const wm_ctx_t *ctx);
 const char *wm_last_error(void);
 const char *wm_build_defines(void);
 int wm_device_count(void);
@@ -201,6 +203,8 @@
 int wm_map_reads_slot(wm_mapper_t *m, int slot, int n, const char *const *names, const char *const *seqs, const int32_t *lens,
                       const char **text, size_t *text_len, const int32_t **hits, const uint32_t **cigars, const int64_t **hit_first);
 int wm_mapper_set_slots(wm_mapper_t *m, int n);
+int wm_mapper_set_queue_streams(wm_mapper_t *m, int n);
+int wm_mapper_queue_streams(const wm_mapper_t *m);
 int wm_map_reads_rep_len_defined(const wm_mapper_t *m, int slot, const uint8_t **flags, size_t *n);
 int wm_map_file(wm_mapper_t *m, const char *reads_path, const char *out_path, int64_t mini_batch_bases, double *stats);
 int wm_index_upload_dev(wm_ctx_t *ctx, const wm_index_t *idx, const void *d_S, const void *d_hkey, const void *d_hval, const void *d_P, const void *d_bloom, int src_device);
diff --git a/winnowmap_amd/build.py b/winnowmap_amd/build.py
--- a/winnowmap_amd/build.py
+++ b/winnowmap_amd/build.py
@@ -225,6 +225,28 @@
     return out
 
 
+def build_emu_queue_plan():
+    emu = os.path.join(ROOT, "tests", "simt_emu")
+    out = os.path.join(emu, "libwm_emu_queue_plan.so")
+    srcs = [os.path.join(emu, "emu_queue_plan.cpp"), os.path.join(CSRC, "queue_plan.h")]
+    with _Lock(out):
+        if _newer(out, srcs):
+            _run_to(out, lambda o: ["g++", "-O2", "-std=c++17", "-fPIC", "-shared", "-pthread", "-I" + CSRC, "-o", o, os.path.join(emu, "emu_queue_plan.cpp")])
+    return out
+
+
+def build_emu_queue_plan_main(sanitize=True):
+    emu = os.path.join(ROOT, "tests", "simt_emu")
+    out = os.path.join(emu, "emu_queue_plan_main_san" if sanitize else "emu_queue_plan_main")
+    srcs = [os.path.join(emu, f) for f in ("emu_queue_plan_main.cpp", "emu_queue_plan.cpp")] + [os.path.join(CSRC, "queue_plan.h")]
+    with _Lock(out):
+        if _newer(out, srcs):
+            _run_to(out, lambda o: ["g++", "-O1", "-g", "-std=c++17", "-pthread"] +
+                                   (["-fsanitize=address,undefined", "-fno-sanitize-recover=undefined", "-fno-omit-frame-pointer"] if sanitize else []) +
+                                   ["-I" + CSRC, "-o", o, os.path.join(emu, "emu_queue_plan_main.cpp"), os.path.join(emu, "emu_queue_plan.cpp")])
+    return out
+
+
 def build_emu_stripe(defines=()):
     emu = os.path.join(ROOT, "tests", "simt_emu")
     tag = "".join("_" + "".join(ch if ch.isalnum() else "_" for ch in d) for d in defines)
diff --git a/winnowmap_amd/csrc/queue_plan.h b/winnowmap_amd/csrc/queue_plan.h
--- /dev/null
+++ b/winnowmap_amd/csrc/queue_plan.h
@@ -0,0 +1,115 @@
+#pragma once
+#include <stdint.h>
+#include <stdlib.h>
+#include <mutex>
+#include <vector>
+#include <algorithm>
+
+namespace wmq {
+
+static inline int queue_count(const char *env_value)
+{
+	int q = env_value && *env_value ? atoi(env_value) : 4;
+	return q < 1 ? 1 : q > 32 ? 32 : q;
+}
+
+static inline void pool_split(int P, int *light, int *heavy) { *light = (P * 3 + 3) / 7; *heavy = (P * 2 + 3) / 7; }
+
+struct Layout {
+	bool narrow;
+	int n_streams;
+	int pool, light, heavy, huge;
+};
+static inline Layout layout(int Q, int C, int forced)
+{
+	Layout l = { false, 0, 0, 0, 0, 0 };
+	if (C < 1) C = 1;
+	if (forced > 0 || (forced < 0 && Q < C + 6)) {
+		l.narrow = true;
+		l.n_streams = forced > 0 ? forced : Q;
+		l.n_streams = l.n_streams < 1 ? 1 : l.n_streams > 32 ? 32 : l.n_streams;
+		return l;
+	}
+	l.pool = C == 1 ? 0 : std::max(0, Q - C);
+	if (l.pool >= 6) { pool_split(l.pool, &l.light, &l.heavy); l.huge = l.pool - l.light - l.heavy; }
+	return l;
+}
+
+struct Mean {
+	double v = 0; bool seen = false;
+	void add(double x) { if (!(x >= 0)) return; v = seen ? v + (x - v) * 0.125 : x; seen = true; }
+};
+
+class Plan {
+public:
+	struct Group { uint64_t id; int stream; double est; const void *cookie; };
+	explicit Plan(int n_streams, int long_lanes = 0, double long_us = 8000.0) { reset(n_streams, long_lanes, long_us); }
+	void reset(int n_streams, int long_lanes = 0, double long_us = 8000.0)
+	{
+		std::lock_guard<std::mutex> lk(mu_);
+		n_ = n_streams < 1 ? 1 : n_streams;
+		long_lanes_ = long_lanes > 0 ? std::min(long_lanes, n_) : std::max(1, n_ / 2);
+		long_us_ = long_us;
+		load_.assign(n_, 0.0); live_.clear(); placed_ = retired_ = 0; next_id_ = 1;
+	}
+	int n() const { return n_; }
+	int long_lanes() const { return long_lanes_; }
+	double long_us() const { return long_us_; }
+	bool is_long(double est) const { return est >= long_us_; }
+	template <class Done> int pick(double est, Done done, uint64_t *id, bool any_lane = false)
+	{
+		if (!(est > 0)) est = 0;
+		std::lock_guard<std::mutex> lk(mu_);
+		retire_locked(done);
+		const int hi = !any_lane && est >= long_us_ ? long_lanes_ : n_;
+		int s = 0;
+		for (int i = 1; i < hi; ++i) if (load_[i] < load_[s]) s = i;
+		charge_locked(s, est, id);
+		return s;
+	}
+	void arm(uint64_t id, const void *cookie)
+	{
+		std::lock_guard<std::mutex> lk(mu_);
+		for (Group &g : live_) if (g.id == id) { g.cookie = cookie; return; }
+	}
+	template <class Done> void retire(Done done) { std::lock_guard<std::mutex> lk(mu_); retire_locked(done); }
+	void complete(uint64_t id)
+	{
+		std::lock_guard<std::mutex> lk(mu_);
+		for (size_t i = 0; i < live_.size(); ++i) if (live_[i].id == id) { drop_locked(i); return; }
+	}
+	double outstanding(int s) const { std::lock_guard<std::mutex> lk(mu_); return s >= 0 && s < n_ ? load_[s] : 0.0; }
+	int live() const { std::lock_guard<std::mutex> lk(mu_); return (int)live_.size(); }
+	double placed_us() const { std::lock_guard<std::mutex> lk(mu_); return placed_; }
+	double retired_us() const { std::lock_guard<std::mutex> lk(mu_); return retired_; }
+private:
+	void charge_locked(int s, double est, uint64_t *id)
+	{
+		const uint64_t g = next_id_++;
+		live_.push_back(Group{ g, s, est, 0 });
+		load_[s] += est; placed_ += est;
+		if (id) *id = g;
+	}
+	void drop_locked(size_t i)
+	{
+		const Group g = live_[i];
+		live_[i] = live_.back(); live_.pop_back();
+		retired_ += g.est;
+		load_[g.stream] -= g.est;
+		bool any = false;
+		for (const Group &o : live_) if (o.stream == g.stream) { any = true; break; }
+		if (!any || load_[g.stream] < 0) load_[g.stream] = any ? std::max(0.0, load_[g.stream]) : 0.0;
+	}
+	template <class Done> void retire_locked(Done done)
+	{
+		for (size_t i = 0; i < live_.size();) { if (live_[i].cookie && done(live_[i].cookie)) drop_locked(i); else ++i; }
+	}
+	mutable std::mutex mu_;
+	int n_, long_lanes_; double long_us_;
+	std::vector<double> load_;
+	std::vector<Group> live_;
+	double placed_, retired_;
+	uint64_t next_id_;
+};
+
+}
diff --git a/winnowmap_amd/csrc/wm_ksw.hip b/winnowmap_amd/csrc/wm_ksw.hip
--- a/winnowmap_amd/csrc/wm_ksw.hip
+++ b/winnowmap_amd/csrc/wm_ksw.hip
@@ -609,7 +609,7 @@
 	int n_nonempty = 0, used_mask = 0, rr = 0;
 	for (int k = 0; k < WM_KSW_NCLASS; ++k) n_nonempty += !b->order[k].empty();
 	static const int n_side = std::max(0, std::min(4, getenv("WM_SIDE_STREAMS") ? atoi(getenv("WM_SIDE_STREAMS")) : 3));
-	const bool fan = n_nonempty > 1 && !trace_k && n_side > 0;
+	const bool fan = !c->qs && n_nonempty > 1 && !trace_k && n_side > 0;
 	if (fan) HIPCHK(hipEventRecord(c->kev[4], c->stream));
 	hipStream_t ks = c->stream;
 	hipStream_t side[4] = {0, 0, 0, 0};
@@ -852,6 +852,7 @@
                           wm_ksw_result_t *results, uint32_t *cigar_pool, size_t cigar_cap, size_t *cigar_used, wm_zd_t *zd = 0)
 {
 	if (!c) return set_err(WM_EINVAL, "null context");
+	QMain qmain(c, WM_QOP_KSW);
 	size_t used = 0;
 	int i0 = 0;
 	float kms = 0;
@@ -869,7 +870,7 @@
 		wm_ksw_dev_batch_t *b = 0;
 		const double ta = now_ms();
 		int rc = ksw_prepare_impl(c, sc, i1 - i0, pos ? 0 : jobs + i0, seqs, seqs_bytes, pos ? pos + i0 : 0, &b);
-		if (rc) return rc;
+		if (rc) { qmain.failed(); return rc; }
 		const double tb_ = now_ms();
 		rc = wm_ksw_dev_run(c, b);
 		const double tc = now_ms();
@@ -878,7 +879,7 @@
 		if (!rc && zd) rc = ksw_fetch_zd(c, b, zd + i0);
 		c->acc_cells += b->cells; c->t_prep += tb_ - ta; c->t_run += tc - tb_; c->t_fetch += now_ms() - tc; kms += b->dp_ms + b->bt_ms;
 		wm_ksw_dev_free(c, b);
-		if (rc) { if (cigar_used) *cigar_used = used + u; return rc; }
+		if (rc) { qmain.failed(); if (cigar_used) *cigar_used = used + u; return rc; }
 		for (int i = i0; i < i1; ++i) results[i].cig_off += (uint32_t)used;
 		used += u;
 		i0 = i1;
diff --git a/winnowmap_amd/csrc/wm_mapper.hip b/winnowmap_amd/csrc/wm_mapper.hip
--- a/winnowmap_amd/csrc/wm_mapper.hip
+++ b/winnowmap_amd/csrc/wm_mapper.hip
@@ -499,11 +499,15 @@
 			for (size_t i = 2 * ((n + 63) / 64); i < pkw; ++i) h_pk[i] = 0;
 			for (size_t i = (n + 63) / 64; i < nmw; ++i) h_nm[i] = 0;
 		}
-		if (!up_stream && hipStreamCreateWithFlags(&up_stream, hipStreamNonBlocking) != hipSuccess) { up_stream = 0; (void)hipGetLastError(); }
+		QueueSet *const qs = c0->qs;
+		uint64_t q_id = 0; const double q_t0 = now_ms();
+		if (!qs && !up_stream && hipStreamCreateWithFlags(&up_stream, hipStreamNonBlocking) != hipSuccess) { up_stream = 0; (void)hipGetLastError(); }
+		const hipStream_t copy_on = qs ? qs->streams[qs->plan.pick(qs->op_estimate(WM_QOP_UPLOAD), QueueSet::event_done, &q_id, true)] : up_stream;
+		struct UpDone { QueueSet *qs; uint64_t id; double t0; ~UpDone() { if (qs) { qs->plan.complete(id); qs->saw_op(WM_QOP_UPLOAD, (now_ms() - t0) * 1e3); } } } up_done{ qs, q_id, q_t0 };
 		uint64_t *d_pk = c0->d_reads + (size_t)slot * slab / 32, *d_nm = c0->d_reads_nm + (size_t)slot * slab / 64;
-		if (n && (up_stream ? (hipMemcpyAsync(d_pk, h_pk, pkw * 8, hipMemcpyHostToDevice, up_stream) != hipSuccess || hipMemcpyAsync(d_nm, h_nm, nmw * 8, hipMemcpyHostToDevice, up_stream) != hipSuccess ||
-		                       hipStreamSynchronize(up_stream) != hipSuccess)
-		                    : (hipMemcpy(d_pk, h_pk, pkw * 8, hipMemcpyHostToDevice) != hipSuccess || hipMemcpy(d_nm, h_nm, nmw * 8, hipMemcpyHostToDevice) != hipSuccess))) {
+		if (n && (copy_on ? (hipMemcpyAsync(d_pk, h_pk, pkw * 8, hipMemcpyHostToDevice, copy_on) != hipSuccess || hipMemcpyAsync(d_nm, h_nm, nmw * 8, hipMemcpyHostToDevice, copy_on) != hipSuccess ||
+		                     hipStreamSynchronize(copy_on) != hipSuccess)
+		                  : (hipMemcpy(d_pk, h_pk, pkw * 8, hipMemcpyHostToDevice) != hipSuccess || hipMemcpy(d_nm, h_nm, nmw * 8, hipMemcpyHostToDevice) != hipSuccess))) {
 			err = std::string("reads upload: ") + hipGetErrorString(hipGetLastError()); return false;
 		}
 		for (GpuOpsCtx &x : ctxs) x.resident = true;
@@ -512,14 +516,18 @@
 		return true;
 	}
 	void release_reads(int slot) { std::lock_guard<std::mutex> lk(reads_mu); if (slot >= 0 && slot < WM_MAX_SLOTS) slot_busy[slot] = false; }
-	template <class F> void with(wm::ErrorSink &sink, F f)
+	template <class F> void with(wm::ErrorSink &sink, int op, F f)
 	{
 		{ std::lock_guard<std::mutex> lk(sink.mu); if (!sink.msg.empty()) return; }
 		int i;
 		{ std::unique_lock<std::mutex> lk(mu); cv.wait(lk, [&] { return !free_.empty(); }); i = free_.back(); free_.pop_back(); }
 		ctxs[i].error.clear();
-		try { f(ctxs[i]); }
-		catch (const std::exception &e) { if (ctxs[i].error.empty()) ctxs[i].error = std::string("batched device call: ") + e.what(); }
+		{
+			QMain qmain(ctxs[i].c, op);
+			try { f(ctxs[i]); }
+			catch (const std::exception &e) { if (ctxs[i].error.empty()) ctxs[i].error = std::string("batched device call: ") + e.what(); }
+			if (!ctxs[i].error.empty()) qmain.failed();
+		}
 		if (!ctxs[i].error.empty()) { sink.put(ctxs[i].error); ctxs[i].error.clear(); }
 		{ std::lock_guard<std::mutex> lk(mu); free_.push_back(i); }
 		cv.notify_one();
@@ -534,23 +542,23 @@
 		run_split(x, a, f);
 		if (x.error.empty()) run_split(x, b, f);
 	}
-	void sketch_batch(wm::ErrorSink &e, int w, int k, std::vector<wm::SketchReq*> &reqs) { with(e, [&](GpuOpsCtx &x) { run_split(x, reqs, [&](std::vector<wm::SketchReq*> &part) { x.sketch_batch(w, k, part); }); }); }
-	void seed_batch(wm::ErrorSink &e, std::vector<wm::SeedReq*> &reqs) { with(e, [&](GpuOpsCtx &x) { run_split(x, reqs, [&](std::vector<wm::SeedReq*> &part) { x.seed_batch(part); }); }); }
-	void chain_batch(wm::ErrorSink &e, std::vector<wm::ChainReq*> &reqs) { with(e, [&](GpuOpsCtx &x) { run_split(x, reqs, [&](std::vector<wm::ChainReq*> &part) { x.chain_batch(part); }); }); }
-	void ksw_batch(wm::ErrorSink &e, const wm_ksw_score_t &sc, std::vector<wm::KswReq*> &reqs) { with(e, [&](GpuOpsCtx &x) { x.ksw_batch(sc, reqs); }); }
-	void exts2_batch(wm::ErrorSink &e, const wm_ksw_score_t &sc, int noncan, int junc_bonus, std::vector<wm::KswReq*> &reqs) { with(e, [&](GpuOpsCtx &x) { x.exts2_batch(sc, noncan, junc_bonus, reqs); }); }
+	void sketch_batch(wm::ErrorSink &e, int w, int k, std::vector<wm::SketchReq*> &reqs) { with(e, WM_QOP_SKETCH, [&](GpuOpsCtx &x) { run_split(x, reqs, [&](std::vector<wm::SketchReq*> &part) { x.sketch_batch(w, k, part); }); }); }
+	void seed_batch(wm::ErrorSink &e, std::vector<wm::SeedReq*> &reqs) { with(e, WM_QOP_SEED, [&](GpuOpsCtx &x) { run_split(x, reqs, [&](std::vector<wm::SeedReq*> &part) { x.seed_batch(part); }); }); }
+	void chain_batch(wm::ErrorSink &e, std::vector<wm::ChainReq*> &reqs) { with(e, WM_QOP_CHAIN, [&](GpuOpsCtx &x) { run_split(x, reqs, [&](std::vector<wm::ChainReq*> &part) { x.chain_batch(part); }); }); }
+	void ksw_batch(wm::ErrorSink &e, const wm_ksw_score_t &sc, std::vector<wm::KswReq*> &reqs) { with(e, WM_QOP_KSW, [&](GpuOpsCtx &x) { x.ksw_batch(sc, reqs); }); }
+	void exts2_batch(wm::ErrorSink &e, const wm_ksw_score_t &sc, int noncan, int junc_bonus, std::vector<wm::KswReq*> &reqs) { with(e, WM_QOP_EXTS2, [&](GpuOpsCtx &x) { x.exts2_batch(sc, noncan, junc_bonus, reqs); }); }
 	void extra_batch(wm::ErrorSink &e, const wm_extra_score_t &sc, std::vector<wm::ExtraReq*> &reqs, bool *served)
 	{
 		*served = false;
-		with(e, [&](GpuOpsCtx &x) { bool all = true; run_split(x, reqs, [&](std::vector<wm::ExtraReq*> &part) { all = x.extra_batch(sc, part) && all; }); *served = all; });
-	}
-	template <class R, class F> void batch_or_rest(wm::ErrorSink &e, std::vector<R*> &reqs, std::vector<R*> &rest, F call)
+		with(e, WM_QOP_EXTRA, [&](GpuOpsCtx &x) { bool all = true; run_split(x, reqs, [&](std::vector<wm::ExtraReq*> &part) { all = x.extra_batch(sc, part) && all; }); *served = all; });
+	}
+	template <class R, class F> void batch_or_rest(wm::ErrorSink &e, int op, std::vector<R*> &reqs, std::vector<R*> &rest, F call)
 	{
 		bool ran = false;
-		with(e, [&](GpuOpsCtx &x) { ran = true; run_split(x, reqs, [&](std::vector<R*> &part) { if (!call(x, part)) rest.insert(rest.end(), part.begin(), part.end()); }); });
+		with(e, op, [&](GpuOpsCtx &x) { ran = true; run_split(x, reqs, [&](std::vector<R*> &part) { if (!call(x, part)) rest.insert(rest.end(), part.begin(), part.end()); }); });
 		if (!ran) rest = reqs;
 	}
-	void window_batch(wm::ErrorSink &e, std::vector<wm::WindowReq*> &reqs) { with(e, [&](GpuOpsCtx &x) { run_split(x, reqs, [&](std::vector<wm::WindowReq*> &part) { x.window_batch(part); }); }); }
+	void window_batch(wm::ErrorSink &e, std::vector<wm::WindowReq*> &reqs) { with(e, WM_QOP_WINDOW, [&](GpuOpsCtx &x) { run_split(x, reqs, [&](std::vector<wm::WindowReq*> &part) { x.window_batch(part); }); }); }
 };
 
 struct CallOps : wm::DeviceOps {
@@ -582,19 +590,19 @@
 	void fix_extra_batch(const wm_extra_score_t &sc, std::vector<wm::FixReq*> &reqs) override
 	{
 		std::vector<wm::FixReq*> rest;
-		g.batch_or_rest(err, reqs, rest, [&](GpuOpsCtx &x, std::vector<wm::FixReq*> &part) { return x.fix_extra_batch(sc, part); });
+		g.batch_or_rest(err, WM_QOP_FIX, reqs, rest, [&](GpuOpsCtx &x, std::vector<wm::FixReq*> &part) { return x.fix_extra_batch(sc, part); });
 		if (!rest.empty()) wm::DeviceOps::fix_extra_batch(sc, rest);
 	}
 	void cs_batch(std::vector<wm::CsReq*> &reqs) override
 	{
 		std::vector<wm::CsReq*> rest;
-		g.batch_or_rest(err, reqs, rest, [](GpuOpsCtx &x, std::vector<wm::CsReq*> &part) { return x.cs_batch(part); });
+		g.batch_or_rest(err, WM_QOP_CS, reqs, rest, [](GpuOpsCtx &x, std::vector<wm::CsReq*> &part) { return x.cs_batch(part); });
 		if (!rest.empty()) wm::DeviceOps::cs_batch(rest);
 	}
 	void eqx_batch(std::vector<wm::EqxReq*> &reqs) override
 	{
 		std::vector<wm::EqxReq*> rest;
-		g.batch_or_rest(err, reqs, rest, [](GpuOpsCtx &x, std::vector<wm::EqxReq*> &part) { return x.eqx_batch(part); });
+		g.batch_or_rest(err, WM_QOP_EQX, reqs, rest, [](GpuOpsCtx &x, std::vector<wm::EqxReq*> &part) { return x.eqx_batch(part); });
 		if (!rest.empty()) wm::DeviceOps::eqx_batch(rest);
 	}
 };
@@ -612,9 +620,13 @@
 	std::mutex stats_mu;
 	std::unique_ptr<GpuOps> ops;
 	int slots_hint = 0;
+	int qstreams = -1;
+	bool layout_done = false;
 	bool sam_header = true;
 	std::vector<std::string> cmdline;
 };
+
+static int mapper_apply_layout(wm_mapper_t *m);
 
 static std::atomic<int> g_even_k(-1);
 static bool even_k_on()
@@ -709,6 +721,7 @@
 	if (!m) return;
 	if (wm::prof_on()) wm::prof_report(stderr);
 	for (wm_ctx_t *w : m->workers) wm_ctx_destroy(w);
+	if (m->c->qs && m->c->owns_qs && m->layout_done) { hipSetDevice(m->c->device); queue_set_destroy(m->c->qs); m->c->qs = 0; m->c->owns_qs = false; }
 	delete m;
 }
 
@@ -733,20 +746,47 @@
 		w->host_threads = m->c->host_threads;
 		m->workers.push_back(w);
 	}
-	{
-		const int hwq = getenv("GPU_MAX_HW_QUEUES") ? atoi(getenv("GPU_MAX_HW_QUEUES")) : 4;
-		int P = getenv("WM_SIDE_POOL") ? atoi(getenv("WM_SIDE_POOL")) : std::max(0, hwq - C);
+	{ const int rc = mapper_apply_layout(m); if (rc) return rc; }
+	{ size_t mark = 0; if (pin_take(m->c, 1, &mark)) pin_release(m->c, mark); }
+	for (wm_ctx_t *w : m->workers) { size_t mark = 0; if (pin_take(w, 1, &mark)) pin_release(w, mark); }
+	return WM_OK;
+}
+
+static int mapper_apply_layout(wm_mapper_t *m)
+{
+	{
+		const int C = 1 + (int)m->workers.size();
+		const char *hwq_env = getenv("GPU_MAX_HW_QUEUES");
+		const int forced = m->qstreams >= 0 ? m->qstreams : wm_qstreams_env();
+		const wmq::Layout lay = wmq::layout(forced == 0 ? (hwq_env ? atoi(hwq_env) : 4) : wmq::queue_count(hwq_env), C, forced);
+		int P = lay.narrow ? 0 : getenv("WM_SIDE_POOL") ? atoi(getenv("WM_SIDE_POOL")) : lay.pool;
 		if (C == 1) P = 0;
 		wm_ctx_t *c0 = m->c;
+		HIPCHK(hipSetDevice(c0->device));
 		HIPCHK(hipStreamSynchronize(c0->stream));
+		for (wm_ctx_t *w : m->workers) { w->qs = 0; w->owns_qs = false; }
+		if (c0->qs && c0->owns_qs) queue_set_destroy(c0->qs);
+		c0->qs = 0; c0->owns_qs = false;
+		if (lay.narrow) { const int rc = queue_set_create(c0->device, lay.n_streams, &c0->qs); if (rc) return rc; c0->owns_qs = true; }
+		for (wm_ctx_t *w : m->workers) { w->qs = c0->qs; w->owns_qs = false; }
 		while ((int)c0->owned_pool.size() > P) { hipStreamDestroy(c0->owned_pool.back()); c0->owned_pool.pop_back(); }
 		while ((int)c0->owned_pool.size() < P) { hipStream_t st; HIPCHK(hipStreamCreateWithFlags(&st, hipStreamNonBlocking)); c0->owned_pool.push_back(st); }
 		c0->side_pool = P > 0 ? c0->owned_pool.data() : 0; c0->n_side_pool = P; c0->side_next = c0->owned_next;
 		for (wm_ctx_t *w : m->workers) { w->side_pool = c0->side_pool; w->n_side_pool = P; w->side_next = c0->owned_next; }
 	}
-	{ size_t mark = 0; if (pin_take(m->c, 1, &mark)) pin_release(m->c, mark); }
-	for (wm_ctx_t *w : m->workers) { size_t mark = 0; if (pin_take(w, 1, &mark)) pin_release(w, mark); }
-	return WM_OK;
+	m->layout_done = true;
+	return WM_OK;
+}
+
+extern "C" int wm_mapper_queue_streams(const wm_mapper_t *m) { return m ? wm_ctx_queue_streams(m->c) : 0; }
+
+extern "C" int wm_mapper_set_queue_streams(wm_mapper_t *m, int n)
+{
+	if (!m) return set_err(WM_EINVAL, "null mapper");
+	if (n > 32) return set_err(WM_EINVAL, "queue streams must be at most 32");
+	std::lock_guard<std::mutex> lk(m->stats_mu);
+	m->qstreams = n < 0 ? -1 : n;
+	return mapper_apply_layout(m);
 }
 
 static int map_reads_impl(wm_mapper_t *m, std::vector<wm::ReadIn> &reads, double tm0, int slot = 0);
@@ -787,6 +827,7 @@
 
 static void ensure_ops(wm_mapper_t *m)
 {
+	if (!m->layout_done && mapper_apply_layout(m)) m->layout_done = true;
 	if (m->ops) return;
 	m->ops.reset(new GpuOps());
 	std::vector<wm_ctx_t*> cs; cs.push_back(m->c); cs.insert(cs.end(), m->workers.begin(), m->workers.end());
diff --git a/winnowmap_amd/csrc/wm_rt.h b/winnowmap_amd/csrc/wm_rt.h
--- a/winnowmap_amd/csrc/wm_rt.h
+++ b/winnowmap_amd/csrc/wm_rt.h
@@ -20,6 +20,7 @@
 #include "host/wm_index.h"
 #include "wm_internal.h"
 #include "ksw_plan.h"
+#include "queue_plan.h"
 struct wm_ctx_s;
 void *pin_take(wm_ctx_s *c, size_t bytes, size_t *mark);
 void pin_release(wm_ctx_s *c, size_t mark);
@@ -60,12 +61,29 @@
 const char *wm_err_text();
 #define HIPCHK(x) do { hipError_t e_ = (x); if (e_ != hipSuccess) return set_err(WM_ENODEV, "%s failed: %s (%s:%d)", #x, hipGetErrorString(e_), __FILE__, __LINE__); } while (0)
 
+enum { WM_QOP_SKETCH = 0, WM_QOP_SEED, WM_QOP_CHAIN, WM_QOP_KSW, WM_QOP_EXTS2, WM_QOP_WINDOW, WM_QOP_EXTRA, WM_QOP_FIX, WM_QOP_EQX, WM_QOP_CS, WM_QOP_UPLOAD, WM_QOP_N };
+struct QueueSet {
+	std::vector<hipStream_t> streams;
+	wmq::Plan plan;
+	std::mutex mu;
+	wmq::Mean op_us[WM_QOP_N];
+	explicit QueueSet(int n) : plan(n) {}
+	double op_estimate(int op) { std::lock_guard<std::mutex> lk(mu); return op_us[op].v; }
+	void saw_op(int op, double us) { std::lock_guard<std::mutex> lk(mu); op_us[op].add(us); }
+	static bool event_done(const void *ev) { return hipEventQuery((hipEvent_t)ev) != hipErrorNotReady; }
+};
+int queue_set_create(int device, int n_streams, QueueSet **out);
+void queue_set_destroy(QueueSet *qs);
+int wm_qstreams_env();
+
 struct wm_ctx_s {
 	int device;
 	hipStream_t stream;
 	hipStream_t kstream[4];
 	hipStream_t *side_pool; int n_side_pool; std::atomic<unsigned> *side_next;
 	std::vector<hipStream_t> owned_pool; std::atomic<unsigned> owned_next[3];
+	QueueSet *qs; bool owns_qs;
+	hipStream_t own_stream;
 	hipEvent_t kev[5];
 	hipEvent_t cev[WM_KSW_NCLASS][2];
 	double k_ms[WM_KSW_NCLASS]; uint64_t k_cells[WM_KSW_NCLASS], k_launches[WM_KSW_NCLASS];
@@ -94,6 +112,26 @@
 };
 
 hipError_t ctx_sync(wm_ctx_s *c);
+struct QMain {
+	wm_ctx_s *c; uint64_t id; bool on; int op; double t0;
+	QMain(wm_ctx_s *c_, int op_) : c(c_), id(0), on(false), op(op_), t0(0)
+	{
+		if (!c || !c->qs || c->stream != c->own_stream) return;
+		t0 = now_ms();
+		const int s = c->qs->plan.pick(c->qs->op_estimate(op), QueueSet::event_done, &id, true);
+		c->stream = c->qs->streams[s];
+		on = true;
+	}
+	void failed() { if (on) { (void)hipStreamSynchronize(c->stream); (void)hipGetLastError(); } }
+	~QMain()
+	{
+		if (!on) return;
+		c->qs->plan.complete(id);
+		c->qs->saw_op(op, (now_ms() - t0) * 1e3);
+		c->stream = c->own_stream;
+	}
+	QMain(const QMain&) = delete; QMain &operator=(const QMain&) = delete;
+};
 void wm_default_malloc();
 hipEvent_t device_base_event(int device);
 void side_split(int P, int *light, int *heavy);
diff --git a/winnowmap_amd/csrc/wm_rt.hip b/winnowmap_amd/csrc/wm_rt.hip
--- a/winnowmap_amd/csrc/wm_rt.hip
+++ b/winnowmap_amd/csrc/wm_rt.hip
@@ -84,9 +84,57 @@
 	return ev[device];
 }
 
+int wm_qstreams_env()
+{
+	const char *e = getenv("WM_QSTREAMS");
+	if (!e || !*e) return -1;
+	const int n = atoi(e);
+	return n < 0 ? -1 : n > 32 ? 32 : n;
+}
+
+int queue_set_create(int device, int n_streams, QueueSet **out)
+{
+	*out = 0;
+	if (n_streams < 1 || n_streams > 32) return set_err(WM_EINVAL, "queue streams must be 1 .. 32");
+	HIPCHK(hipSetDevice(device));
+	QueueSet *qs = new QueueSet(n_streams);
+	for (int i = 0; i < n_streams; ++i) {
+		hipStream_t st;
+		const hipError_t e = hipStreamCreateWithFlags(&st, hipStreamNonBlocking);
+		if (e != hipSuccess) { queue_set_destroy(qs); return set_err(WM_ENODEV, "hipStreamCreateWithFlags failed: %s", hipGetErrorString(e)); }
+		qs->streams.push_back(st);
+	}
+	*out = qs;
+	return WM_OK;
+}
+void queue_set_destroy(QueueSet *qs)
+{
+	if (!qs) return;
+	for (hipStream_t st : qs->streams) { hipStreamSynchronize(st); hipStreamDestroy(st); }
+	delete qs;
+}
+extern "C" int wm_ctx_set_queue_streams(wm_ctx_t *c, int n)
+{
+	if (!c) return set_err(WM_EINVAL, "null context");
+	if (n < 0 || n > 32) return set_err(WM_EINVAL, "queue streams must be 0 .. 32");
+	HIPCHK(hipSetDevice(c->device));
+	HIPCHK(hipStreamSynchronize(c->stream));
+	c->stream = c->own_stream;
+	if (c->qs && c->owns_qs) queue_set_destroy(c->qs);
+	c->qs = 0; c->owns_qs = false;
+	if (n == 0) return WM_OK;
+	const int rc = queue_set_create(c->device, n, &c->qs);
+	if (rc) return rc;
+	c->owns_qs = true;
+	return WM_OK;
+}
+
+extern "C" int wm_ctx_queue_streams(const wm_ctx_t *c) { return c && c->qs ? (int)c->qs->streams.size() : 0; }
+
 void side_split(int P, int *light, int *heavy)
 {
-	int a = (P * 3 + 3) / 7, h = (P * 2 + 3) / 7;
+	int a, h;
+	wmq::pool_split(P, &a, &h);
 	if (const char *e = getenv("WM_SIDE_SPLIT")) sscanf(e, "%d,%d", &a, &h);
 	*light = std::max(0, a); *heavy = std::max(0, h);
 }
@@ -117,6 +165,7 @@
 	c->arena_bytes = arena_bytes;
 	HIPCHK(hipMalloc((void**)&c->arena, arena_bytes));
 	HIPCHK(hipStreamCreateWithFlags(&c->stream, hipStreamNonBlocking));
+	c->own_stream = c->stream; c->qs = 0; c->owns_qs = false;
 	for (int i = 0; i < 4; ++i) c->kstream[i] = 0;
 	c->side_pool = 0; c->n_side_pool = 0; c->side_next = 0;
 	for (int i = 0; i < 3; ++i) c->owned_next[i] = 0;
@@ -138,6 +187,8 @@
 	if (!c) return;
 	hipSetDevice(c->device);
 	hipStreamSynchronize(c->stream);
+	if (c->qs && c->owns_qs) queue_set_destroy(c->qs);
+	c->qs = 0; c->stream = c->own_stream;
 	for (int i = 0; i < 4; ++i) hipEventDestroy(c->ev[i]);
 	hipEventDestroy(c->sync_ev);
 	hipStreamDestroy(c->stream);
diff --git a/winnowmap_amd/gpu.py b/winnowmap_amd/gpu.py
--- a/winnowmap_amd/gpu.py
+++ b/winnowmap_amd/gpu.py
@@ -77,6 +77,16 @@
         lib().wm_last_sketch_chunks.argtypes = [C.c_void_p]
         lib().wm_last_sketch_chunks.restype = C.c_int
         return int(lib().wm_last_sketch_chunks(self._h))
+
+    def set_queue_streams(self, n):
+        lib().wm_ctx_set_queue_streams.argtypes = [C.c_void_p, C.c_int]
+        lib().wm_ctx_set_queue_streams.restype = C.c_int
+        _chk(lib().wm_ctx_set_queue_streams(self._h, n))
+
+    def queue_streams(self):
+        lib().wm_ctx_queue_streams.argtypes = [C.c_void_p]
+        lib().wm_ctx_queue_streams.restype = C.c_int
+        return int(lib().wm_ctx_queue_streams(self._h))
 
     def ksw_batch(self, score, jobs, seqs):
         jobs = np.ascontiguousarray(jobs, KSW_JOB_DTYPE)
@@ -767,6 +777,16 @@
     def set_threads(self, n_threads, arena_bytes_per_thread=0):
         _chk(lib().wm_mapper_set_threads(self._h, n_threads, arena_bytes_per_thread))
 
+    def set_queue_streams(self, n):
+        lib().wm_mapper_set_queue_streams.argtypes = [C.c_void_p, C.c_int]
+        lib().wm_mapper_set_queue_streams.restype = C.c_int
+        _chk(lib().wm_mapper_set_queue_streams(self._h, n))
+
+    def queue_streams(self):
+        lib().wm_mapper_queue_streams.argtypes = [C.c_void_p]
+        lib().wm_mapper_queue_streams.restype = C.c_int
+        return int(lib().wm_mapper_queue_streams(self._h))
+
     @staticmethod
     def marshal(names, seqs):
         n = len(seqs)
```

New measurement: 0.2148, median of 6. +22.1%, better.
